# yu45020/Text_Segmentation_Image_Inpainting

Measured on NVIDIA H100. Metric: PartialConv UNet 512x512 images/sec (fwd+bwd), higher is better.
Workload: dtype bf16

## Files before the change

text_segmentation_image_inpainting_b200/csrc/conv_stem.cu:

```cuda
#include <string.h>

#include <algorithm>

#include "pcb_common.cuh"

namespace {

constexpr int S2D_C = 32;
constexpr int SK = 4;

struct StemPlan {
    bool ok;
    pcb_conv sub;
    size_t sub_fe;
    size_t fwd_extra;
};

StemPlan plan_of(const pcb_conv *c) {
    StemPlan K;
    memset(&K, 0, sizeof(K));
    if (getenv("PCB_DISABLE_S2D_STEM")) return K;
    if (c->dtype != PCB_BF16 || c->groups != 1 || c->nparts != 1 || c->kh != 7 || c->kw != 7 || c->stride != 2 || c->pad_h != 3 || c->pad_w != 3 ||
        c->dil != 1) return K;
    const pcb_part &p = c->parts[0];
    if (p.x_up || p.c > 8 || p.x_cstride != 8 || (p.mask && p.mask_up != 0) || ((c->h | c->w) & 1)) return K;
    if (p.x && (reinterpret_cast<uintptr_t>(p.x) & 15)) return K;
    if (c->ho != c->h / 2 || c->wo != c->w / 2 || c->cout < 32 || (c->cout & 7)) return K;
    pcb_conv &S = K.sub;
    S.n = c->n; S.h = c->h / 2; S.w = c->w / 2; S.cin = S2D_C; S.cout = c->cout; S.kh = S.kw = SK; S.stride = 1; S.pad_h = S.pad_w = 2; S.dil = 1;
    S.groups = 1; S.ho = S.h; S.wo = S.w; S.dtype = PCB_BF16; S.no_guard = c->no_guard; S.nparts = 1;
    S.parts[0].x = nullptr; S.parts[0].mask = nullptr; S.parts[0].c = S2D_C; S.parts[0].x_cstride = S2D_C;
    if (!pcb_tc_eligible(&S)) return K;
    size_t de;
    pcb_tc_weight_layout(&S, &K.sub_fe, &de);
    K.sub_fe = (K.sub_fe + 63) / 64 * 64;
    K.fwd_extra = K.sub_fe + 2 * static_cast<size_t>(c->cout) * SK * SK * S2D_C;
    K.ok = true;
    return K;
}

size_t rup256(size_t v) { return (v + 255) / 256 * 256; }
size_t s2d_bytes(const pcb_conv *c) { return rup256(static_cast<size_t>(c->n) * (c->h / 2) * (c->w / 2) * S2D_C * sizeof(bf16)); }
size_t dwsub_bytes(const pcb_conv *c) { return rup256(sizeof(float) * c->cout * SK * SK * S2D_C); }

__global__ void s2d_kernel(const bf16 *__restrict__ x, const uint8_t *__restrict__ mask, bf16 *__restrict__ xs, int n, int h, int w) {
    const int hs = h >> 1, ws = w >> 1;
    const long long total = static_cast<long long>(n) * hs * ws * 2;
    for (long long i = blockIdx.x * static_cast<long long>(blockDim.x) + threadIdx.x; i < total; i += static_cast<long long>(gridDim.x) * blockDim.x) {
        const int a = static_cast<int>(i & 1);
        const long long cell = i >> 1;
        const int sx = static_cast<int>(cell % ws);
        const long long t = cell / ws;
        const int sy = static_cast<int>(t % hs), img = static_cast<int>(t / hs);
        const long long q = (static_cast<long long>(img) * h + 2 * sy + a) * w + 2 * sx;
        uint4 v0 = __ldg(reinterpret_cast<const uint4 *>(x + q * 8)), v1 = __ldg(reinterpret_cast<const uint4 *>(x + q * 8 + 8));
        if (mask) {
            if (mask[q] == 0) v0 = make_uint4(0u, 0u, 0u, 0u);
            if (mask[q + 1] == 0) v1 = make_uint4(0u, 0u, 0u, 0u);
        }
        uint4 *dst = reinterpret_cast<uint4 *>(xs + cell * S2D_C + a * 16);
        dst[0] = v0; dst[1] = v1;
    }
}

__global__ void stem_weight_kernel(const float *__restrict__ w, float *__restrict__ wsub, int cout, int cin) {
    const int i = blockIdx.x * blockDim.x + threadIdx.x;
    if (i >= cout * SK * SK * S2D_C) return;
    const int k = i % S2D_C, jb = (i / S2D_C) % SK, ja = (i / (S2D_C * SK)) % SK, co = i / (S2D_C * SK * SK);
    const int ch = k & 7, b = (k >> 3) & 1, a = k >> 4;
    const int ty = 2 * ja + a - 1, tx = 2 * jb + b - 1;
    wsub[i] = (ty >= 0 && ty < 7 && tx >= 0 && tx < 7 && ch < cin) ? w[((static_cast<long long>(co) * 7 + ty) * 7 + tx) * cin + ch] : 0.f;
}

__global__ void stem_dw_gather_kernel(const float *__restrict__ dwsub, float *__restrict__ dw, int cout, int cin) {
    const int i = blockIdx.x * blockDim.x + threadIdx.x;
    if (i >= cout * 49 * cin) return;
    const int ch = i % cin, tx = (i / cin) % 7, ty = (i / (cin * 7)) % 7, co = i / (cin * 49);
    const int ja = (ty + 1) >> 1, a = (ty + 1) & 1, jb = (tx + 1) >> 1, b = (tx + 1) & 1;
    dw[i] += dwsub[((static_cast<long long>(co) * SK + ja) * SK + jb) * S2D_C + (a * 2 + b) * 8 + ch];
}

int run_s2d(const pcb_conv *c, bf16 *xs, cudaStream_t st) {
    const pcb_part &p = c->parts[0];
    PCB_CHECK(p.x != nullptr, "space-to-depth stem: null x");
    const long long total = static_cast<long long>(c->n) * (c->h / 2) * (c->w / 2) * 2;
    const int grid = static_cast<int>(std::max<long long>(1, std::min<long long>((total + 255) / 256, 16ll * pcb_num_sms())));
    s2d_kernel<<<grid, 256, 0, st>>>(static_cast<const bf16 *>(p.x), p.mask, xs, c->n, c->h, c->w);
    PCB_LAUNCH_CHECK();
    return 0;
}

}

bool pcb_stem_ok(const pcb_conv *c) { return plan_of(c).ok; }

size_t pcb_stem_weight_extra(const pcb_conv *c) {
    const StemPlan K = plan_of(c);
    return K.ok ? K.fwd_extra : 0;
}

size_t pcb_stem_workspace(const pcb_conv *c) {
    StemPlan K = plan_of(c);
    if (!K.ok) return 0;
    return s2d_bytes(c) + dwsub_bytes(c) + pcb_tc_workspace(&K.sub);
}

int pcb_stem_weight_prepare(const pcb_conv *c, const float *w_master, void *w_fwd_extra, bool zero_padding, cudaStream_t st) {
    const StemPlan K = plan_of(c);
    PCB_CHECK(K.ok && w_fwd_extra, "space-to-depth stem: weight prepare on a layer that does not take this path");
    float *wsub = reinterpret_cast<float *>(static_cast<bf16 *>(w_fwd_extra) + K.sub_fe);
    const int total = c->cout * SK * SK * S2D_C;
    stem_weight_kernel<<<(total + 255) / 256, 256, 0, st>>>(w_master, wsub, c->cout, c->cin);
    PCB_LAUNCH_CHECK();
    return pcb_tc_weight_prepare(&K.sub, wsub, w_fwd_extra, nullptr, zero_padding, st);
}

int pcb_stem_forward(const pcb_conv *c, const void *w_fwd_extra, const float *bias, void *y, int y_cstride, const float *msum, void *workspace,
                     double *bn_sums, const pcb_ep *ep, cudaStream_t st) {
    StemPlan K = plan_of(c);
    PCB_CHECK(K.ok && workspace, "space-to-depth stem forward: wrong layer / no workspace");
    uint8_t *ws = static_cast<uint8_t *>(workspace);
    bf16 *xs = reinterpret_cast<bf16 *>(ws);
    if (int rc = run_s2d(c, xs, st)) return rc;
    K.sub.parts[0].x = xs;
    uint64_t *sub_ws = reinterpret_cast<uint64_t *>(ws + s2d_bytes(c) + dwsub_bytes(c));
    if (int rc = pcb_tc_forward_mask_pass(&K.sub, sub_ws, st)) return rc;
    return pcb_tc_forward_ws(&K.sub, w_fwd_extra, bias, y, y_cstride, msum, sub_ws, true, bn_sums, ep, st);
}

int pcb_stem_wgrad(const pcb_conv *c, const void *dc, int dc_cstride, float *dw, void *workspace, bool zero_dw, cudaStream_t st) {
    StemPlan K = plan_of(c);
    PCB_CHECK(K.ok && workspace, "space-to-depth stem wgrad: wrong layer / no workspace");
    if (zero_dw) PCB_CUDA(cudaMemsetAsync(dw, 0, sizeof(float) * c->cout * 49 * c->cin, st));
    uint8_t *ws = static_cast<uint8_t *>(workspace);
    bf16 *xs = reinterpret_cast<bf16 *>(ws);
    float *dwsub = reinterpret_cast<float *>(ws + s2d_bytes(c));
    void *sub_ws = ws + s2d_bytes(c) + dwsub_bytes(c);
    if (int rc = run_s2d(c, xs, st)) return rc;
    K.sub.parts[0].x = xs;
    if (int rc = pcb_tc_wgrad(&K.sub, dc, dc_cstride, dwsub, sub_ws, true, st)) return rc;
    const int total = c->cout * 49 * c->cin;
    stem_dw_gather_kernel<<<(total + 255) / 256, 256, 0, st>>>(dwsub, dw, c->cout, c->cin);
    PCB_LAUNCH_CHECK();
    return 0;
}
```

text_segmentation_image_inpainting_b200/csrc/conv_tc.cu:

```cuda
#include <cuda.h>
#include <stdlib.h>
#include <string.h>

#include <algorithm>

#include "pcb_common.cuh"
#include "pcb_ptx.cuh"

namespace {

constexpr int BLOCK_M = 128;
constexpr int BLOCK_K = 64;
constexpr int A_STAGE_BYTES = BLOCK_M * 128;
constexpr int NUM_PRODUCER_THREADS = 128;
constexpr int TC_MAX_PARTS = 2;
constexpr int MMA_WARPS = 8;
constexpr int MMA_THREADS = MMA_WARPS * 32;
constexpr int acc_pitch(int block_n) { return block_n + 4; }
constexpr int acc_stage_bytes(int block_n) { return BLOCK_M * acc_pitch(block_n) * 4; }

inline int rup(int v, int m) { return (v + m - 1) / m * m; }

struct TcPart {
    const bf16 *x;
// ... 371 lines not shown
                }
#pragma unroll
                for (int p = 0; p < TC_MAX_PARTS; ++p)
                    if (p < P.nparts) wnext[p][i] = __ldg(P.parts[p].tapmask + idx);
            }
        };
        issue_mask_loads(blockIdx.x);
        for (int tile = blockIdx.x; tile < num_tiles && !dead; tile += gridDim.x) {
            const int m0 = (tile / n_tiles) * BLOCK_M, n0 = (tile % n_tiles) * BLOCK_N;
            uint64_t wcur[TC_MAX_PARTS][NW];
#pragma unroll
            for (int p = 0; p < TC_MAX_PARTS; ++p)
#pragma unroll
                for (int i = 0; i < NW; ++i) wcur[p][i] = wnext[p][i];
            issue_mask_loads(tile + gridDim.x);
            if (!tile_active(n0)) continue;
            if (HALO) {
                int ph[HALO_MAX_HG];
                int cterm[TC_MAX_PARTS][HALO_MAX_HG];
                uint32_t vb[TC_MAX_PARTS][HALO_MAX_HG];
#pragma unroll
                for (int i = 0; i < HALO_MAX_HG; ++i) {
                    ph[i] = 0;
#pragma unroll
                    for (int p = 0; p < TC_MAX_PARTS; ++p) { vb[p][i] = 0; cterm[p][i] = 0; }
                    if (i >= HG) continue;
                    const int S = r0 + 16 * i;
                    const int g = S / HG, sl = S - g * HG;
                    const int m = m0 + g * 8;
                    const bool ok = m < P.m_total;
                    const int mm = ok ? m : 0;
                    const int nn = mm / plane, rem = mm - nn * plane;
                    const int hh = rem / pwid, ww = rem - hh * pwid;
                    if (MODE == 0) {
                        ph[i] = hh - P.pad_h;
                        const int col = ww - P.pad_w + sl;
                        const int tcs = sl > 7 ? (sl - 7 + P.dil - 1) / P.dil : 0;
#pragma unroll
                        for (int p = 0; p < TC_MAX_PARTS; ++p) {
                            if (p >= P.nparts || !ok) continue;
                            const TcPart &pt = P.parts[p];
                            const uint64_t word = wcur[p][i];
                            uint32_t bits = 0;
                            for (int tr = 0; tr < P.kh; ++tr) bits |= static_cast<uint32_t>((word >> (tr * P.kw + tcs)) & 1ull) << tr;
                            vb[p][i] = bits;
                            const int colc = min(max(col, 0), P.w - 1) >> pt.xup;
                            cterm[p][i] = (nn * (P.h >> pt.xup) * (P.w >> pt.xup) + colc) * pt.cstride + chunk * 8;
                        }
                    } else {
                        ph[i] = hh + P.pad_h;
                        const int col = ww + P.pad_w - (P.kw - 1) * P.dil + sl;
                        const bool cok = ok && col >= 0 && col < P.wo;
                        uint32_t bits = 0;
                        for (int tr = 0; tr < P.kh; ++tr) { const int hi = ph[i] - tr * P.dil; bits |= (cok && hi >= 0 && hi < P.ho ? 1u : 0u) << tr; }
                        vb[0][i] = bits;
                        cterm[0][i] = (nn * P.ho * P.wo + min(max(col, 0), P.wo - 1)) * P.dc_cstride + chunk * 8;
                    }
                }
                for (int tr = 0; tr < P.kh && !dead; ++tr) {
#pragma unroll
                    for (int p = 0; p < TC_MAX_PARTS; ++p) {
                        if (p >= np || dead) break;
                        const TcPart &pt = P.parts[p];
                        const bf16 *src = (MODE == 0) ? pt.x : P.dc;
                        const int xup = (MODE == 0) ? pt.xup : 0;
                        const int hmax = ((MODE == 0) ? (P.h >> xup) : P.ho) - 1;
                        const int rowpitch = (MODE == 0) ? (P.w >> xup) * pt.cstride : P.wo * P.dc_cstride;
                        const int nb = ((MODE == 0) ? pt.kext : P.dc_kext) / BLOCK_K;
                        const int c8 = (MODE == 0) ? pt.c8 : P.dc_c8;
                        int rterm[HALO_MAX_HG];
#pragma unroll
                        for (int i = 0; i < HALO_MAX_HG; ++i) {
                            const int hi = (MODE == 0) ? ((ph[i] + tr * P.dil) >> xup) : (ph[i] - tr * P.dil);
                            rterm[i] = cterm[p][i] + min(max(hi, 0), hmax) * rowpitch;
                        }
                        for (int cb = 0; cb < nb; ++cb, ++it) {
                            const int s = it % SA;
                            if (!ptx::mbar_wait(bar_empty_a + 8 * s, ((it / SA) & 1) ^ 1, P.abort_flag, 111)) { dead = true; break; }
                            const bool cv = cb * BLOCK_K + chunk * 8 < c8;
                            const uint32_t dst0 = sA + s * A_STAGE + chunk * LBO + r0 * 16;
                            const bf16 *srcb = src + cb * BLOCK_K;
#pragma unroll
                            for (int i = 0; i < HALO_MAX_HG; ++i) {
                                if (i >= HG) break;
                                ptx::cp_async_16(dst0 + i * 256, srcb + rterm[i], cv && ((vb[p][i] >> tr) & 1u));
                            }
                            ptx::cp_async_mbar_arrive(bar_full_a + 8 * s);
                            ptx::mbar_arrive(bar_full_a + 8 * s);
                        }
                    }
                }
            } else {
                const uint32_t sw = static_cast<uint32_t>((chunk ^ (r0 & 7)) << 4);
                int ph[8], pw[8];
                int ibase[TC_MAX_PARTS][8];
                bool prow[8];
                const int ls = 31 - __clz(P.stride);
#pragma unroll
                for (int i = 0; i < 8; ++i) {
                    const int m = m0 + r0 + 16 * i;
                    prow[i] = m < P.m_total;
                    const int mm = prow[i] ? m : 0;
                    const int nn = mm / plane, rem = mm - nn * plane;
                    const int hh = rem / pwid, ww = rem - hh * pwid;
                    if (MODE == 0) {
                        ph[i] = hh * P.stride - P.pad_h; pw[i] = ww * P.stride - P.pad_w;
#pragma unroll
                        for (int p = 0; p < TC_MAX_PARTS; ++p)
                            ibase[p][i] = (p < P.nparts) ? nn * (P.h >> P.parts[p].xup) * (P.w >> P.parts[p].xup) * P.parts[p].cstride + chunk * 8 : 0;
                    } else {
                        ph[i] = hh + P.pad_h; pw[i] = ww + P.pad_w;
                        ibase[0][i] = nn * P.ho * P.wo * P.dc_cstride + chunk * 8;
#pragma unroll
                        for (int p = 1; p < TC_MAX_PARTS; ++p) ibase[p][i] = 0;
                    }
                }
                uint64_t tmv[TC_MAX_PARTS][8];
#pragma unroll
                for (int p = 0; p < TC_MAX_PARTS; ++p)
#pragma unroll
                    for (int i = 0; i < 8; ++i) tmv[p][i] = wcur[p][i];

                auto push = [&](const bf16 *base, const int (&off)[8], const bool (&ok)[8]) -> bool {
                    const int s = it % SA;
                    if (!ptx::mbar_wait(bar_empty_a + 8 * s, ((it / SA) & 1) ^ 1, P.abort_flag, 101)) return false;
                    const uint32_t dst = sA + s * A_STAGE + r0 * 128 + sw;
#pragma unroll
                    for (int i = 0; i < 8; ++i) ptx::cp_async_16(dst + i * (16 * 128), base + off[i], ok[i]);
                    ptx::cp_async_mbar_arrive(bar_full_a + 8 * s);
                    ptx::mbar_arrive(bar_full_a + 8 * s);
                    ++it;
                    return true;
                };
                if (MODE == 0 && P.rowpack) {
                    const TcPart &pt = P.parts[0];
                    const int cs = pt.cstride, rowpitch = P.w * cs;
                    for (int tr = 0; tr < P.kh && !dead; ++tr) {
                        int off[8];
                        bool ok[8];
#pragma unroll
                        for (int i = 0; i < 8; ++i) {
                            const bool v = (chunk < P.kw) && ((tmv[0][i] >> (tr * P.kw + chunk)) & 1ull);
                            off[i] = v ? (ibase[0][i] - chunk * 8) + (ph[i] + tr * P.dil) * rowpitch + (pw[i] + chunk * P.dil) * cs : 0;
                            ok[i] = v;
                        }
                        if (!push(pt.x, off, ok)) dead = true;
                    }
                } else {
                    for (int tap = 0; tap < taps && !dead; ++tap) {
                        const int tr = tap / P.kw, tc = tap - tr * P.kw;
#pragma unroll
                        for (int p = 0; p < TC_MAX_PARTS; ++p) {
                            if (p >= np || dead) break;
                            const TcPart &pt = P.parts[p];
                            const bf16 *src = (MODE == 0) ? pt.x : P.dc;
                            const int cs = (MODE == 0) ? pt.cstride : P.dc_cstride;
                            const int xup = (MODE == 0) ? pt.xup : 0;
                            const int rowpitch = ((MODE == 0) ? (P.w >> xup) : P.wo) * cs;
                            int base[8];
                            bool rv[8];
#pragma unroll
                            for (int i = 0; i < 8; ++i) {
                                bool v;
                                int hi, wi;
                                if (MODE == 0) {
                                    v = (tmv[p][i] >> tap) & 1ull;
                                    hi = (ph[i] + tr * P.dil) >> xup; wi = (pw[i] + tc * P.dil) >> xup;
                                } else {
                                    const int th = ph[i] - tr * P.dil, tw = pw[i] - tc * P.dil;
                                    hi = th >> ls; wi = tw >> ls;
                                    v = prow[i] && th >= 0 && tw >= 0 && ((th | tw) & (P.stride - 1)) == 0 && hi < P.ho && wi < P.wo;
                                }
                                base[i] = v ? ibase[p][i] + hi * rowpitch + wi * cs : 0;
                                rv[i] = v;
                            }
                            const int nb = ((MODE == 0) ? pt.kext : P.dc_kext) / BLOCK_K;
                            const int c8 = (MODE == 0) ? pt.c8 : P.dc_c8;
                            for (int cb = 0; cb < nb; ++cb) {
                                const bool cv = cb * BLOCK_K + chunk * 8 < c8;
                                int off[8];
                                bool ok[8];
#pragma unroll
                                for (int i = 0; i < 8; ++i) { ok[i] = rv[i] && cv; off[i] = ok[i] ? base[i] + cb * BLOCK_K : 0; }
                                if (!push(src, off, ok)) { dead = true; break; }
                            }
                        }
                    }
                }
            }
        }
        ptx::cp_async_wait<0>();
    } else if (warp == 12) {
        if (lane == 0) {
            int itb = 0;
            bool dead = false;
            auto load = [&](int kidx, int n0) -> bool {
                const int s = itb % SB;
                if (!ptx::mbar_wait(bar_empty_b + 8 * s, ((itb / SB) & 1) ^ 1, P.abort_flag, 103)) return false;
                ptx::mbar_arrive_expect_tx(bar_full_b + 8 * s, B_STAGE_BYTES);
                ptx::tma_load_2d(sB + s * B_STAGE_BYTES, &tmap_w, kidx, n0, bar_full_b + 8 * s);
                ++itb;
                return true;
            };
            for (int tile = blockIdx.x; tile < num_tiles && !dead; tile += gridDim.x) {
                const int n0 = (tile % n_tiles) * BLOCK_N;
                if (!tile_active(n0)) continue;
                if (HALO) {
                    for (int tr = 0; tr < P.kh && !dead; ++tr)
                        for (int p = 0; p < np && !dead; ++p) {
                            const int nb = ((MODE == 0) ? P.parts[p].kext : P.dc_kext) / BLOCK_K;
                            for (int cb = 0; cb < nb && !dead; ++cb)
                                for (int tc = 0; tc < P.kw; ++tc) {
                                    const int tap = tr * P.kw + tc;
                                    const int kidx = (MODE == 0) ? tap * P.ktap + P.parts[p].koff + cb * BLOCK_K : tap * P.dc_kext + cb * BLOCK_K;
                                    if (!load(kidx, n0)) { dead = true; break; }
                                }
                        }
                } else {
                    const int num_kb = (MODE == 0) ? (P.rowpack ? P.kh : taps * (P.ktap / BLOCK_K)) : taps * (P.dc_kext / BLOCK_K);
                    for (int kb = 0; kb < num_kb; ++kb)
                        if (!load(kb * BLOCK_K, n0)) { dead = true; break; }
                }
            }
        }
    } else {
        const int e = warp - 4, g = e >> 2;
        const bool leader = (threadIdx.x & 127) == 0;
        int num_a = 0;
        if (HALO) {
            for (int p = 0; p < np; ++p) num_a += ((MODE == 0) ? P.parts[p].kext : P.dc_kext) / BLOCK_K;
            num_a *= P.kh;
        } else {
            num_a = (MODE == 0) ? (P.rowpack ? P.kh : taps * (P.ktap / BLOCK_K)) : taps * (P.dc_kext / BLOCK_K);
        }
        const uint32_t a_rows = HALO ? 8u * HG * 16u : 64u * 128u;
        float *s_stat = (MODE == 0 && P.bn_sums != nullptr && P.partial == nullptr)
                            ? reinterpret_cast<float *>(smem_raw + (s_stat_addr - ptx::smem_u32(smem_raw))) : nullptr;
        const EpiRole<BLOCK_N> R(e);
        float *my_stat = s_stat ? s_stat + R.slice() * STAT_SLICE : nullptr;
        int stat_n0 = -1;
        if (my_stat) {
            for (int i = lane; i < STAT_SLICE; i += 32) my_stat[i] = 0.f;
            __syncwarp();
        }
        int ita = 0, itb = 0;
        bool dead = false;
        for (int tile = blockIdx.x; tile < num_tiles && !dead; tile += gridDim.x) {
            const int m0 = (tile / n_tiles) * BLOCK_M, n0 = (tile % n_tiles) * BLOCK_N;
            if (!tile_active(n0)) continue;
            if (my_stat && n0 != stat_n0) {
                if (stat_n0 >= 0) tc_stats_flush<BLOCK_N>(P, my_stat, lane, stat_n0, R.cb, R.ce, 128);
                stat_n0 = n0;
            }
            float acc[BLOCK_N / 2];
            zero_acc(acc);
            for (int a = 0; a < num_a && !dead; ++a, ++ita) {
                const int sa = ita % SA;
                if (!__all_sync(0xffffffffu, ptx::mbar_wait(bar_full_a + 8 * sa, (ita / SA) & 1, P.abort_flag, 104))) { dead = true; break; }
                ptx::fence_proxy_async_smem();
                const int sb0 = itb % SB;
                for (int tc = 0; tc < nB; ++tc, ++itb) {
                    const int sb = itb % SB;
                    if (!__all_sync(0xffffffffu, ptx::mbar_wait(bar_full_b + 8 * sb, (itb / SB) & 1, P.abort_flag, 105))) { dead = true; break; }
                    const uint64_t db = ptx::make_smem_desc(sB + sb * B_STAGE_BYTES, 16, 1024);
                    ptx::wgmma_fence();
                    if (HALO) {
                        const int shift = ((MODE == 0) ? tc : (P.kw - 1 - tc)) * P.dil;
                        const uint32_t a0 = sA + sa * A_STAGE + g * a_rows + shift * 16;
#pragma unroll
                        for (int k = 0; k < BLOCK_K / 16; ++k)
                            ptx::wgmma_bf16<BLOCK_N, 0, 0>(acc, ptx::make_smem_desc_noswizzle(a0 + k * 2 * LBO, LBO, HG * 16), db + 2 * k);
                    } else {
                        const uint64_t da = ptx::make_smem_desc(sA + sa * A_STAGE + g * a_rows, 16, 1024);
#pragma unroll
                        for (int k = 0; k < BLOCK_K / 16; ++k)
                            ptx::wgmma_bf16<BLOCK_N, 0, 0>(acc, da + 2 * k, db + 2 * k);
                    }
                    ptx::wgmma_commit();
                }
                ptx::wgmma_wait<0>();
                ptx::wgmma_fence_regs(acc);
                if (leader) {
                    for (int tc = 0; tc < nB; ++tc) ptx::mbar_arrive(bar_empty_b + 8 * ((sb0 + tc) % SB));
                    ptx::mbar_arrive(bar_empty_a + 8 * sa);
                }
            }
            if (dead) { stat_n0 = -1; break; }
            mma_epilogue<BLOCK_N, MODE>(P, acc, acc_stage, e, lane, m0, n0, my_stat);
        }
        if (my_stat && stat_n0 >= 0) tc_stats_flush<BLOCK_N>(P, my_stat, lane, stat_n0, R.cb, R.ce, 128);
    }
}


constexpr int EPI_WARP0 = MMA_WARPS + 4;
constexpr int TMA_THREADS = (EPI_WARP0 + EPI_WARPS) * 32;
constexpr int TMA_FIX_THREADS = 96;
constexpr int TMA_REGS = 128;
constexpr int TMA_CONSUMER_REGS = 192, TMA_SUPPORT_REGS = 64;
static_assert(TMA_THREADS == 512 && 2 * 128 * TMA_CONSUMER_REGS + 2 * 128 * TMA_SUPPORT_REGS == TMA_THREADS * TMA_REGS &&
              TMA_THREADS * TMA_REGS <= 65536, "TMA-fed fwd / dgrad register budget");

constexpr size_t TMA_BAR_BYTES = 24 * MAX_RING + 16;

template <int BLOCK_N, int MODE>
__device__ __forceinline__ void tc_epilogue_bf16(const TcParams &P, const EpiRow &er, const bf16 *srow, int lane, int n0, float *s_stat) {
    const bool stats = (MODE == 0) && (s_stat != nullptr);
#pragma unroll 1
    for (int c0 = 0; c0 < BLOCK_N; c0 += 32) {
        const int col = n0 + c0;
        bf16 *orow = nullptr;
        int nstore = 0;
        float scale = 1.f;
        if (MODE == 0) {
            if (er.rvalid && col < P.y_cstride) { orow = P.y + er.mo * P.y_cstride + col; nstore = min(32, P.y_cstride - col); }
        } else {
#pragma unroll
            for (int p = 0; p < TC_MAX_PARTS; ++p) {
                if (p >= P.nparts) break;
                const TcPart &pt = P.parts[p];
                const int local = col - pt.koff;
                if (local >= 0 && local < pt.kext && pt.dx != nullptr && local < pt.c8 && er.rvalid) {
                    orow = pt.dx + er.mo * pt.dx_cstride + local;
                    nstore = min(32, pt.c8 - local);
                    scale = er.dscale[p];
                }
            }
        }
        if (nstore == 0 && !stats) continue;
        uint4 o[4];
#pragma unroll
        for (int j = 0; j < 4; ++j) o[j] = reinterpret_cast<const uint4 *>(srow + c0)[j];
        if (MODE == 1 && scale != 1.f) {
            __nv_bfloat162 *ob = reinterpret_cast<__nv_bfloat162 *>(o);
#pragma unroll
            for (int j = 0; j < 16; ++j) {
                const float2 f = __bfloat1622float2(ob[j]);
                ob[j] = __floats2bfloat162_rn(f.x * scale, f.y * scale);
            }
        }
        if (nstore > 0) {
            uint4 *dst = reinterpret_cast<uint4 *>(orow);
#pragma unroll
            for (int j = 0; j < 4; ++j)
                if (j * 8 < nstore) dst[j] = o[j];
        }
        if (stats) {
            const float live = er.rvalid ? 1.f : 0.f;
            const __nv_bfloat162 *ob = reinterpret_cast<const __nv_bfloat162 *>(o);
            float cs = 0.f, cq = 0.f;
#pragma unroll
            for (int h = 0; h < 2; ++h) {
                float v[16];
#pragma unroll
                for (int j = 0; j < 8; ++j) {
                    const float2 f = __bfloat1622float2(ob[8 * h + j]);
                    v[2 * j] = f.x * live; v[2 * j + 1] = f.y * live;
                }
                const float s = warp_transpose_sum16(v, lane);
#pragma unroll
                for (int j = 0; j < 8; ++j) {
                    const float2 f = __bfloat1622float2(ob[8 * h + j]);
                    const float a = f.x * live, b = f.y * live;
                    v[2 * j] = a * a; v[2 * j + 1] = b * b;
                }
                const float q = warp_transpose_sum16(v, lane);
                if ((lane >> 4) == h) { cs = s; cq = q; }
            }
            s_stat[c0 + lane] += cs;
            s_stat[EPI_STAT_SQ + c0 + lane] += cq;
        }
    }
}

template <int BLOCK_N, int MODE, typename TileFn>
__device__ __forceinline__ void tma_epilogue_warps(const TcParams &P, int tile0, int tstep, int num_tiles, TileFn tile_origin,
                                                   const uint8_t *stage, uint32_t acc_full, uint32_t acc_empty, float *s_stat,
                                                   int &stat_n0, int w, int lane, int code) {
    const int row = w * 32 + lane;
    const bool f32 = P.partial != nullptr;
    if (s_stat) {
        for (int i = lane; i < EPI_STAT_SLICE; i += 32) s_stat[i] = 0.f;
        __syncwarp();
    }
    uint32_t ph = 0;
    for (int tile = tile0; tile < num_tiles; tile += tstep) {
        int m0, n0;
        tile_origin(tile, m0, n0);
        if (n0 < 0) continue;
        if (s_stat && n0 != stat_n0) {
            if (stat_n0 >= 0) tc_stats_flush<BLOCK_N>(P, s_stat, lane, stat_n0, 0, BLOCK_N, EPI_STAT_SQ);
            stat_n0 = n0;
        }
        const EpiRow er = tc_epi_row<MODE>(P, m0 + row, false);
        if (!__all_sync(0xffffffffu, ptx::mbar_wait(acc_full, ph, P.abort_flag, code))) { stat_n0 = -1; return; }
        ph ^= 1;
        if constexpr (BLOCK_N <= 128) {
            if (f32) tc_epilogue<BLOCK_N, MODE>(P, er, reinterpret_cast<const float *>(stage) + row * acc_pitch(BLOCK_N), lane, n0, s_stat, 0, BLOCK_N, EPI_STAT_SQ);
        }
        if (!f32) tc_epilogue_bf16<BLOCK_N, MODE>(P, er, reinterpret_cast<const bf16 *>(stage) + row * bf16_pitch(BLOCK_N), lane, n0, s_stat);
        __syncwarp();
        if (lane == 0) ptx::mbar_arrive(acc_empty);
    }
}

struct ConsRows {
    float inv[2];
    bool hole[2];
};
template <int MODE>
__device__ __forceinline__ ConsRows cons_rows(const TcParams &P, int m0, int e, int lane) {
    ConsRows cr;
#pragma unroll
    for (int h = 0; h < 2; ++h) {
        cr.inv[h] = 0.f; cr.hole[h] = false;
        if (MODE == 0 && P.partial == nullptr) {
            const EpiRow er = tc_epi_row<0>(P, m0 + 64 * (e >> 2) + 16 * (e & 3) + (lane >> 2) + 8 * h);
            cr.inv[h] = er.inv; cr.hole[h] = er.hole;
        }
    }
    return cr;
}

template <int BLOCK_N, int MODE>
__device__ __forceinline__ void stage_acc_bf16(const TcParams &P, const float (&acc)[BLOCK_N / 2], bf16 *stage, int e, int lane, int n0,
                                               const ConsRows &cr) {
    constexpr int PITCH = bf16_pitch(BLOCK_N);
    const int r0 = 64 * (e >> 2) + 16 * (e & 3) + (lane >> 2), c0 = 2 * (lane & 3);
    const bool has_bias = (MODE == 0) && (P.bias != nullptr);
    const bool ep = (MODE == 0) && (P.ep_on != 0);
    const bool ep_aff = ep && (P.ep_scale != nullptr);
#pragma unroll
    for (int j = 0; j < BLOCK_N / 8; ++j) {
        const int col = n0 + 8 * j + c0;
        float b0 = 0.f, b1 = 0.f, s0 = 1.f, s1 = 1.f, t0 = 0.f, t1 = 0.f;
        if (MODE == 0) {
            const bool in0 = col < P.cout, in1 = col + 1 < P.cout;
            if (has_bias) { if (in0) b0 = __ldg(P.bias + col); if (in1) b1 = __ldg(P.bias + col + 1); }
            if (ep_aff) {
                if (in0) { s0 = __ldg(P.ep_scale + col); t0 = __ldg(P.ep_shift + col); }
                if (in1) { s1 = __ldg(P.ep_scale + col + 1); t1 = __ldg(P.ep_shift + col + 1); }
            }
        }
#pragma unroll
        for (int h = 0; h < 2; ++h) {
            float a = acc[4 * j + 2 * h], b = acc[4 * j + 2 * h + 1];
            if (MODE == 0) {
                a = cr.hole[h] ? 0.f : fmaf(a, cr.inv[h], b0);
                b = cr.hole[h] ? 0.f : fmaf(b, cr.inv[h], b1);
                if (ep) {
                    a = apply_act(fmaf(a, s0, t0), P.ep_act, P.ep_slope);
                    b = apply_act(fmaf(b, s1, t1), P.ep_act, P.ep_slope);
                }
                if (col >= P.cout) a = 0.f;
                if (col + 1 >= P.cout) b = 0.f;
            }
            *reinterpret_cast<__nv_bfloat162 *>(stage + (r0 + 8 * h) * PITCH + 8 * j + c0) = __floats2bfloat162_rn(a, b);
        }
    }
}

template <int BLOCK_N, int MODE>
__device__ __forceinline__ bool tma_stage_tile(const TcParams &P, const float (&acc)[BLOCK_N / 2], uint8_t *stage, uint32_t acc_full,
                                               uint32_t acc_empty, uint32_t &ph, int e, int lane, int n0, const ConsRows &cr, int code) {
    if (!__all_sync(0xffffffffu, ptx::mbar_wait(acc_empty, ph, P.abort_flag, code))) return false;
    ph ^= 1;
    if constexpr (BLOCK_N <= 128) {
        if (P.partial != nullptr) stage_acc<BLOCK_N>(acc, reinterpret_cast<float *>(stage), e, lane);
    }
    if (P.partial == nullptr) stage_acc_bf16<BLOCK_N, MODE>(P, acc, reinterpret_cast<bf16 *>(stage), e, lane, n0, cr);
    __syncwarp();
    if (lane == 0) ptx::mbar_arrive(acc_full);
    return true;
}

template <int BLOCK_N, int MODE, bool HALO>
__global__ void __maxnreg__(TMA_REGS)
pconv_tc_tma_kernel(const __grid_constant__ TcParams P, const __grid_constant__ CUtensorMap tmap_w,
                    const __grid_constant__ CUtensorMap tmap_a0, const __grid_constant__ CUtensorMap tmap_a1) {
    constexpr uint32_t B_BYTES = BLOCK_N * 128;
    extern __shared__ uint8_t smem_raw[];
    const uint32_t smem_base = align1024(ptx::smem_u32(smem_raw));
    const int S = P.stages;
    const int nB = HALO ? P.kw : 1;
    const int hx = HALO ? (P.kw - 1) * P.dil : 0;
    const uint32_t A_BYTES = static_cast<uint32_t>(BLOCK_M + hx) * 128u;
    const uint32_t A_ROOM = (A_BYTES + 1023u) & ~1023u;
    const uint32_t STAGE = A_ROOM + nB * B_BYTES;
    const uint32_t STAGE_TX = A_BYTES + nB * B_BYTES;
    const uint32_t sBar = smem_base + S * STAGE;
    const uint32_t bar_full = sBar, bar_fixed = sBar + 8 * MAX_RING, bar_empty = sBar + 16 * MAX_RING;
    const uint32_t acc_full = sBar + 24 * MAX_RING, acc_empty = acc_full + 8;
    const uint32_t s_stat_addr = sBar + TMA_BAR_BYTES;
    const uint32_t s_acc = s_stat_addr + EPI_STAT_SMEM_BYTES;
    uint8_t *smem_gen = smem_raw + (smem_base - ptx::smem_u32(smem_raw));

    const int warp = __shfl_sync(0xffffffffu, threadIdx.x >> 5, 0), lane = threadIdx.x & 31;
    const int np = (MODE == 0) ? P.nparts : 1;
    const int n_tiles = P.ncols / BLOCK_N;
    const int KS = P.ksplit;
    const int m_tiles = (P.m_total + BLOCK_M - 1) / BLOCK_M;
    const int num_tiles = m_tiles * n_tiles * KS;
    const int tile0 = static_cast<int>(blockIdx.x), tstep = static_cast<int>(gridDim.x);
    auto m0_of = [&](int mt) -> int { return mt * BLOCK_M; };
    const bool fix = (MODE == 0) && P.use_fix;
    const int kwi = HALO ? 1 : P.kw;

    auto tile_active = [&](int n0) -> bool {
        if (MODE == 0) return true;
        for (int p = 0; p < P.nparts; ++p)
            if (P.parts[p].dx && n0 < P.parts[p].koff + P.parts[p].kext && n0 + BLOCK_N > P.parts[p].koff) return true;
        return false;
    };

    if (threadIdx.x == 0) {
        for (int s = 0; s < MAX_RING; ++s) {
            ptx::mbar_init(bar_full + 8 * s, 1); ptx::mbar_init(bar_fixed + 8 * s, TMA_FIX_THREADS / 32); ptx::mbar_init(bar_empty + 8 * s, 2);
        }
        ptx::mbar_init(acc_full, MMA_WARPS); ptx::mbar_init(acc_empty, EPI_WARPS);
        ptx::fence_mbar_init();
    }
    if (warp == 8 && lane == 0) { ptx::prefetch_tmap(&tmap_w); ptx::prefetch_tmap(&tmap_a0); if (np > 1) ptx::prefetch_tmap(&tmap_a1); }
    __syncthreads();

    float *s_stat = nullptr;
    int stat_n0 = -1;
    uint8_t *acc_stage = smem_gen + (s_acc - smem_base);
    if (warp < MMA_WARPS) {
        ptx::setmaxnreg_inc<TMA_CONSUMER_REGS>();
        const int e = warp, g = warp >> 2;
        const bool leader = (threadIdx.x & 127) == 0;
        const uint32_t ready = fix ? bar_fixed : bar_full;
        const uint64_t desc_a0 = ptx::make_smem_desc(smem_base + g * 64 * 128, 16, 1024);
        const uint64_t desc_b0 = ptx::make_smem_desc(smem_base + A_ROOM, 16, 1024);
        const uint32_t stage16 = STAGE >> 4;
        const int shift0 = (HALO && MODE == 1) ? hx * 8 : 0;
        const int dshift = HALO ? ((MODE == 1) ? -P.dil * 8 : P.dil * 8) : 0;
        const int rows_a = P.kh * kwi;
        int nb0, nb1 = 0, kl0, kl1 = 4;
        {
            const int kext = (MODE == 0) ? P.parts[0].kext : P.dc_kext, c8 = (MODE == 0) ? P.parts[0].c8 : P.dc_c8;
            nb0 = kext / BLOCK_K; kl0 = min(4, (c8 - (nb0 - 1) * BLOCK_K + 15) >> 4);
            if (MODE == 0 && np > 1) { nb1 = P.parts[1].kext / BLOCK_K; kl1 = min(4, (P.parts[1].c8 - (nb1 - 1) * BLOCK_K + 15) >> 4); }
        }
        int s = 0;
        uint32_t ph = 0, aph = 1;
        bool dead = false;
        for (int tile = tile0; tile < num_tiles && !dead; tile += tstep) {
            const int sp = tile % KS, mn = tile / KS;
            const int n0 = (mn % n_tiles) * BLOCK_N;
            if (!tile_active(n0)) continue;
            const ConsRows cr = cons_rows<MODE>(P, m0_of(mn / n_tiles), e, lane);
            float acc[BLOCK_N / 2];
            zero_acc(acc);
            int held = -1;
            for (int r = 0; r < rows_a && !dead; ++r) {
#pragma unroll
                for (int p = 0; p < TC_MAX_PARTS; ++p) {
                    const int nbp = (p == 0) ? nb0 : nb1, klast = (p == 0) ? kl0 : kl1;
                    const int gb0 = (p == 0) ? 0 : nb0;
                    for (int cb = 0; cb < nbp; ++cb) {
                        if (KS > 1 && (gb0 + cb) % KS != sp) continue;
                        if (!__all_sync(0xffffffffu, ptx::mbar_wait(ready + 8 * s, ph, P.abort_flag, 124))) { dead = true; break; }
                        uint64_t da = desc_a0 + static_cast<uint64_t>(s * stage16 + shift0), db = desc_b0 + static_cast<uint64_t>(s * stage16);
                        const int ksteps = (cb + 1 < nbp) ? 4 : klast;
                        ptx::wgmma_fence();
                        for (int tc = 0; tc < nB; ++tc, da += dshift, db += B_BYTES >> 4) {
                            if (ksteps == 4) {
#pragma unroll
                                for (int k = 0; k < 4; ++k) ptx::wgmma_bf16<BLOCK_N, 0, 0>(acc, da + 2 * k, db + 2 * k);
                            } else {
                                for (int k = 0; k < ksteps; ++k) ptx::wgmma_bf16<BLOCK_N, 0, 0>(acc, da + 2 * k, db + 2 * k);
                            }
                        }
                        ptx::wgmma_commit();
                        ptx::wgmma_wait<1>();
                        if (held >= 0 && leader) ptx::mbar_arrive(bar_empty + 8 * held);
                        held = s;
                        if (++s == S) { s = 0; ph ^= 1; }
                    }
                    if (dead) break;
                }
            }
            ptx::wgmma_wait<0>();
            ptx::wgmma_fence_regs(acc);
            if (held >= 0 && leader) ptx::mbar_arrive(bar_empty + 8 * held);
            if (dead) break;
            if (!tma_stage_tile<BLOCK_N, MODE>(P, acc, acc_stage, acc_full, acc_empty, aph, e, lane, n0, cr, 125)) break;
        }
    } else {
        ptx::setmaxnreg_dec<TMA_SUPPORT_REGS>();
        if (warp >= EPI_WARP0) {
            const int w = warp - EPI_WARP0;
            s_stat = (MODE == 0 && P.bn_sums != nullptr && P.partial == nullptr)
                         ? reinterpret_cast<float *>(smem_gen + (s_stat_addr - smem_base)) + w * EPI_STAT_SLICE : nullptr;
            auto origin = [&](int tile, int &m0, int &n0) {
                const int mn = tile / KS;
                m0 = m0_of(mn / n_tiles); n0 = (mn % n_tiles) * BLOCK_N;
                if (!tile_active(n0)) n0 = -1;
            };
            tma_epilogue_warps<BLOCK_N, MODE>(P, tile0, tstep, num_tiles, origin, acc_stage, acc_full, acc_empty, s_stat, stat_n0, w, lane, 126);
            ptx::named_sync(1, EPI_WARPS * 32);
            if (s_stat != nullptr && stat_n0 >= 0) tc_stats_final<BLOCK_N>(P, s_stat - w * EPI_STAT_SLICE, w, lane, stat_n0);
        } else if (warp == 8) {
            int s = 0;
            uint32_t ph = 1;
            const int plane = (MODE == 0) ? P.ho * P.wo : P.h * P.w;
            const int pwid = (MODE == 0) ? P.wo : P.w;
            const int kext0 = (MODE == 0) ? P.parts[0].kext : P.dc_kext, kext1 = (MODE == 0 && np > 1) ? P.parts[1].kext : 0;
            const int dstep = (MODE == 0) ? P.dil : -P.dil;
            const int row_k = P.wk_row, col_k = P.wk_col;
            bool dead = false;
            for (int tile = tile0; tile < num_tiles && !dead; tile += tstep) {
                const int sp = tile % KS, mn = tile / KS;
                const int m0 = m0_of(mn / n_tiles), n0 = (mn % n_tiles) * BLOCK_N;
                if (!tile_active(n0)) continue;
                const int img = m0 / plane, rem = m0 - img * plane;
                const int oy = rem / pwid, ox = rem - oy * pwid;
                const int x_org = (MODE == 0) ? ox * P.stride - P.pad_w : (HALO ? ox + P.pad_w - hx : ox + P.pad_w);
                const int y_org = (MODE == 0) ? oy * P.stride - P.pad_h : oy + P.pad_h;
                int nx_org = 0, ny_org = 0, nimg = -1;
                if (P.l2pf && tile + tstep < num_tiles) {
                    const int nmn = (tile + tstep) / KS;
                    const int nm0 = m0_of(nmn / n_tiles);
                    if (nm0 != m0) {
                        nimg = nm0 / plane;
                        const int nrem = nm0 - nimg * plane, noy = nrem / pwid, nox = nrem - noy * pwid;
                        nx_org = (MODE == 0) ? nox * P.stride - P.pad_w : (HALO ? nox + P.pad_w - hx : nox + P.pad_w);
                        ny_org = (MODE == 0) ? noy * P.stride - P.pad_h : noy + P.pad_h;
                    }
                }
                int krow = P.wk_base;
                for (int tr = 0, y = y_org; tr < P.kh && !dead; ++tr, y += dstep, krow += row_k)
                    for (int ti = 0, x = x_org, kidx = krow; ti < kwi && !dead; ++ti, x += dstep, kidx = krow + ti * col_k) {
#pragma unroll
                        for (int p = 0; p < TC_MAX_PARTS; ++p) {
                            const int kext = (p == 0) ? kext0 : kext1;
                            const CUtensorMap *ma = (p == 0) ? &tmap_a0 : &tmap_a1;
                            const int gb0 = (p == 0) ? 0 : kext0 / BLOCK_K;
                            for (int c0 = 0; c0 < kext; c0 += BLOCK_K, kidx += BLOCK_K) {
                                if (KS > 1 && (gb0 + c0 / BLOCK_K) % KS != sp) continue;
                                if (!__all_sync(0xffffffffu, ptx::mbar_wait(bar_empty + 8 * s, ph, P.abort_flag, 121))) { dead = true; break; }
                                if (ptx::elect_one()) {
                                    const uint32_t full = bar_full + 8 * s, dst = smem_base + s * STAGE;
                                    ptx::mbar_arrive_expect_tx(full, STAGE_TX);
                                    ptx::tma_load_4d(dst, ma, c0, x, y, img, full);
                                    uint32_t bdst = dst + A_ROOM;
                                    for (int tc = 0, kb = kidx; tc < nB; ++tc, kb += col_k, bdst += B_BYTES)
                                        ptx::tma_load_2d(bdst, &tmap_w, kb, n0, full);
                                    if (nimg >= 0) ptx::tma_prefetch_4d(ma, c0, nx_org + ti * dstep, ny_org + tr * dstep, nimg);
                                }
                                __syncwarp();
                                if (++s == S) { s = 0; ph ^= 1; }
                            }
                            if (dead) break;
                        }
                    }
            }
        } else {
            if (fix) {
                constexpr int FR = HALO ? 3 : 2;
                const int t = (warp - 9) * 32 + lane;
                int s = 0;
                uint32_t ph = 0;
                bool dead = false;
                auto zero_row = [&](int row) {
                    uint4 *r = reinterpret_cast<uint4 *>(smem_gen + s * STAGE + row * 128);
                    const uint4 z = make_uint4(0u, 0u, 0u, 0u);
#pragma unroll
                    for (int k = 0; k < 8; ++k) r[k] = z;
                };
                if (!HALO) {
                    uint64_t wnext[FR][TC_MAX_PARTS];
                    auto load_words = [&](int tl) {
#pragma unroll
                        for (int r = 0; r < FR; ++r)
#pragma unroll
                            for (int p = 0; p < TC_MAX_PARTS; ++p) {
                                wnext[r][p] = 0ull;
                                const int m = m0_of(tl / KS / n_tiles) + t + TMA_FIX_THREADS * r;
                                if (p < P.nparts && tl < num_tiles && t + TMA_FIX_THREADS * r < BLOCK_M && m < P.m_total)
                                    wnext[r][p] = __ldg(P.parts[p].tapmask + m);
                            }
                    };
                    load_words(tile0);
                    for (int tile = tile0; tile < num_tiles && !dead; tile += tstep) {
                        const int sp = tile % KS;
                        uint64_t wcur[FR][TC_MAX_PARTS];
#pragma unroll
                        for (int r = 0; r < FR; ++r)
#pragma unroll
                            for (int p = 0; p < TC_MAX_PARTS; ++p) wcur[r][p] = wnext[r][p];
                        load_words(tile + tstep);
                        if (MODE == 1 && !tile_active(((tile / KS) % n_tiles) * BLOCK_N)) continue;
                        const int taps = P.kh * P.kw;
                        for (int tap = 0; tap < taps && !dead; ++tap) {
#pragma unroll
                            for (int p = 0; p < TC_MAX_PARTS; ++p) {
                                if (p >= np) break;
                                bool hole[FR], mine = false;
#pragma unroll
                                for (int r = 0; r < FR; ++r) {
                                    hole[r] = t + TMA_FIX_THREADS * r < BLOCK_M && ((wcur[r][p] >> tap) & 1ull) == 0ull;
                                    mine = mine || hole[r];
                                }
                                const bool any_hole = __any_sync(0xffffffffu, mine);
                                const int nb = ((MODE == 0) ? P.parts[p].kext : P.dc_kext) / BLOCK_K;
                                const int gb0 = (p == 0) ? 0 : P.parts[0].kext / BLOCK_K;
                                for (int cb = 0; cb < nb; ++cb) {
                                    if (KS > 1 && (gb0 + cb) % KS != sp) continue;
                                    if (!ptx::mbar_wait(bar_full + 8 * s, ph, P.abort_flag, 122)) { dead = true; break; }
                                    if (any_hole) {
#pragma unroll
                                        for (int r = 0; r < FR; ++r)
                                            if (hole[r]) zero_row(t + TMA_FIX_THREADS * r);
                                        ptx::fence_proxy_async_smem();
                                    }
                                    __syncwarp();
                                    if (lane == 0) ptx::mbar_arrive(bar_fixed + 8 * s);
                                    if (++s == S) { s = 0; ph ^= 1; }
                                }
                                if (dead) break;
                            }
                        }
                    }
                } else {
                    const int plane = P.ho * P.wo;
                    auto load_bits = [&](int tl, uint32_t (&b)[FR]) {
#pragma unroll
                        for (int r = 0; r < FR; ++r) b[r] = 0;
                        if (tl >= num_tiles) return;
                        const int m0 = m0_of(tl / KS / n_tiles);
                        const int img = m0 / plane, rem = m0 - img * plane;
                        const int oy = rem / P.wo, ox = rem - oy * P.wo;
#pragma unroll
                        for (int p = 0; p < TC_MAX_PARTS; ++p) {
                            if (p >= P.nparts || P.parts[p].mask == nullptr) continue;
                            const int mup = P.parts[p].mup;
                            const uint8_t *mk = P.parts[p].mask + static_cast<long long>(img) * (P.h >> mup) * (P.w >> mup);
                            for (int tr = 0; tr < P.kh; ++tr) {
                                const int y = oy - P.pad_h + tr * P.dil;
                                if (y < 0 || y >= P.h) continue;
#pragma unroll
                                for (int r = 0; r < FR; ++r) {
                                    const int row = t + TMA_FIX_THREADS * r, x = ox - P.pad_w + row;
                                    if (row < BLOCK_M + hx && x >= 0 && x < P.w && __ldg(mk + (y >> mup) * (P.w >> mup) + (x >> mup)) == 0)
                                        b[r] |= 1u << (p * 8 + tr);
                                }
                            }
                        }
                    };
                    uint32_t nb_bits[FR];
                    load_bits(tile0, nb_bits);
                    for (int tile = tile0; tile < num_tiles && !dead; tile += tstep) {
                        const int sp = tile % KS;
                        uint32_t cb_bits[FR];
#pragma unroll
                        for (int r = 0; r < FR; ++r) cb_bits[r] = nb_bits[r];
                        load_bits(tile + tstep, nb_bits);
                        if (MODE == 1 && !tile_active(((tile / KS) % n_tiles) * BLOCK_N)) continue;
                        for (int tr = 0; tr < P.kh && !dead; ++tr) {
#pragma unroll
                            for (int p = 0; p < TC_MAX_PARTS; ++p) {
                                if (p >= np) break;
                                bool hole[FR], mine = false;
#pragma unroll
                                for (int r = 0; r < FR; ++r) { hole[r] = (cb_bits[r] >> (p * 8 + tr)) & 1u; mine = mine || hole[r]; }
                                const bool any_hole = __any_sync(0xffffffffu, mine);
                                const int nb = ((MODE == 0) ? P.parts[p].kext : P.dc_kext) / BLOCK_K;
                                const int gb0 = (p == 0) ? 0 : P.parts[0].kext / BLOCK_K;
                                for (int cb = 0; cb < nb; ++cb) {
                                    if (KS > 1 && (gb0 + cb) % KS != sp) continue;
                                    if (!ptx::mbar_wait(bar_full + 8 * s, ph, P.abort_flag, 122)) { dead = true; break; }
                                    if (any_hole) {
#pragma unroll
                                        for (int r = 0; r < FR; ++r)
                                            if (hole[r]) zero_row(t + TMA_FIX_THREADS * r);
                                        ptx::fence_proxy_async_smem();
                                    }
                                    __syncwarp();
                                    if (lane == 0) ptx::mbar_arrive(bar_fixed + 8 * s);
                                    if (++s == S) { s = 0; ph ^= 1; }
                                }
                                if (dead) break;
                            }
                        }
                    }
                }
            }
        }
    }

}


constexpr int SP_MAX_ITEMS = 40;
struct SpItem { int part, dx, dy, wk, nb, wk_step, shift0, dshift; };
struct SpTable {
    int n_items;
    int step[TC_MAX_PARTS];
    int es[TC_MAX_PARTS];
    int ph[TC_MAX_PARTS], pw[TC_MAX_PARTS];
    int arows[TC_MAX_PARTS];
    int rows_max;
    SpItem it[SP_MAX_ITEMS];
};

template <int BLOCK_N, int MODE>
__global__ void __maxnreg__(TMA_REGS)
pconv_tc_sp_kernel(const __grid_constant__ TcParams P, const __grid_constant__ SpTable TB, const __grid_constant__ CUtensorMap tmap_w,
                   const __grid_constant__ CUtensorMap tmap_a0, const __grid_constant__ CUtensorMap tmap_a1) {
    constexpr uint32_t B_BYTES = BLOCK_N * 128;
    extern __shared__ uint8_t smem_raw[];
    const uint32_t smem_base = align1024(ptx::smem_u32(smem_raw));
    const int S = P.stages;
    int nb_max = 1;
    for (int i = 0; i < TB.n_items; ++i) nb_max = max(nb_max, TB.it[i].nb);
    const uint32_t A_ROOM = (static_cast<uint32_t>(TB.rows_max) * 128u + 1023u) & ~1023u;
    const uint32_t STAGE = A_ROOM + nb_max * B_BYTES;
    const uint32_t sBar = smem_base + S * STAGE;
    const uint32_t bar_full = sBar, bar_fixed = sBar + 8 * MAX_RING, bar_empty = sBar + 16 * MAX_RING;
    const uint32_t acc_full = sBar + 24 * MAX_RING, acc_empty = acc_full + 8;
    const uint32_t s_stat_addr = sBar + TMA_BAR_BYTES;
    const uint32_t s_acc = s_stat_addr + EPI_STAT_SMEM_BYTES;
    uint8_t *smem_gen = smem_raw + (smem_base - ptx::smem_u32(smem_raw));

    const int warp = __shfl_sync(0xffffffffu, threadIdx.x >> 5, 0), lane = threadIdx.x & 31;
    const int n_tiles = P.ncols / BLOCK_N;
    const int m_tiles = (P.m_total + BLOCK_M - 1) / BLOCK_M;
    const int num_tiles = m_tiles * n_tiles;
    const int tile0 = static_cast<int>(blockIdx.x), tstep = static_cast<int>(gridDim.x);
    const bool fix = P.use_fix != 0;
    const int gw = (MODE == 0) ? P.wo : P.w, gh = (MODE == 0) ? P.ho : P.h;
    const int plane = gw * gh;
    int nbk[TC_MAX_PARTS], klast[TC_MAX_PARTS];
#pragma unroll
    for (int p = 0; p < TC_MAX_PARTS; ++p) {
        const int kext = (MODE == 0) ? P.parts[p].kext : P.dc_kext, c8 = (MODE == 0) ? P.parts[p].c8 : P.dc_c8;
        nbk[p] = (p < ((MODE == 0) ? P.nparts : 1)) ? kext / BLOCK_K : 0;
        klast[p] = nbk[p] ? min(4, (c8 - (nbk[p] - 1) * BLOCK_K + 15) >> 4) : 4;
    }

    if (threadIdx.x == 0) {
        for (int s = 0; s < MAX_RING; ++s) { ptx::mbar_init(bar_full + 8 * s, 1); ptx::mbar_init(bar_fixed + 8 * s, TMA_FIX_THREADS / 32); ptx::mbar_init(bar_empty + 8 * s, 2); }
        ptx::mbar_init(acc_full, MMA_WARPS); ptx::mbar_init(acc_empty, EPI_WARPS);
        ptx::fence_mbar_init();
    }
    if (warp == 8 && lane == 0) { ptx::prefetch_tmap(&tmap_w); ptx::prefetch_tmap(&tmap_a0); ptx::prefetch_tmap(&tmap_a1); }
    __syncthreads();

    float *s_stat = nullptr;
    int stat_n0 = -1;
    uint8_t *acc_stage = smem_gen + (s_acc - smem_base);
    if (warp < MMA_WARPS) {
        ptx::setmaxnreg_inc<TMA_CONSUMER_REGS>();
        const int e = warp, g = warp >> 2;
        const bool leader = (threadIdx.x & 127) == 0;
        const uint32_t ready = fix ? bar_fixed : bar_full;
        const uint64_t desc_a0 = ptx::make_smem_desc(smem_base + g * 64 * 128, 16, 1024);
        const uint64_t desc_b0 = ptx::make_smem_desc(smem_base + A_ROOM, 16, 1024);
        const uint32_t stage16 = STAGE >> 4;
        int s = 0;
        uint32_t ph = 0, aph = 1;
        bool dead = false;
        for (int tile = tile0; tile < num_tiles && !dead; tile += tstep) {
            const ConsRows cr = cons_rows<MODE>(P, (tile / n_tiles) * BLOCK_M, e, lane);
            float acc[BLOCK_N / 2];
            zero_acc(acc);
            int held = -1;
            for (int i = 0; i < TB.n_items && !dead; ++i) {
                const SpItem it = TB.it[i];
                for (int cb = 0; cb < nbk[it.part]; ++cb) {
                    if (!__all_sync(0xffffffffu, ptx::mbar_wait(ready + 8 * s, ph, P.abort_flag, 324))) { dead = true; break; }
                    uint64_t da = desc_a0 + static_cast<uint64_t>(s * stage16 + it.shift0), db = desc_b0 + static_cast<uint64_t>(s * stage16);
                    const int ksteps = (cb + 1 < nbk[it.part]) ? 4 : klast[it.part];
                    ptx::wgmma_fence();
                    for (int tc = 0; tc < it.nb; ++tc, da += it.dshift, db += B_BYTES >> 4)
                        for (int k = 0; k < ksteps; ++k) ptx::wgmma_bf16<BLOCK_N, 0, 0>(acc, da + 2 * k, db + 2 * k);
                    ptx::wgmma_commit();
                    ptx::wgmma_wait<1>();
                    if (held >= 0 && leader) ptx::mbar_arrive(bar_empty + 8 * held);
                    held = s;
                    if (++s == S) { s = 0; ph ^= 1; }
                }
            }
            ptx::wgmma_wait<0>();
            ptx::wgmma_fence_regs(acc);
            if (held >= 0 && leader) ptx::mbar_arrive(bar_empty + 8 * held);
            if (dead) break;
            if (!tma_stage_tile<BLOCK_N, MODE>(P, acc, acc_stage, acc_full, acc_empty, aph, e, lane, (tile % n_tiles) * BLOCK_N, cr, 325)) break;
        }
    } else {
        ptx::setmaxnreg_dec<TMA_SUPPORT_REGS>();
        if (warp >= EPI_WARP0) {
            const int w = warp - EPI_WARP0;
            s_stat = (MODE == 0 && P.bn_sums != nullptr) ? reinterpret_cast<float *>(smem_gen + (s_stat_addr - smem_base)) + w * EPI_STAT_SLICE : nullptr;
            auto origin = [&](int tile, int &m0, int &n0) { m0 = (tile / n_tiles) * BLOCK_M; n0 = (tile % n_tiles) * BLOCK_N; };
            tma_epilogue_warps<BLOCK_N, MODE>(P, tile0, tstep, num_tiles, origin, acc_stage, acc_full, acc_empty, s_stat, stat_n0, w, lane, 326);
            ptx::named_sync(1, EPI_WARPS * 32);
            if (s_stat != nullptr && stat_n0 >= 0) tc_stats_final<BLOCK_N>(P, s_stat - w * EPI_STAT_SLICE, w, lane, stat_n0);
        } else if (warp == 8) {
            int s = 0;
            uint32_t ph = 1;
            bool dead = false;
            for (int tile = tile0; tile < num_tiles && !dead; tile += tstep) {
                const int m0 = (tile / n_tiles) * BLOCK_M, n0 = (tile % n_tiles) * BLOCK_N;
                const int img = m0 / plane, rem = m0 - img * plane;
                const int oy = rem / gw, ox = rem - oy * gw;
                for (int i = 0; i < TB.n_items && !dead; ++i) {
                    const SpItem it = TB.it[i];
                    const CUtensorMap *ma = (it.part == 0) ? &tmap_a0 : &tmap_a1;
                    const int x = ox * TB.step[it.part] + it.dx, y = oy * TB.step[it.part] + it.dy;
                    const uint32_t a_bytes = static_cast<uint32_t>(TB.arows[it.part]) * 128u;
                    for (int cb = 0; cb < nbk[it.part]; ++cb) {
                        if (!__all_sync(0xffffffffu, ptx::mbar_wait(bar_empty + 8 * s, ph, P.abort_flag, 321))) { dead = true; break; }
                        if (ptx::elect_one()) {
                            const uint32_t full = bar_full + 8 * s, dst = smem_base + s * STAGE;
                            ptx::mbar_arrive_expect_tx(full, a_bytes + it.nb * B_BYTES);
                            ptx::tma_load_4d(dst, ma, cb * BLOCK_K, x, y, img, full);
                            uint32_t bdst = dst + A_ROOM;
                            for (int tc = 0, kb = it.wk + cb * BLOCK_K; tc < it.nb; ++tc, kb += it.wk_step, bdst += B_BYTES)
                                ptx::tma_load_2d(bdst, &tmap_w, kb, n0, full);
                        }
                        __syncwarp();
                        if (++s == S) { s = 0; ph ^= 1; }
                    }
                }
            }
        } else {
            if (fix) {
                constexpr int FR = 3;
                const int t = (warp - 9) * 32 + lane;
                int s = 0;
                uint32_t ph = 0;
                bool dead = false;
                auto load_bits = [&](int tl, uint64_t (&b)[FR]) {
#pragma unroll
                    for (int r = 0; r < FR; ++r) b[r] = 0ull;
                    if (tl >= num_tiles) return;
                    const int m0 = (tl / n_tiles) * BLOCK_M;
                    const int img = m0 / plane, rem = m0 - img * plane;
                    const int oy = rem / gw, ox = rem - oy * gw;
                    for (int i = 0; i < TB.n_items; ++i) {
                        const SpItem it = TB.it[i];
                        const uint8_t *mk = P.parts[it.part].mask;
                        if (mk == nullptr) continue;
                        const int pwid = TB.pw[it.part], phei = TB.ph[it.part], es = TB.es[it.part];
                        const int hrows = TB.arows[it.part] - BLOCK_M;
                        const int x0 = ox * TB.step[it.part] + it.dx, y0 = oy * TB.step[it.part] + it.dy;
#pragma unroll
                        for (int r = 0; r < FR; ++r) {
                            const int row = t + TMA_FIX_THREADS * r;
// ... 15 lines not shown
                    for (int r = 0; r < FR; ++r) cb_bits[r] = nb_bits[r];
                    load_bits(tile + tstep, nb_bits);
                    for (int i = 0; i < TB.n_items && !dead; ++i) {
                        bool hole[FR], mine = false;
#pragma unroll
                        for (int r = 0; r < FR; ++r) { hole[r] = (cb_bits[r] >> i) & 1ull; mine = mine || hole[r]; }
                        const bool any_hole = __any_sync(0xffffffffu, mine);
                        const int nb_i = nbk[TB.it[i].part];
                        for (int cb = 0; cb < nb_i; ++cb) {
                            if (!ptx::mbar_wait(bar_full + 8 * s, ph, P.abort_flag, 322)) { dead = true; break; }
                            if (any_hole) {
                                const uint4 z = make_uint4(0u, 0u, 0u, 0u);
#pragma unroll
                                for (int r = 0; r < FR; ++r)
                                    if (hole[r]) {
                                        uint4 *rw = reinterpret_cast<uint4 *>(smem_gen + s * STAGE + (t + TMA_FIX_THREADS * r) * 128);
#pragma unroll
                                        for (int k = 0; k < 8; ++k) rw[k] = z;
                                    }
                                ptx::fence_proxy_async_smem();
                            }
                            __syncwarp();
                            if (lane == 0) ptx::mbar_arrive(bar_fixed + 8 * s);
                            if (++s == S) { s = 0; ph ^= 1; }
                        }
                    }
                }
            }
        }
    }

}

__global__ void upsample_part_kernel(const bf16 *__restrict__ src, int cstride, int c8, long long pixels_src, int hs, int ws, bf16 *__restrict__ dst) {
    const int chunks = c8 >> 3;
    const long long total = pixels_src * chunks;
    for (long long i = blockIdx.x * static_cast<long long>(blockDim.x) + threadIdx.x; i < total; i += static_cast<long long>(gridDim.x) * blockDim.x) {
        const int ch = static_cast<int>(i % chunks);
        const long long pix = i / chunks;
        const int x = static_cast<int>(pix % ws);
        const long long t = pix / ws;
        const int y = static_cast<int>(t % hs);
        const long long n = t / hs;
        const uint4 v = __ldg(reinterpret_cast<const uint4 *>(src + pix * cstride + ch * 8));
        bf16 *d = dst + ((n * (2 * hs) + 2 * y) * (2ll * ws) + 2 * x) * c8 + ch * 8;
        uint4 *d0 = reinterpret_cast<uint4 *>(d), *d1 = reinterpret_cast<uint4 *>(d + 2ll * ws * c8);
        d0[0] = v; *reinterpret_cast<uint4 *>(d + c8) = v;
        d1[0] = v; *reinterpret_cast<uint4 *>(d + 2ll * ws * c8 + c8) = v;
    }
}

struct WgParams {
    int n, h, w, cin, cout, kh, kw, stride, pad_h, pad_w, dil, ho, wo;
    int m_total;
    int nparts, rowpack;
    int ktap;
    int ntaps;
    TcPart parts[TC_MAX_PARTS];
    int tap_groups;
    int ci_tiles;
    int kb_per_split;
    float *dw;
    int *abort_flag;
    int box_w, box_h, box_n, stages, use_fix;
};

constexpr int WGRAD_THREADS = MMA_THREADS + 5 * 32;

template <int BLOCK_N, int T>
__device__ __forceinline__ void wgrad_store(const WgParams &P, const float (&acc)[T][BLOCK_N / 2], int ntap, int lane, int n0,
                                            int ncols, const int (&ci)[2], const int (&tap)[2][T]) {
    const int taps_full = P.kh * P.kw;
#pragma unroll
    for (int tl = 0; tl < T; ++tl) {
        if (tl >= ntap) break;
#pragma unroll
        for (int i = 0; i < BLOCK_N / 2; ++i) {
            if (2 * i >= ncols) break;
            const int h = (i >> 1) & 1;
            const int co = n0 + 8 * (i >> 2) + 2 * (lane & 3) + (i & 1);
            if (ci[h] >= 0 && co < P.cout)
                atomicAdd(P.dw + (static_cast<long long>(co) * taps_full + tap[h][tl]) * P.cin + ci[h], acc[tl][i]);
        }
    }
}

template <int BLOCK_N, int T, int STAGES>
__global__ void __launch_bounds__(WGRAD_THREADS, 1)
pconv_tc_wgrad_kernel(const __grid_constant__ WgParams P, const __grid_constant__ CUtensorMap tmap_dc) {
    constexpr int B_STAGE_BYTES = BLOCK_N * 128;
    constexpr int A_TAP_BYTES = 16384;
    constexpr int A_STAGE = T * A_TAP_BYTES;
    extern __shared__ uint8_t smem_raw[];
    const uint32_t smem_base = align1024(ptx::smem_u32(smem_raw));
    const uint32_t sA = smem_base;
    const uint32_t sB = sA + STAGES * A_STAGE;
    const uint32_t sBar = sB + STAGES * B_STAGE_BYTES;
    const uint32_t bar_full_a = sBar, bar_full_b = sBar + 8 * STAGES, bar_empty = sBar + 16 * STAGES;

    const int warp = threadIdx.x >> 5, lane = threadIdx.x & 31;
    int bx = blockIdx.x;
    const int ci_tile = bx % P.ci_tiles; bx /= P.ci_tiles;
    const int tap_group = bx % P.tap_groups;
    const int co_tile = bx / P.tap_groups;
    const int taps_full = P.kh * P.kw;
    const int tap0 = tap_group * T;
    const int ntap = min(T, P.ntaps - tap0);
    const int n0 = co_tile * BLOCK_N;
    const int total_kb = (P.m_total + 63) / 64;
    const int kb_begin = blockIdx.y * P.kb_per_split;
    const int kb_end = min(total_kb, kb_begin + P.kb_per_split);
    const int num_kb = max(0, kb_end - kb_begin);

    if (threadIdx.x == 0) {
        for (int s = 0; s < STAGES; ++s) {
            ptx::mbar_init(bar_full_a + 8 * s, NUM_PRODUCER_THREADS);
            ptx::mbar_init(bar_full_b + 8 * s, 1);
            ptx::mbar_init(bar_empty + 8 * s, 2);
        }
        ptx::fence_mbar_init();
    }
    if (warp == 12 && lane == 0) ptx::prefetch_tmap(&tmap_dc);
    __syncthreads();

    if (warp >= MMA_WARPS && warp < MMA_WARPS + 4) {
        const int t = threadIdx.x - MMA_THREADS;
        const int chunk = t & 7, r0 = t >> 3;
        const uint32_t sw = static_cast<uint32_t>((chunk ^ (r0 & 7)) << 4);
        int blk_part[2], blk_off[2];
        bool blk_cv[2];
#pragma unroll
        for (int hb = 0; hb < 2; ++hb) {
            const int kpos = ci_tile * 128 + hb * 64;
            blk_part[hb] = -1; blk_off[hb] = 0; blk_cv[hb] = false;
            if (P.rowpack) {
                if (kpos == 0) { blk_part[hb] = 0; blk_cv[hb] = chunk < P.kw; }
            } else {
                for (int p = 0; p < P.nparts; ++p)
                    if (kpos >= P.parts[p].koff && kpos < P.parts[p].koff + P.parts[p].kext) {
                        blk_part[hb] = p; blk_off[hb] = kpos - P.parts[p].koff;
                        blk_cv[hb] = blk_off[hb] + chunk * 8 < P.parts[p].c8;
                    }
            }
        }
        const int plane = P.ho * P.wo;
        bool dead = false;
        int dtr[T], dtc[T], tbit[T];
#pragma unroll
        for (int tl = 0; tl < T; ++tl) {
            const int tg = tap0 + tl;
            if (P.rowpack) { dtr[tl] = tg * P.dil; dtc[tl] = chunk * P.dil; tbit[tl] = tg * P.kw + chunk; }
            else { const int tr = tg / P.kw, tc = tg - tr * P.kw; dtr[tl] = tr * P.dil; dtc[tl] = tc * P.dil; tbit[tl] = tg; }
        }
        const bf16 *bsrc[2];
        int bcs[2], brow[2], bimg[2], bxup[2], boff[2];
#pragma unroll
        for (int hb = 0; hb < 2; ++hb) {
            const TcPart &pt = P.parts[blk_part[hb] >= 0 ? blk_part[hb] : 0];
            bsrc[hb] = pt.x; bcs[hb] = pt.cstride; bxup[hb] = pt.xup;
            brow[hb] = (P.w >> pt.xup) * pt.cstride;
            bimg[hb] = (P.h >> pt.xup) * brow[hb];
            boff[hb] = P.rowpack ? 0 : blk_off[hb] + chunk * 8;
        }
        const bool fastrow = P.wo >= 64;
        uint64_t tm_next[4][2];
        auto load_tm = [&](int kb, uint64_t (&dst)[4][2]) {
#pragma unroll
            for (int i = 0; i < 4; ++i) {
                const int m = kb * 64 + r0 + 16 * i;
#pragma unroll
                for (int hb = 0; hb < 2; ++hb)
                    dst[i][hb] = (m < P.m_total && blk_part[hb] >= 0 && blk_cv[hb]) ? __ldg(P.parts[blk_part[hb]].tapmask + m) : 0ull;
            }
        };
        if (num_kb > 0) load_tm(kb_begin, tm_next);
        for (int it = 0; it < num_kb && !dead; ++it) {
            const int kb = kb_begin + it;
            const int s = it % STAGES;
            const uint32_t parity = ((it / STAGES) & 1) ^ 1;
            uint64_t tm_cur[4][2];
#pragma unroll
            for (int i = 0; i < 4; ++i) { tm_cur[i][0] = tm_next[i][0]; tm_cur[i][1] = tm_next[i][1]; }
            if (it + 1 < num_kb) load_tm(kb + 1, tm_next);
            const int mf = kb * 64;
            const int nf = mf / plane, remf = mf - nf * plane;
            const int ohf = remf / P.wo, owf = remf - ohf * P.wo;
            if (!ptx::mbar_wait(bar_empty + 8 * s, parity, P.abort_flag, 201)) { dead = true; break; }
#pragma unroll
            for (int i = 0; i < 4; ++i) {
                const int r = r0 + 16 * i;
                int nn = nf, oh = ohf, ow = owf + r;
                if (fastrow) {
                    if (ow >= P.wo) { ow -= P.wo; if (++oh >= P.ho) { oh = 0; ++nn; } }
                } else {
                    const int mm = min(mf + r, P.m_total - 1);
                    nn = mm / plane; const int rem = mm - nn * plane; oh = rem / P.wo; ow = rem - oh * P.wo;
                }
                const int hb0 = oh * P.stride - P.pad_h, wb0 = ow * P.stride - P.pad_w;
#pragma unroll
                for (int tl = 0; tl < T; ++tl) {
                    if (tl >= ntap) break;
                    const int hi = hb0 + dtr[tl], wi = wb0 + dtc[tl];
#pragma unroll
                    for (int hb = 0; hb < 2; ++hb) {
                        const bool v = (tm_cur[i][hb] >> tbit[tl]) & 1ull;
                        const int off = v ? nn * bimg[hb] + (hi >> bxup[hb]) * brow[hb] + (wi >> bxup[hb]) * bcs[hb] + boff[hb] : 0;
                        const uint32_t dst = sA + s * A_STAGE + tl * A_TAP_BYTES + hb * 8192 + r * 128 + sw;
                        ptx::cp_async_16(dst, bsrc[hb] + off, v);
                    }
                }
            }
            ptx::cp_async_mbar_arrive(bar_full_a + 8 * s);
            ptx::mbar_arrive(bar_full_a + 8 * s);
        }
        ptx::cp_async_wait<0>();
    } else if (warp == 12) {
        if (lane == 0) {
            for (int it = 0; it < num_kb; ++it) {
                const int kb = kb_begin + it;
                const int s = it % STAGES;
                const uint32_t parity = ((it / STAGES) & 1) ^ 1;
                if (!ptx::mbar_wait(bar_empty + 8 * s, parity, P.abort_flag, 203)) break;
                ptx::mbar_arrive_expect_tx(bar_full_b + 8 * s, B_STAGE_BYTES);
#pragma unroll
                for (int j = 0; j < BLOCK_N / 64; ++j)
                    ptx::tma_load_2d(sB + s * B_STAGE_BYTES + j * 8192, &tmap_dc, n0 + j * 64, kb * 64, bar_full_b + 8 * s);
            }
        }
    } else if (warp < MMA_WARPS && num_kb > 0) {
        const int g = warp >> 2;
        const bool leader = (threadIdx.x & 127) == 0;
        float acc[T][BLOCK_N / 2];
#pragma unroll
        for (int tl = 0; tl < T; ++tl) zero_acc(acc[tl]);
        bool dead = false;
        int held = -1;
        for (int it = 0; it < num_kb && !dead; ++it) {
            const int s = it % STAGES;
            const uint32_t parity = (it / STAGES) & 1;
            if (!__all_sync(0xffffffffu, ptx::mbar_wait(bar_full_a + 8 * s, parity, P.abort_flag, 204) &&
                                             ptx::mbar_wait(bar_full_b + 8 * s, parity, P.abort_flag, 205))) { dead = true; break; }
            ptx::fence_proxy_async_smem();
            ptx::wgmma_fence();
#pragma unroll
            for (int tl = 0; tl < T; ++tl) {
                if (tl >= ntap) break;
#pragma unroll
                for (int k = 0; k < 4; ++k) {
                    const uint64_t da = ptx::make_smem_desc(sA + s * A_STAGE + tl * A_TAP_BYTES + g * 8192 + k * 2048, 8192, 1024);
                    const uint64_t db = ptx::make_smem_desc(sB + s * B_STAGE_BYTES + k * 2048, 8192, 1024);
                    ptx::wgmma_bf16<BLOCK_N, 1, 1>(acc[tl], da, db);
                }
            }
            ptx::wgmma_commit();
            ptx::wgmma_wait<1>();
            if (held >= 0 && leader) ptx::mbar_arrive(bar_empty + 8 * held);
            held = s;
        }
        ptx::wgmma_wait<0>();
#pragma unroll
        for (int tl = 0; tl < T; ++tl) ptx::wgmma_fence_regs(acc[tl]);
        if (held >= 0 && leader) ptx::mbar_arrive(bar_empty + 8 * held);
        if (!dead) {
            int ci[2], tap[2][T];
            for (int h = 0; h < 2; ++h) {
                const int row = 64 * g + 16 * (warp & 3) + (lane >> 2) + 8 * h;
                const int kpos = ci_tile * 128 + row;
                ci[h] = -1;
#pragma unroll
                for (int tl = 0; tl < T; ++tl) tap[h][tl] = tap0 + tl;
                if (P.rowpack) {
                    const int tc = row >> 3, ch = row & 7;
                    if (row < 64 && ci_tile == 0 && tc < P.kw && ch < P.cin) {
                        ci[h] = ch;
#pragma unroll
                        for (int tl = 0; tl < T; ++tl) tap[h][tl] = (tap0 + tl) * P.kw + tc;
                    }
                } else {
                    for (int p = 0; p < P.nparts; ++p) {
                        const int local = kpos - P.parts[p].koff;
                        if (local >= 0 && local < P.parts[p].c) ci[h] = P.parts[p].choff + local;
                    }
                }
            }
            wgrad_store<BLOCK_N, T>(P, acc, ntap, lane, n0, BLOCK_N, ci, tap);
        }
    }
}


constexpr int WGRAD_TMA_THREADS = 384;
constexpr int WGRAD_FIX_THREADS = 96;
constexpr int WGRAD_TMA_REGS = 168;
constexpr int WGRAD_CONSUMER_REGS = 224, WGRAD_SUPPORT_REGS = 56;
static_assert(2 * 128 * WGRAD_CONSUMER_REGS + 128 * WGRAD_SUPPORT_REGS == WGRAD_TMA_THREADS * WGRAD_TMA_REGS &&
              WGRAD_TMA_THREADS * WGRAD_TMA_REGS <= 65536, "wgrad register budget");

template <int BLOCK_N, int T, bool HALO>
__global__ void __maxnreg__(WGRAD_TMA_REGS)
pconv_tc_wgrad_tma_kernel(const __grid_constant__ WgParams P, const __grid_constant__ CUtensorMap tmap_dc,
                          const __grid_constant__ CUtensorMap tmap_a0, const __grid_constant__ CUtensorMap tmap_a1) {
    constexpr uint32_t B_BYTES = BLOCK_N * 128;
    constexpr int FIX_ROWS = HALO ? 3 : 1;
    extern __shared__ uint8_t smem_raw[];
    const uint32_t smem_base = align1024(ptx::smem_u32(smem_raw));
    uint8_t *smem_gen = smem_raw + (smem_base - ptx::smem_u32(smem_raw));
    const int S = P.stages;
    const int hx = HALO ? (P.kw - 1) * P.dil : 0;
    const int rows_a = 64 + hx;
    const uint32_t A_BLK = (static_cast<uint32_t>(rows_a) * 128u + 1023u) & ~1023u;
    const uint32_t A_BYTES = (HALO ? 1 : T) * 2 * A_BLK;
    const uint32_t STAGE = A_BYTES + B_BYTES;
    const uint32_t sBar = smem_base + S * STAGE;
    const uint32_t bar_full = sBar, bar_fixed = sBar + 8 * MAX_RING, bar_empty = sBar + 16 * MAX_RING;

    const int warp = __shfl_sync(0xffffffffu, threadIdx.x >> 5, 0), lane = threadIdx.x & 31;
    int bx = blockIdx.x;
    const int ci_tile = bx % P.ci_tiles; bx /= P.ci_tiles;
    const int tap_group = bx % P.tap_groups;
    const int co_tile = bx / P.tap_groups;
    const int taps_full = P.kh * P.kw;
    const int tap0 = tap_group * T;
    const int ntap = HALO ? T : min(T, taps_full - tap0);
    const int n0 = co_tile * BLOCK_N;
    const int total_kb = (P.m_total + 63) / 64;
    const int kb_begin = blockIdx.y * P.kb_per_split;
    const int num_kb = max(0, min(total_kb, kb_begin + P.kb_per_split) - kb_begin);
    int blk_part[2], blk_c0[2];
#pragma unroll
    for (int hb = 0; hb < 2; ++hb) {
        const int kpos = ci_tile * 128 + hb * 64;
        blk_part[hb] = -1; blk_c0[hb] = 0;
        for (int p = 0; p < P.nparts; ++p)
            if (kpos >= P.parts[p].koff && kpos < P.parts[p].koff + P.parts[p].kext && kpos - P.parts[p].koff < P.parts[p].c8) {
                blk_part[hb] = p; blk_c0[hb] = kpos - P.parts[p].koff;
            }
    }
    const int nblk = (blk_part[0] >= 0 ? 1 : 0) + (blk_part[1] >= 0 ? 1 : 0);
    const int solo = nblk == 1 ? (blk_part[0] >= 0 ? 0 : 1) : -1;
    const bool fix = P.use_fix != 0;

    if (threadIdx.x == 0) {
        for (int s = 0; s < MAX_RING; ++s) {
            ptx::mbar_init(bar_full + 8 * s, 1);
            ptx::mbar_init(bar_fixed + 8 * s, WGRAD_FIX_THREADS / 32);
            ptx::mbar_init(bar_empty + 8 * s, 2);
        }
        ptx::fence_mbar_init();
    }
    if (warp == 8 && lane == 0) { ptx::prefetch_tmap(&tmap_dc); ptx::prefetch_tmap(&tmap_a0); ptx::prefetch_tmap(&tmap_a1); }
    __syncthreads();
    if (warp < MMA_WARPS) {
        ptx::setmaxnreg_inc<WGRAD_CONSUMER_REGS>();
        const int g = warp >> 2;
        const int ablk = solo >= 0 ? solo : g;
        const bool split_n = solo >= 0 && BLOCK_N == 128;
        const bool live = !(solo >= 0 && BLOCK_N == 64) || g == 0;
        const int nc0 = split_n ? 64 * g : 0, ncols = split_n ? 64 : BLOCK_N;
        const bool leader = (threadIdx.x & 127) == 0;
        const uint32_t ready = fix ? bar_fixed : bar_full;
        const uint64_t desc_a0 = ptx::make_smem_desc(smem_base + ablk * A_BLK, A_BLK, 1024);
        const uint64_t desc_b0 = ptx::make_smem_desc(smem_base + A_BYTES + nc0 * 128, 8192, 1024);
        const uint32_t stage16 = STAGE >> 4;
        const uint32_t tap16 = HALO ? static_cast<uint32_t>(P.dil * 8) : (2 * A_BLK) >> 4;
        float acc[T][BLOCK_N / 2];
#pragma unroll
        for (int tl = 0; tl < T; ++tl) zero_acc(acc[tl]);
        int s = 0, held = -1;
        uint32_t ph = 0;
        bool dead = false;
        for (int it = 0; it < num_kb; ++it) {
            if (!__all_sync(0xffffffffu, ptx::mbar_wait(ready + 8 * s, ph, P.abort_flag, 224))) { dead = true; break; }
            if (!live) {
                if (held >= 0 && leader) ptx::mbar_arrive(bar_empty + 8 * held);
                held = s;
                if (++s == S) { s = 0; ph ^= 1; }
                continue;
            }
            uint64_t da = desc_a0 + static_cast<uint64_t>(s * stage16);
            const uint64_t db = desc_b0 + static_cast<uint64_t>(s * stage16);
            ptx::wgmma_fence();
            if (BLOCK_N == 128 && split_n) {
#pragma unroll
                for (int tl = 0; tl < T; ++tl, da += tap16) {
                    if (tl >= ntap) break;
#pragma unroll
                    for (int k = 0; k < 4; ++k)
                        ptx::wgmma_m64n64<1, 1>(acc[tl], da + 128 * k, db + 128 * k);
                }
            } else {
#pragma unroll
                for (int tl = 0; tl < T; ++tl, da += tap16) {
                    if (tl >= ntap) break;
#pragma unroll
                    for (int k = 0; k < 4; ++k)
                        ptx::wgmma_bf16<BLOCK_N, 1, 1>(acc[tl], da + 128 * k, db + 128 * k);
                }
            }
            ptx::wgmma_commit();
            ptx::wgmma_wait<1>();
            if (held >= 0 && leader) ptx::mbar_arrive(bar_empty + 8 * held);
            held = s;
            if (++s == S) { s = 0; ph ^= 1; }
        }
        ptx::wgmma_wait<0>();
#pragma unroll
        for (int tl = 0; tl < T; ++tl) ptx::wgmma_fence_regs(acc[tl]);
        if (held >= 0 && leader) ptx::mbar_arrive(bar_empty + 8 * held);
        if (!dead && live && num_kb > 0) {
            int ci[2], tap[2][T];
            for (int h = 0; h < 2; ++h) {
                const int kpos = ci_tile * 128 + 64 * ablk + 16 * (warp & 3) + (lane >> 2) + 8 * h;
                ci[h] = -1;
                for (int p = 0; p < P.nparts; ++p) {
                    const int local = kpos - P.parts[p].koff;
                    if (local >= 0 && local < P.parts[p].c) ci[h] = P.parts[p].choff + local;
                }
#pragma unroll
                for (int tl = 0; tl < T; ++tl) tap[h][tl] = tap0 + tl;
            }
            wgrad_store<BLOCK_N, T>(P, acc, ntap, lane, n0 + nc0, ncols, ci, tap);
        }
    } else {
        ptx::setmaxnreg_dec<WGRAD_SUPPORT_REGS>();
        if (warp == 8) {
            const int plane = P.ho * P.wo;
            const uint32_t tx_bytes = static_cast<uint32_t>((HALO ? 1 : ntap) * nblk * rows_a * 128) + B_BYTES;
            int s = 0;
            uint32_t ph = 1;
            for (int it = 0; it < num_kb; ++it) {
                const int m0 = (kb_begin + it) * 64;
                const int img = m0 / plane, rem = m0 - img * plane;
                const int oy = rem / P.wo, ox = rem - oy * P.wo;
                if (!__all_sync(0xffffffffu, ptx::mbar_wait(bar_empty + 8 * s, ph, P.abort_flag, 221))) break;
                if (ptx::elect_one()) {
                    const uint32_t full = bar_full + 8 * s, dst = smem_base + s * STAGE;
                    ptx::mbar_arrive_expect_tx(full, tx_bytes);
                    for (int tl = 0; tl < (HALO ? 1 : ntap); ++tl) {
                        const int tap = tap0 + tl;
                        const int tr = HALO ? tap_group : tap / P.kw, tc = HALO ? 0 : tap - tr * P.kw;
                        const int y = oy * P.stride - P.pad_h + tr * P.dil, x = ox * P.stride - P.pad_w + tc * P.dil;
#pragma unroll
                        for (int hb = 0; hb < 2; ++hb)
                            if (blk_part[hb] >= 0)
                                ptx::tma_load_4d(dst + (tl * 2 + hb) * A_BLK, blk_part[hb] == 0 ? &tmap_a0 : &tmap_a1, blk_c0[hb], x, y, img, full);
                    }
#pragma unroll
                    for (int j = 0; j < BLOCK_N / 64; ++j)
                        ptx::tma_load_2d(dst + A_BYTES + j * 8192, &tmap_dc, n0 + j * 64, m0, full);
                }
                __syncwarp();
                if (++s == S) { s = 0; ph ^= 1; }
            }
        } else if (fix) {
            const int fi = (warp - 9) * 32 + lane;
            int jpix[FIX_ROWS], bit[FIX_ROWS];
#pragma unroll
            for (int j = 0; j < FIX_ROWS; ++j) {
                const int f = fi + WGRAD_FIX_THREADS * j;
                const int tcs = (HALO && f > 63) ? (f - 63 + P.dil - 1) / P.dil : 0;
                jpix[j] = f < rows_a ? f - tcs * P.dil : -1;
                bit[j] = HALO ? tap_group * P.kw + tcs : tap0;
            }
            uint64_t wnext[FIX_ROWS][2];
            auto load_words = [&](int kb) {
#pragma unroll
                for (int j = 0; j < FIX_ROWS; ++j) {
                    const int m = kb * 64 + jpix[j];
#pragma unroll
                    for (int hb = 0; hb < 2; ++hb)
                        wnext[j][hb] = (jpix[j] >= 0 && blk_part[hb] >= 0 && m < P.m_total && kb < kb_begin + num_kb) ? __ldg(P.parts[blk_part[hb]].tapmask + m) : 0ull;
                }
            };
            load_words(kb_begin);
            int s = 0;
            uint32_t ph = 0;
            for (int it = 0; it < num_kb; ++it) {
                uint32_t hole = 0;
#pragma unroll
                for (int j = 0; j < FIX_ROWS; ++j)
#pragma unroll
                    for (int hb = 0; hb < 2; ++hb)
#pragma unroll
                        for (int tl = 0; tl < (HALO ? 1 : T); ++tl)
                            if (tl < ntap && jpix[j] >= 0 && blk_part[hb] >= 0 && ((wnext[j][hb] >> (bit[j] + tl)) & 1ull) == 0ull)
                                hole |= 1u << ((j * 2 + hb) * T + tl);
                load_words(kb_begin + it + 1);
                if (!__all_sync(0xffffffffu, ptx::mbar_wait(bar_full + 8 * s, ph, P.abort_flag, 222))) break;
                if (hole) {
#pragma unroll
                    for (int j = 0; j < FIX_ROWS; ++j)
#pragma unroll
                        for (int hb = 0; hb < 2; ++hb)
#pragma unroll
                            for (int tl = 0; tl < (HALO ? 1 : T); ++tl)
                                if ((hole >> ((j * 2 + hb) * T + tl)) & 1u) {
                                    uint4 *r = reinterpret_cast<uint4 *>(smem_gen + s * STAGE + (tl * 2 + hb) * A_BLK + (fi + WGRAD_FIX_THREADS * j) * 128);
                                    const uint4 z = make_uint4(0u, 0u, 0u, 0u);
#pragma unroll
                                    for (int k = 0; k < 8; ++k) r[k] = z;
                                }
                }
                if (__any_sync(0xffffffffu, hole != 0)) ptx::fence_proxy_async_smem();
                __syncwarp();
                if (lane == 0) ptx::mbar_arrive(bar_fixed + 8 * s);
                if (++s == S) { s = 0; ph ^= 1; }
            }
        }
    }
}

struct TapMaskParams {
    int n, h, w, kh, kw, stride, pad_h, pad_w, dil, ho, wo, m_total, nparts;
    const uint8_t *mask[TC_MAX_PARTS];
    int mup[TC_MAX_PARTS];
    uint64_t *out;
};

__global__ void tapmask_kernel(const TapMaskParams P) {
    const int m = blockIdx.x * blockDim.x + threadIdx.x;
    if (m >= P.m_total) return;
    const int plane = P.ho * P.wo;
    const int nn = m / plane, rem = m - nn * plane, oh = rem / P.wo, ow = rem - oh * P.wo;
#pragma unroll
    for (int p = 0; p < TC_MAX_PARTS; ++p) {
        if (p >= P.nparts) break;
        const uint8_t *mk = P.mask[p];
        const int u = P.mup[p];
        uint64_t bits = 0;
        int tap = 0;
        for (int tr = 0; tr < P.kh; ++tr)
            for (int tc = 0; tc < P.kw; ++tc, ++tap) {
                const int hi = oh * P.stride - P.pad_h + tr * P.dil, wi = ow * P.stride - P.pad_w + tc * P.dil;
                bool v = hi >= 0 && hi < P.h && wi >= 0 && wi < P.w;
                if (v && mk) v = mk[(static_cast<long long>(nn) * (P.h >> u) + (hi >> u)) * (P.w >> u) + (wi >> u)] != 0;
                bits |= (v ? 1ull : 0ull) << tap;
            }
        P.out[static_cast<long long>(p) * P.m_total + m] = bits;
    }
}

struct WPrepParams {
    int cout, taps, cin, kw, rowpack, nparts, ktap, cout64;
    int choff[TC_MAX_PARTS], c[TC_MAX_PARTS], koff[TC_MAX_PARTS];
    long long kf, kd;
};

__global__ void __launch_bounds__(256) tc_weight_prepare_tiled_kernel(const float *__restrict__ wm, const WPrepParams P, bf16 *__restrict__ w_fwd,
                                                                      bf16 *__restrict__ w_dg) {
    __shared__ float tile[32][33];
    const int tap = blockIdx.z, co0 = blockIdx.y * 32, ci0 = blockIdx.x * 32;
    const int tx = threadIdx.x & 31, ty = threadIdx.x >> 5;
#pragma unroll
    for (int i = 0; i < 4; ++i) {
        const int co = co0 + ty + 8 * i, ci = ci0 + tx;
        float v = 0.f;
        if (co < P.cout && ci < P.cin) v = wm[(static_cast<long long>(co) * P.taps + tap) * P.cin + ci];
        tile[ty + 8 * i][tx] = v;
    }
    __syncthreads();
    {
        const int ci = ci0 + tx;
        if (ci < P.cin) {
            int p = 0;
            while (p + 1 < P.nparts && ci >= P.choff[p] + P.c[p]) ++p;
            const int kpos = P.koff[p] + (ci - P.choff[p]);
#pragma unroll
            for (int i = 0; i < 4; ++i) {
                const int co = co0 + ty + 8 * i;
                if (co < P.cout) w_fwd[static_cast<long long>(co) * P.kf + static_cast<long long>(tap) * P.ktap + kpos] = __float2bfloat16_rn(tile[ty + 8 * i][tx]);
            }
        }
    }
    if (w_dg) {
        const int co = co0 + tx;
#pragma unroll
        for (int i = 0; i < 4; ++i) {
            const int ci = ci0 + ty + 8 * i;
            if (co < P.cout && ci < P.cin) {
                int p = 0;
                while (p + 1 < P.nparts && ci >= P.choff[p] + P.c[p]) ++p;
                const int kpos = P.koff[p] + (ci - P.choff[p]);
                w_dg[static_cast<long long>(kpos) * P.kd + static_cast<long long>(tap) * P.cout64 + co] = __float2bfloat16_rn(tile[tx][ty + 8 * i]);
            }
        }
    }
}

__global__ void tc_weight_prepare_kernel(const float *__restrict__ wm, const WPrepParams P, bf16 *__restrict__ w_fwd, bf16 *__restrict__ w_dg) {
    const long long total = static_cast<long long>(P.cout) * P.taps * P.cin;
    for (long long i = blockIdx.x * static_cast<long long>(blockDim.x) + threadIdx.x; i < total; i += static_cast<long long>(gridDim.x) * blockDim.x) {
        const int ci = static_cast<int>(i % P.cin);
        const long long t = i / P.cin;
        const int tap = static_cast<int>(t % P.taps), co = static_cast<int>(t / P.taps);
        const bf16 v = __float2bfloat16_rn(wm[i]);
        if (P.rowpack) {
            const int tr = tap / P.kw, tc = tap - tr * P.kw;
            w_fwd[static_cast<long long>(co) * P.kf + tr * 64 + tc * 8 + ci] = v;
        } else {
            int p = 0;
            while (p + 1 < P.nparts && ci >= P.choff[p] + P.c[p]) ++p;
            const int kpos = P.koff[p] + (ci - P.choff[p]);
            w_fwd[static_cast<long long>(co) * P.kf + static_cast<long long>(tap) * P.ktap + kpos] = v;
            if (w_dg) w_dg[static_cast<long long>(kpos) * P.kd + static_cast<long long>(tap) * P.cout64 + co] = v;
        }
    }
}

typedef CUresult (*EncodeTiledFn)(CUtensorMap *, CUtensorMapDataType, cuuint32_t, void *, const cuuint64_t *,
                                  const cuuint64_t *, const cuuint32_t *, const cuuint32_t *, CUtensorMapInterleave,
                                  CUtensorMapSwizzle, CUtensorMapL2promotion, CUtensorMapFloatOOBfill);

EncodeTiledFn get_encode_fn() {
    static EncodeTiledFn fn = nullptr;
    if (!fn) {
        void *p = nullptr;
        cudaDriverEntryPointQueryResult qres;
        if (cudaGetDriverEntryPoint("cuTensorMapEncodeTiled", &p, cudaEnableDefault, &qres) == cudaSuccess &&
            qres == cudaDriverEntryPointSuccess)
            fn = reinterpret_cast<EncodeTiledFn>(p);
    }
    return fn;
}

int make_tmap_2d(CUtensorMap *tm, const void *base, long long rows, long long cols, long long pitch_elems, int box_rows) {
    EncodeTiledFn enc = get_encode_fn();
    PCB_CHECK(enc != nullptr, "cuTensorMapEncodeTiled not available from the driver");
    cuuint64_t dims[2] = {static_cast<cuuint64_t>(cols), static_cast<cuuint64_t>(rows)};
    cuuint64_t strides[1] = {static_cast<cuuint64_t>(pitch_elems) * 2};
    cuuint32_t box[2] = {64, static_cast<cuuint32_t>(box_rows)};
    cuuint32_t estr[2] = {1, 1};
    CUresult r = enc(tm, CU_TENSOR_MAP_DATA_TYPE_BFLOAT16, 2, const_cast<void *>(base), dims, strides, box, estr,
                     CU_TENSOR_MAP_INTERLEAVE_NONE, CU_TENSOR_MAP_SWIZZLE_128B, CU_TENSOR_MAP_L2_PROMOTION_L2_256B,
                     CU_TENSOR_MAP_FLOAT_OOB_FILL_NONE);
    PCB_CHECK(r == CUDA_SUCCESS, "cuTensorMapEncodeTiled failed (%d) rows=%lld cols=%lld pitch=%lld box_rows=%d base=%p", (int)r,
              rows, cols, pitch_elems, box_rows, base);
    return 0;
}

int make_tmap_nhwc(CUtensorMap *tm, const void *base, int channels, int w, int h, int n, long long cstride, int bx, int by, int bn, int es) {
    EncodeTiledFn enc = get_encode_fn();
    PCB_CHECK(enc != nullptr, "cuTensorMapEncodeTiled not available from the driver");
    cuuint64_t dims[4] = {static_cast<cuuint64_t>(channels), static_cast<cuuint64_t>(w), static_cast<cuuint64_t>(h), static_cast<cuuint64_t>(n)};
    cuuint64_t strides[3] = {static_cast<cuuint64_t>(cstride) * 2, static_cast<cuuint64_t>(w) * cstride * 2, static_cast<cuuint64_t>(h) * w * cstride * 2};
    cuuint32_t box[4] = {64, static_cast<cuuint32_t>(bx * es), static_cast<cuuint32_t>(by * es), static_cast<cuuint32_t>(bn)};
    cuuint32_t estr[4] = {1, static_cast<cuuint32_t>(es), static_cast<cuuint32_t>(es), 1};
    CUresult r = enc(tm, CU_TENSOR_MAP_DATA_TYPE_BFLOAT16, 4, const_cast<void *>(base), dims, strides, box, estr,
                     CU_TENSOR_MAP_INTERLEAVE_NONE, CU_TENSOR_MAP_SWIZZLE_128B, CU_TENSOR_MAP_L2_PROMOTION_L2_256B,
                     CU_TENSOR_MAP_FLOAT_OOB_FILL_NONE);
    PCB_CHECK(r == CUDA_SUCCESS, "cuTensorMapEncodeTiled(4D) failed (%d) c=%d w=%d h=%d n=%d cstride=%lld box=%d,%d,%d es=%d base=%p", (int)r,
              channels, w, h, n, cstride, bx, by, bn, es, base);
    return 0;
}

int *abort_flag_ptr() {
    static int *flag[PCB_MAX_DEVICES] = {};
    const int dev = pcb_cur_device();
    if (!flag[dev]) {
        if (cudaMalloc(&flag[dev], sizeof(int)) != cudaSuccess) { flag[dev] = nullptr; return nullptr; }
        cudaMemset(flag[dev], 0, sizeof(int));
    }
    return flag[dev];
}

bool is_rowpack(const pcb_conv *c) { return c->nparts == 1 && c->cin <= 8 && c->kw <= 8 && c->parts[0].x_up == 0; }

bool common_ok(const pcb_conv *c) {
    if (c->dtype != PCB_BF16 || c->groups != 1 || c->kh * c->kw > 64) return false;
    if (c->stride & (c->stride - 1)) return false;
    const long long lim = (1ll << 31) - 1;
    if (static_cast<long long>(c->n) * c->ho * c->wo * rup(c->cout, 64) > lim) return false;
    if (c->nparts < 1 || c->nparts > TC_MAX_PARTS) return false;
    for (int p = 0; p < c->nparts; ++p) {
        const pcb_part &pt = c->parts[p];
        if (pt.x_cstride % 8 != 0 || pt.x_cstride < rup(pt.c, 8)) return false;
        if (static_cast<long long>(c->n) * (c->h >> pt.x_up) * (c->w >> pt.x_up) * pt.x_cstride > lim) return false;
        if (pt.x && (reinterpret_cast<uintptr_t>(pt.x) & 15)) return false;
    }
    if (is_rowpack(c)) return c->cout >= 16;
    return c->cin >= 32 || c->cout >= 32;
}

struct Layout {
    int rowpack, ktap, cout64, rows_f, bn_f;
    long long kf, kd;
    int koff[TC_MAX_PARTS], kext[TC_MAX_PARTS];
};

Layout layout_of(const pcb_conv *c) {
    Layout L;
    memset(&L, 0, sizeof(L));
    L.rowpack = is_rowpack(c);
    const int taps = c->kh * c->kw;
    if (L.rowpack) {
        L.ktap = 64; L.koff[0] = 0; L.kext[0] = 64;
        L.kf = static_cast<long long>(c->kh) * 64;
    } else {
        int off = 0;
        for (int p = 0; p < c->nparts; ++p) { L.koff[p] = off; L.kext[p] = rup(c->parts[p].c, 64); off += L.kext[p]; }
        L.ktap = off;
        L.kf = static_cast<long long>(taps) * L.ktap;
    }
    L.cout64 = rup(c->cout, 64);
    L.bn_f = (c->cout % 128 == 0) ? 128 : 64;
    L.rows_f = rup(c->cout, L.bn_f);
    L.kd = static_cast<long long>(taps) * L.cout64;
    return L;
}

void fill_parts(const pcb_conv *c, const Layout &L, TcPart *out, const uint64_t *tapmask, long long m_total) {
    int off = 0;
    for (int p = 0; p < c->nparts; ++p) {
        out[p].x = static_cast<const bf16 *>(c->parts[p].x);
        out[p].tapmask = tapmask ? tapmask + static_cast<long long>(p) * m_total : nullptr;
        out[p].mask = c->parts[p].mask;
        out[p].dx = nullptr; out[p].dx_cstride = 0;
        out[p].c = c->parts[p].c;
        out[p].c8 = rup(c->parts[p].c, 8);
        out[p].kext = L.kext[p];
        out[p].koff = L.koff[p];
        out[p].choff = off;
        out[p].cstride = c->parts[p].x_cstride;
        out[p].xup = c->parts[p].x_up;
        out[p].mup = c->parts[p].mask_up;
        off += c->parts[p].c;
    }
}

int launch_tapmask(const pcb_conv *c, uint64_t *out, cudaStream_t st) {
    TapMaskParams T;
    memset(&T, 0, sizeof(T));
    T.n = c->n; T.h = c->h; T.w = c->w; T.kh = c->kh; T.kw = c->kw; T.stride = c->stride; T.pad_h = c->pad_h;
    T.pad_w = c->pad_w; T.dil = c->dil; T.ho = c->ho; T.wo = c->wo; T.m_total = c->n * c->ho * c->wo; T.nparts = c->nparts;
    for (int p = 0; p < c->nparts; ++p) { T.mask[p] = c->parts[p].mask; T.mup[p] = c->parts[p].mask_up; }
    T.out = out;
    tapmask_kernel<<<(T.m_total + 255) / 256, 256, 0, st>>>(T);
    PCB_LAUNCH_CHECK();
    return 0;
}

void set_ep(TcParams &P, const pcb_ep *ep) {
    if (ep == nullptr) return;
    P.ep_on = 1; P.ep_scale = ep->scale; P.ep_shift = ep->shift; P.ep_act = ep->act; P.ep_slope = ep->slope;
}

void base_params(TcParams &P, const pcb_conv *c, const Layout &L) {
    memset(&P, 0, sizeof(P));
    P.n = c->n; P.h = c->h; P.w = c->w; P.cin = c->cin; P.cout = c->cout; P.kh = c->kh; P.kw = c->kw; P.stride = c->stride;
    P.pad_h = c->pad_h; P.pad_w = c->pad_w; P.dil = c->dil; P.ho = c->ho; P.wo = c->wo;
    P.nparts = c->nparts; P.no_guard = c->no_guard; P.rowpack = L.rowpack; P.ktap = L.ktap;
    P.sub = 1; P.py = 0; P.px = 0; P.fh = c->h; P.fw = c->w;
    P.l2pf = getenv("PCB_TMA_L2_PREFETCH") != nullptr;
}

int halo_hg(const pcb_conv *c, bool rowpack) {
    if (rowpack || c->stride != 1 || getenv("PCB_DISABLE_HALO")) return 0;
    const int hg = 8 + (c->kw - 1) * c->dil;
    if (c->kw < 2 || hg > HALO_MAX_HG || c->kh > 8) return 0;
    if (c->wo % 8 != 0 || c->w % 8 != 0 || c->wo != c->w) return 0;
    return hg;
}

constexpr size_t MAX_SMEM = 227 * 1024;
constexpr size_t RING_BUDGET = 208 * 1024;

template <int BLOCK_N, int MODE, bool HALO>
int launch_persistent(TcParams &P, const CUtensorMap &tm, cudaStream_t st) {
    const size_t a_stage = HALO ? ((8 * 16 * (16 * P.hg + 1) + 127) / 128 * 128) : A_STAGE_BYTES;
    const size_t b_stage = BLOCK_N * 128;
    const size_t budget = RING_BUDGET - acc_stage_bytes(BLOCK_N);
    P.ring_b = 6;
    P.ring_a = HALO ? 3 : 6;
    while (P.ring_a * a_stage + P.ring_b * b_stage > budget && P.ring_b > 3) --P.ring_b;
    while (P.ring_a * a_stage + P.ring_b * b_stage > budget && P.ring_a > 2) --P.ring_a;
    const size_t smem = 1024 + P.ring_a * a_stage + P.ring_b * b_stage + 32 * MAX_RING + 16 + STAT_SMEM_BYTES + acc_stage_bytes(BLOCK_N);
    PCB_CHECK(smem <= MAX_SMEM, "tensor-core conv: %zu bytes of shared memory do not fit", smem);
    auto kern = pconv_tc_persistent_kernel<BLOCK_N, MODE, HALO>;
    PCB_SMEM_OPT_IN(kern, MAX_SMEM);
    const int num_tiles = ((P.m_total + BLOCK_M - 1) / BLOCK_M) * (P.ncols / BLOCK_N);
    const int grid = std::min(num_tiles, pcb_num_sms());
    kern<<<grid, PERSIST_THREADS, smem, st>>>(P, tm);
    PCB_LAUNCH_CHECK();
    return 0;
}


float *splitk_scratch(size_t bytes) {
    static float *buf[PCB_MAX_DEVICES] = {};
    static size_t cap[PCB_MAX_DEVICES] = {};
    const int dev = pcb_cur_device();
    if (bytes > cap[dev]) {
        const size_t want = std::max<size_t>(bytes, 16u << 20);
        float *fresh = nullptr;
        if (cudaMalloc(&fresh, want) != cudaSuccess) { cudaGetLastError(); return nullptr; }
        buf[dev] = fresh; cap[dev] = want;
    }
    return buf[dev];
}

__global__ void splitk_finish_fwd_kernel(const float *__restrict__ part, int ncols, const float *__restrict__ msum, const float *__restrict__ bias, int cout,
                                         int no_guard, long long m_total, bf16 *__restrict__ y, int y_cstride) {
    const int cv = y_cstride >> 3;
    const long long total = m_total * cv;
    for (long long i = blockIdx.x * static_cast<long long>(blockDim.x) + threadIdx.x; i < total; i += static_cast<long long>(gridDim.x) * blockDim.x) {
        const long long m = i / cv;
        const int col = static_cast<int>(i - m * cv) * 8;
        const float s = msum ? msum[m] : 1.f;
        const bool hole = (s == 0.f) && !no_guard;
        const float inv = hole ? 0.f : 1.0f / s;
        uint4 o;
        __nv_bfloat162 *ob = reinterpret_cast<__nv_bfloat162 *>(&o);
#pragma unroll
        for (int j = 0; j < 4; ++j) {
            const int co = col + 2 * j;
            float a = (co < ncols) ? part[m * ncols + co] : 0.f, b = (co + 1 < ncols) ? part[m * ncols + co + 1] : 0.f;
            a = (hole || co >= cout) ? 0.f : a * inv + (bias ? bias[co] : 0.f);
            b = (hole || co + 1 >= cout) ? 0.f : b * inv + (bias ? bias[co + 1] : 0.f);
            ob[j] = __floats2bfloat162_rn(a, b);
        }
        *reinterpret_cast<uint4 *>(y + m * y_cstride + col) = o;
    }
}

__global__ void splitk_finish_dgrad_kernel(const float *__restrict__ part, const TcParams P) {
    const int cv = P.ncols >> 3;
    const long long total = static_cast<long long>(P.m_total) * cv;
    for (long long i = blockIdx.x * static_cast<long long>(blockDim.x) + threadIdx.x; i < total; i += static_cast<long long>(gridDim.x) * blockDim.x) {
        const int m = static_cast<int>(i / cv);
        const int col = static_cast<int>(i - static_cast<long long>(m) * cv) * 8;
        const int en = m / (P.h * P.w), rem = m - en * P.h * P.w;
        const int eh = (rem / P.w) * P.sub + P.py, ew = (rem % P.w) * P.sub + P.px;
        const long long mo = (static_cast<long long>(en) * P.fh + eh) * P.fw + ew;
        for (int p = 0; p < P.nparts; ++p) {
            const TcPart &pt = P.parts[p];
            const int local = col - pt.koff;
            if (local < 0 || local >= pt.c8 || pt.dx == nullptr) continue;
            float scale = 1.f;
            if (pt.mask != nullptr)
                scale = pt.mask[(static_cast<long long>(en) * (P.fh >> pt.mup) + (eh >> pt.mup)) * (P.fw >> pt.mup) + (ew >> pt.mup)] ? 1.f : 0.f;
            const float *src = part + static_cast<long long>(m) * P.ncols + col;
            uint4 o;
            __nv_bfloat162 *ob = reinterpret_cast<__nv_bfloat162 *>(&o);
#pragma unroll
            for (int j = 0; j < 4; ++j) ob[j] = __floats2bfloat162_rn(src[2 * j] * scale, src[2 * j + 1] * scale);
            *reinterpret_cast<uint4 *>(pt.dx + mo * pt.dx_cstride + local) = o;
        }
    }
}

int pick_ksplit(long long m_total, int ncols, int bn, int blocks_per_tap) {
    if (!getenv("PCB_SPLITK")) return 1;
    const long long tiles = ((m_total + BLOCK_M - 1) / BLOCK_M) * (ncols / bn);
    const int sms = pcb_num_sms();
    if (tiles * 2 > sms) return 1;
    int ks = static_cast<int>(std::min<long long>(16, sms / tiles));
    ks = std::min(ks, blocks_per_tap);
    return ks < 2 ? 1 : ks;
}

bool tile_box(int wt, int ht, int *bw, int *bh, int *bn) {
    if (wt < 4) return false;
    if (wt % 128 == 0) { *bw = 128; *bh = 1; *bn = 1; return true; }
    if (128 % wt) return false;
    const int rows = 128 / wt;
    *bw = wt;
    if (ht % rows == 0) { *bh = rows; *bn = 1; return true; }
    if (rows % ht) return false;
    *bh = ht; *bn = rows / ht;
    return true;
}

bool tma_fwd_ok(const pcb_conv *c) {
    if (getenv("PCB_DISABLE_TMA") || is_rowpack(c)) return false;
    int bw, bh, bn;
    if (!tile_box(c->wo, c->ho, &bw, &bh, &bn)) return false;
    if (c->stride > 2 || bw * c->stride > 256 || bh * c->stride > 256) return false;
    for (int p = 0; p < c->nparts; ++p)
        if (c->parts[p].x_up && ((c->h | c->w) & 1)) return false;
    return true;
}

bool tma_dgrad_ok(const pcb_conv *c) {
    if (getenv("PCB_DISABLE_TMA") || is_rowpack(c) || c->stride != 1) return false;
    int bw, bh, bn;
    return tile_box(c->w, c->h, &bw, &bh, &bn);
}

bool tma_dgrad_s2_ok(const pcb_conv *c) {
    if (getenv("PCB_DISABLE_TMA") || getenv("PCB_DISABLE_TMA_S2") || is_rowpack(c)) return false;
    if (c->stride != 2 || c->dil != 1 || c->kh < 2 || c->kw < 2 || ((c->h | c->w) & 1) || c->ho != c->h / 2 || c->wo != c->w / 2) return false;
    int bw, bh, bn;
    return tile_box(c->w / 2, c->h / 2, &bw, &bh, &bn);
}

size_t up_bytes(const pcb_conv *c, int p) {
    return (static_cast<size_t>(c->n) * c->h * c->w * rup(c->parts[p].c, 8) * 2 + 255) / 256 * 256;
}
size_t tapmask_bytes(const pcb_conv *c) {
    return (static_cast<size_t>(c->nparts) * c->n * c->ho * c->wo * sizeof(uint64_t) + 255) / 256 * 256;
}

size_t tma_fixed_smem(int block_n, bool splitk) {
    return 1024 + TMA_BAR_BYTES + EPI_STAT_SMEM_BYTES + (splitk ? acc_stage_bytes(block_n) : bf16_stage_bytes(block_n));
}

template <int BLOCK_N, int MODE, bool HALO>
int launch_tma_n(TcParams &P, const CUtensorMap &tw, const CUtensorMap &ta0, const CUtensorMap &ta1, cudaStream_t st) {
    const int nb = HALO ? P.kw : 1;
    const size_t a_room = (static_cast<size_t>(BLOCK_M + (HALO ? (P.kw - 1) * P.dil : 0)) * 128 + 1023) / 1024 * 1024;
    const size_t stage = a_room + static_cast<size_t>(nb) * BLOCK_N * 128;
    PCB_CHECK(BLOCK_N <= 128 || P.partial == nullptr, "TMA-fed conv: split-K stages fp32 partials, at most 128 columns wide");
    const size_t fixed = tma_fixed_smem(BLOCK_N, P.partial != nullptr);
    P.stages = static_cast<int>(std::min<size_t>(MAX_RING, (MAX_SMEM - fixed) / stage));
    PCB_CHECK(P.stages >= 2, "TMA-fed conv: stage of %zu bytes does not fit twice", stage);
    const size_t smem = fixed + P.stages * stage;
    auto kern = pconv_tc_tma_kernel<BLOCK_N, MODE, HALO>;
    PCB_SMEM_OPT_IN(kern, MAX_SMEM);
    if (P.ksplit < 1) P.ksplit = 1;
    const int m_tiles = (P.m_total + BLOCK_M - 1) / BLOCK_M;
    const int num_tiles = m_tiles * (P.ncols / BLOCK_N) * P.ksplit;
    const int grid = std::min(num_tiles, pcb_num_sms());
    kern<<<grid, TMA_THREADS, smem, st>>>(P, tw, ta0, ta1);
    PCB_LAUNCH_CHECK();
    return 0;
}

template <int MODE>
int launch_tma(TcParams &P, const CUtensorMap &tw, const CUtensorMap &ta0, const CUtensorMap &ta1, int bn, bool halo, cudaStream_t st) {
    PCB_CHECK(!(halo && bn == 256), "TMA-fed conv: no 256-wide row-halo tiles");
    if (halo) {
        if (bn == 128) return launch_tma_n<128, MODE, true>(P, tw, ta0, ta1, st);
        if (bn == 64) return launch_tma_n<64, MODE, true>(P, tw, ta0, ta1, st);
        return launch_tma_n<32, MODE, true>(P, tw, ta0, ta1, st);
    }
    if (bn == 256) return launch_tma_n<256, MODE, false>(P, tw, ta0, ta1, st);
    if (bn == 128) return launch_tma_n<128, MODE, false>(P, tw, ta0, ta1, st);
    if (bn == 64) return launch_tma_n<64, MODE, false>(P, tw, ta0, ta1, st);
    return launch_tma_n<32, MODE, false>(P, tw, ta0, ta1, st);
}

bool halo_stages_fit(int kw, int dil, int block_n) {
    const size_t stage = (static_cast<size_t>(128 + (kw - 1) * dil) * 128 + 1023) / 1024 * 1024 + static_cast<size_t>(kw) * block_n * 128;
    return 3 * stage + acc_stage_bytes(block_n) <= RING_BUDGET;
}

bool tma_halo_ok(const pcb_conv *c, int bw, int bh, int bn, int block_n) {
    if (getenv("PCB_DISABLE_TMA_HALO")) return false;
    if (!(c->stride == 1 && bw == 128 && bh == 1 && bn == 1 && c->kw >= 2 && 128 + (c->kw - 1) * c->dil <= 256 && c->kh <= 8)) return false;
    return halo_stages_fit(c->kw, c->dil, block_n);
}

int pick_bn(int cols, long long m_total, bool fwd) {
    const long long m_tiles = (m_total + BLOCK_M - 1) / BLOCK_M;
    if (cols <= 32) return 32;
    const long long sms = pcb_num_sms();
    auto waves = [&](int b) { return (m_tiles * (cols / b) + sms - 1) / sms; };
    if (cols % 256 == 0 && 2 * waves(256) <= waves(128) && (!fwd || waves(256) == 1)) return 256;
    int bn = (cols % 128 == 0) ? 128 : 64;
    if (!getenv("PCB_NO_NARROW_N"))
        while (bn > 32 && cols % (bn / 2) == 0 && m_tiles * (cols / bn) < pcb_num_sms() / 2) bn /= 2;
    return bn;
}

template <int MODE>
int launch_tc(TcParams &P, const CUtensorMap &tm, int bn, cudaStream_t st) {
    if (P.hg) return (bn == 128) ? launch_persistent<128, MODE, true>(P, tm, st) : launch_persistent<64, MODE, true>(P, tm, st);
    return (bn == 128) ? launch_persistent<128, MODE, false>(P, tm, st) : launch_persistent<64, MODE, false>(P, tm, st);
}

}

static bool smallco_ok(const pcb_conv *c);
namespace {

struct SpAxis { int e0[2], ne[2], tapbits[2][4]; bool ok; };

int floordiv2(int v) { return v >= 0 ? v / 2 : -((-v + 1) / 2); }

SpAxis sp_axis(int k, int d, int p) {
    SpAxis A;
    memset(&A, 0, sizeof(A));
    A.ok = k <= 4;
    for (int q = 0; q < 2 && A.ok; ++q) {
        A.e0[q] = floordiv2(q - p);
        const int last = floordiv2(q + (k - 1) * d - p);
        A.ne[q] = last - A.e0[q] + 1;
        if (A.ne[q] < 1 || A.ne[q] > 4) { A.ok = false; break; }
        for (int t = 0; t < k; ++t) A.tapbits[q][floordiv2(q + t * d - p) - A.e0[q]] |= 1 << t;
        for (int e = 0; e < A.ne[q]; ++e)
            if (!A.tapbits[q][e]) A.ok = false;
    }
    return A;
}

struct SpPlan {
    bool ok;
    bool fwd, dgrad;
    int pu, ps;
    SpAxis ay, ax;
    int net[4], eoff[4], net_total;
    int kext_u, kext_s, c8_u, c8_s;
    long long kc[4], clsoff[4], sp_fwd_elems, sp_dg_elems, kd_sp;
    int bw, bh, bn;
};

SpPlan sp_plan(const pcb_conv *c) {
    SpPlan S;
    memset(&S, 0, sizeof(S));
    S.pu = S.ps = -1;
    if (getenv("PCB_DISABLE_SUBPIXEL") || getenv("PCB_DISABLE_TMA") || !common_ok(c) || is_rowpack(c)) return S;
    if (c->stride != 1 || c->ho != c->h || c->wo != c->w || ((c->h | c->w) & 1) || c->nparts > 2) return S;
    for (int p = 0; p < c->nparts; ++p) {
        if (c->parts[p].x_up) { if (S.pu >= 0) return S; S.pu = p; }
        else { if (S.ps >= 0) return S; S.ps = p; }
    }
    if (S.pu < 0) return S;
    if (c->parts[S.pu].mask && c->parts[S.pu].mask_up != 1) return S;
    if (S.ps >= 0 && c->parts[S.ps].mask && c->parts[S.ps].mask_up != 0) return S;
    if (smallco_ok(c)) return S;
    S.ay = sp_axis(c->kh, c->dil, c->pad_h);
    S.ax = sp_axis(c->kw, c->dil, c->pad_w);
    if (!S.ay.ok || !S.ax.ok) return S;
    if (!tile_box(c->w / 2, c->h / 2, &S.bw, &S.bh, &S.bn)) return S;
    const Layout L = layout_of(c);
    S.kext_u = L.kext[S.pu]; S.c8_u = rup(c->parts[S.pu].c, 8);
    S.kext_s = S.ps >= 0 ? L.kext[S.ps] : 0; S.c8_s = S.ps >= 0 ? rup(c->parts[S.ps].c, 8) : 0;
    const int taps = c->kh * c->kw;
    long long off = 0;
    int eo = 0;
    for (int cls = 0; cls < 4; ++cls) {
        S.net[cls] = S.ay.ne[cls >> 1] * S.ax.ne[cls & 1];
        S.eoff[cls] = eo; eo += S.net[cls];
        S.kc[cls] = static_cast<long long>(S.net[cls]) * S.kext_u + static_cast<long long>(S.ps >= 0 ? taps : 0) * S.kext_s;
        S.clsoff[cls] = off; off += static_cast<long long>(L.rows_f) * S.kc[cls];
        if (S.net[cls] + (S.ps >= 0 ? taps : 0) > SP_MAX_ITEMS) return S;
    }
    S.net_total = eo;
    if (S.net_total > SP_MAX_ITEMS) return S;
    S.kd_sp = static_cast<long long>(S.net_total) * L.cout64;
    S.ok = true;
    const long long src_tiles = (static_cast<long long>(c->n) * (c->h / 2) * (c->w / 2) + BLOCK_M - 1) / BLOCK_M;
    S.dgrad = src_tiles >= pcb_num_sms() / 3 || getenv("PCB_SUBPIXEL_ALL") != nullptr;
    S.fwd = getenv("PCB_SUBPIXEL_FWD") != nullptr || getenv("PCB_SUBPIXEL_ALL") != nullptr;
    S.sp_fwd_elems = S.fwd ? off : 0;
    S.sp_dg_elems = S.dgrad ? static_cast<long long>(rup(S.kext_u, 128)) * S.kd_sp : 0;
    if (!S.fwd && !S.dgrad) S.ok = false;
    return S;
}

struct SpWParams {
    int cout, taps, cin, kw, cout64, rows_f;
    int choff_u, c_u, kext_u, choff_s, c_s, kext_s, has_skip;
    int net[4], eoff[4], nex[4], slot0[4];
    int ybits[2][4], xbits[2][4];
    long long kc[4], clsoff[4], kd_sp;
    int want_fwd, want_dg;
};

__global__ void sp_weight_prepare_kernel(const float *__restrict__ wm, const SpWParams W, bf16 *__restrict__ w_f, bf16 *__restrict__ w_d) {
    const int co = blockIdx.x;
    int slot = blockIdx.y, cls = 0;
    while (cls < 3 && slot >= W.slot0[cls + 1]) ++cls;
    slot -= W.slot0[cls];
    const float *wrow = wm + static_cast<long long>(co) * W.taps * W.cin;
    if (slot < W.net[cls]) {
        const int ey = slot / W.nex[cls], ex = slot - ey * W.nex[cls];
        const int yb = W.ybits[cls >> 1][ey], xb = W.xbits[cls & 1][ex];
        for (int ci = threadIdx.x; ci < W.c_u; ci += blockDim.x) {
            float v = 0.f;
            for (int tr = 0; tr < 4; ++tr)
                if ((yb >> tr) & 1)
                    for (int tc = 0; tc < 4; ++tc)
                        if ((xb >> tc) & 1) v += wrow[static_cast<long long>(tr * W.kw + tc) * W.cin + W.choff_u + ci];
            const bf16 b = __float2bfloat16_rn(v);
            if (W.want_fwd) w_f[W.clsoff[cls] + static_cast<long long>(co) * W.kc[cls] + static_cast<long long>(slot) * W.kext_u + ci] = b;
            if (W.want_dg) w_d[static_cast<long long>(ci) * W.kd_sp + static_cast<long long>(W.eoff[cls] + slot) * W.cout64 + co] = b;
        }
    } else if (W.has_skip && W.want_fwd) {
        const int tap = slot - W.net[cls];
        for (int ci = threadIdx.x; ci < W.c_s; ci += blockDim.x)
            w_f[W.clsoff[cls] + static_cast<long long>(co) * W.kc[cls] + static_cast<long long>(W.net[cls]) * W.kext_u + static_cast<long long>(tap) * W.kext_s + ci] =
                __float2bfloat16_rn(wrow[static_cast<long long>(tap) * W.cin + W.choff_s + ci]);
    }
}

__global__ void sp_weight_dg_kernel(const float *__restrict__ wm, const SpWParams W, bf16 *__restrict__ w_d) {
    const int ci = blockIdx.x;
    int slot = blockIdx.y, cls = 0;
    while (cls < 3 && slot >= W.eoff[cls + 1]) ++cls;
    slot -= W.eoff[cls];
    const int ey = slot / W.nex[cls], ex = slot - ey * W.nex[cls];
    const int yb = W.ybits[cls >> 1][ey], xb = W.xbits[cls & 1][ex];
    for (int co = threadIdx.x; co < W.cout; co += blockDim.x) {
        const float *wrow = wm + static_cast<long long>(co) * W.taps * W.cin + W.choff_u + ci;
        float v = 0.f;
        for (int tr = 0; tr < 4; ++tr)
            if ((yb >> tr) & 1)
                for (int tc = 0; tc < 4; ++tc)
                    if ((xb >> tc) & 1) v += wrow[static_cast<long long>(tr * W.kw + tc) * W.cin];
        w_d[static_cast<long long>(ci) * W.kd_sp + static_cast<long long>(W.eoff[cls] + slot) * W.cout64 + co] = __float2bfloat16_rn(v);
    }
}

int sp_weight_prepare(const pcb_conv *c, const SpPlan &S, const Layout &L, const float *w_master, bf16 *w_f, bf16 *w_d, cudaStream_t st) {
    SpWParams W;
    memset(&W, 0, sizeof(W));
    W.cout = c->cout; W.taps = c->kh * c->kw; W.cin = c->cin; W.kw = c->kw; W.cout64 = L.cout64; W.rows_f = L.rows_f;
    int off = 0;
    for (int p = 0; p < c->nparts; ++p) {
        if (p == S.pu) { W.choff_u = off; W.c_u = c->parts[p].c; }
        if (p == S.ps) { W.choff_s = off; W.c_s = c->parts[p].c; }
        off += c->parts[p].c;
    }
    W.kext_u = S.kext_u; W.kext_s = S.kext_s; W.has_skip = S.ps >= 0; W.kd_sp = S.kd_sp;
    W.want_fwd = S.fwd; W.want_dg = S.dgrad;
    int slot = 0;
    for (int cls = 0; cls < 4; ++cls) {
        W.net[cls] = S.net[cls]; W.eoff[cls] = S.eoff[cls]; W.nex[cls] = S.ax.ne[cls & 1]; W.slot0[cls] = slot;
        slot += S.net[cls] + (S.ps >= 0 ? W.taps : 0);
        W.kc[cls] = S.kc[cls]; W.clsoff[cls] = S.clsoff[cls];
    }
    for (int q = 0; q < 2; ++q)
        for (int e = 0; e < 4; ++e) { W.ybits[q][e] = S.ay.tapbits[q][e]; W.xbits[q][e] = S.ax.tapbits[q][e]; }
    if (S.fwd) {
        sp_weight_prepare_kernel<<<dim3(c->cout, slot), 128, 0, st>>>(w_master, W, w_f, w_d);
        PCB_LAUNCH_CHECK();
    } else if (S.dgrad) {
        sp_weight_dg_kernel<<<dim3(W.c_u, S.net_total), 128, 0, st>>>(w_master, W, w_d);
        PCB_LAUNCH_CHECK();
    }
    return 0;
}

int sp_bn(int cols, long long m_total) { return std::min(pick_bn(cols, m_total, true), 64); }

template <int BLOCK_N, int MODE>
int launch_sp_n(TcParams &P, const SpTable &TB, const CUtensorMap &tw, const CUtensorMap &ta0, const CUtensorMap &ta1, cudaStream_t st) {
    int nb_max = 1;
    for (int i = 0; i < TB.n_items; ++i) nb_max = std::max(nb_max, TB.it[i].nb);
    const size_t a_room = (static_cast<size_t>(TB.rows_max) * 128 + 1023) / 1024 * 1024;
    const size_t stage = a_room + static_cast<size_t>(nb_max) * BLOCK_N * 128;
    const size_t fixed = tma_fixed_smem(BLOCK_N, false);
    P.stages = static_cast<int>(std::min<size_t>(MAX_RING, (MAX_SMEM - fixed) / stage));
    PCB_CHECK(P.stages >= 2, "sub-pixel conv: stage of %zu bytes does not fit twice", stage);
    const size_t smem = fixed + P.stages * stage;
    auto kern = pconv_tc_sp_kernel<BLOCK_N, MODE>;
    PCB_SMEM_OPT_IN(kern, MAX_SMEM);
    const int num_tiles = ((P.m_total + BLOCK_M - 1) / BLOCK_M) * (P.ncols / BLOCK_N);
    const int grid = std::min(num_tiles, pcb_num_sms());
    kern<<<grid, TMA_THREADS, smem, st>>>(P, TB, tw, ta0, ta1);
    PCB_LAUNCH_CHECK();
    return 0;
}

template <int MODE>
int launch_sp(TcParams &P, const SpTable &TB, const CUtensorMap &tw, const CUtensorMap &ta0, const CUtensorMap &ta1, int bn, cudaStream_t st) {
    if (bn == 64) return launch_sp_n<64, MODE>(P, TB, tw, ta0, ta1, st);
    return launch_sp_n<32, MODE>(P, TB, tw, ta0, ta1, st);
}

struct ClassStreams4 { cudaStream_t aux[3]; cudaEvent_t ev_fork, ev_join[3]; bool ready; };
int class_streams(ClassStreams4 **out) {
    static thread_local ClassStreams4 cs_all[PCB_MAX_DEVICES] = {};
    ClassStreams4 &CS = cs_all[pcb_cur_device()];
    if (!CS.ready) {
        for (int i = 0; i < 3; ++i) {
            PCB_CUDA(cudaStreamCreateWithFlags(&CS.aux[i], cudaStreamNonBlocking));
            PCB_CUDA(cudaEventCreateWithFlags(&CS.ev_join[i], cudaEventDisableTiming));
        }
        PCB_CUDA(cudaEventCreateWithFlags(&CS.ev_fork, cudaEventDisableTiming));
        CS.ready = true;
    }
    *out = &CS;
    return 0;
}

int sp_forward(const pcb_conv *c, const SpPlan &S, const Layout &L, const bf16 *w_sp, const float *bias, void *y, int y_cstride, const float *msum,
               double *bn_sums, const pcb_ep *ep, int *flag, cudaStream_t st) {
    const int hc = c->h / 2, wc = c->w / 2;
    const long long m_class = static_cast<long long>(c->n) * hc * wc;
    TcParams P;
    base_params(P, c, L);
    fill_parts(c, L, P.parts, nullptr, 0);
    P.ho = hc; P.wo = wc; P.m_total = static_cast<int>(m_class);
    P.sub = 2; P.fh = c->ho; P.fw = c->wo;
    P.bias = bias; P.msum = msum; P.y = static_cast<bf16 *>(y); P.y_cstride = y_cstride; P.abort_flag = flag;
    P.bn_sums = bn_sums; P.bn_c = c->cout;
    set_ep(P, ep);
    P.box_w = S.bw; P.box_h = S.bh; P.box_n = S.bn;
    const int cols = (c->cout <= 32) ? 32 : L.rows_f;
    const int bn = sp_bn(cols, m_class);
    P.ncols = cols;
    for (int p = 0; p < c->nparts; ++p)
        if (c->parts[p].mask) P.use_fix = 1;
    const bool row_tiles = S.bw == 128 && S.bh == 1 && S.bn == 1;
    const int taps = c->kh * c->kw;
    const long long class_tiles = ((m_class + BLOCK_M - 1) / BLOCK_M) * (cols / bn);
    const bool fork = class_tiles < pcb_num_sms() && !getenv("PCB_DISABLE_CLASS_STREAMS");
    ClassStreams4 *CS = nullptr;
    if (fork) {
        if (int rc = class_streams(&CS)) return rc;
        PCB_CUDA(cudaEventRecord(CS->ev_fork, st));
    }
    for (int cls = 0; cls < 4; ++cls) {
        const int py = cls >> 1, px = cls & 1;
        const int ney = S.ay.ne[py], nex = S.ax.ne[px], ey0 = S.ay.e0[py], ex0 = S.ax.e0[px];
        SpTable TB;
        memset(&TB, 0, sizeof(TB));
        const int pu = S.pu, ps = S.ps;
        TB.step[pu] = 1; TB.es[pu] = 1; TB.ph[pu] = hc; TB.pw[pu] = wc;
        const bool halo_u = row_tiles && nex > 1 && !getenv("PCB_DISABLE_TMA_HALO");
        TB.arows[pu] = BLOCK_M + (halo_u ? nex - 1 : 0);
        int ni = 0;
        for (int e = 0; e < ney; ++e) {
            if (halo_u) {
                SpItem &it = TB.it[ni++];
                it.part = pu; it.dx = ex0; it.dy = ey0 + e; it.nb = nex; it.wk = (e * nex) * S.kext_u; it.wk_step = S.kext_u; it.shift0 = 0; it.dshift = 8;
            } else {
                for (int f = 0; f < nex; ++f) {
                    SpItem &it = TB.it[ni++];
                    it.part = pu; it.dx = ex0 + f; it.dy = ey0 + e; it.nb = 1; it.wk = (e * nex + f) * S.kext_u; it.wk_step = 0; it.shift0 = 0; it.dshift = 0;
                }
            }
        }
        if (ps >= 0) {
            TB.step[ps] = 2; TB.es[ps] = 2; TB.ph[ps] = c->h; TB.pw[ps] = c->w;
            TB.arows[ps] = BLOCK_M;
            for (int tr = 0; tr < c->kh; ++tr)
                for (int tc = 0; tc < c->kw; ++tc) {
                    SpItem &it = TB.it[ni++];
                    it.part = ps; it.dx = px + tc * c->dil - c->pad_w; it.dy = py + tr * c->dil - c->pad_h; it.nb = 1;
                    it.wk = S.net[cls] * S.kext_u + (tr * c->kw + tc) * S.kext_s; it.wk_step = 0; it.shift0 = 0; it.dshift = 0;
                }
        }
        TB.n_items = ni;
        TB.rows_max = std::max(TB.arows[pu], ps >= 0 ? TB.arows[ps] : 0);
        PCB_CHECK(ni <= SP_MAX_ITEMS, "sub-pixel conv: too many items");
        CUtensorMap ta[TC_MAX_PARTS], tw;
        memset(ta, 0, sizeof(ta));
        if (int rc = make_tmap_nhwc(&ta[pu], c->parts[pu].x, S.c8_u, wc, hc, c->n, c->parts[pu].x_cstride, S.bw + (halo_u ? nex - 1 : 0), S.bh, S.bn, 1)) return rc;
        if (ps >= 0) {
            if (int rc = make_tmap_nhwc(&ta[ps], c->parts[ps].x, S.c8_s, c->w, c->h, c->n, c->parts[ps].x_cstride, S.bw, S.bh, S.bn, 2)) return rc;
        } else ta[1 - pu] = ta[pu];
        if (int rc = make_tmap_2d(&tw, w_sp + S.clsoff[cls], L.rows_f, S.kc[cls], S.kc[cls], bn)) return rc;
        TcParams Q = P;
        Q.py = py; Q.px = px;
        cudaStream_t cs = (fork && cls > 0) ? CS->aux[cls - 1] : st;
        if (fork && cls > 0) PCB_CUDA(cudaStreamWaitEvent(cs, CS->ev_fork, 0));
        if (int rc = launch_sp<0>(Q, TB, tw, ta[0], ta[1], bn, cs)) return rc;
        if (fork && cls > 0) {
            PCB_CUDA(cudaEventRecord(CS->ev_join[cls - 1], cs));
            PCB_CUDA(cudaStreamWaitEvent(st, CS->ev_join[cls - 1], 0));
        }
    }
    return 0;
}

int sp_dgrad_up(const pcb_conv *c, const SpPlan &S, const Layout &L, const void *dc, int dc_cstride, const bf16 *w_sp_dg, void *dx_u, int dx_cstride,
                int *flag, cudaStream_t st) {
    const int hs = c->h / 2, ws = c->w / 2;
    const long long m_src = static_cast<long long>(c->n) * hs * ws;
    TcParams P;
    base_params(P, c, L);
    P.h = hs; P.w = ws; P.m_total = static_cast<int>(m_src);
    P.sub = 1; P.py = 0; P.px = 0; P.fh = hs; P.fw = ws;
    P.nparts = 1;
    memset(P.parts, 0, sizeof(P.parts));
    TcPart &pt = P.parts[0];
    pt.c = c->parts[S.pu].c; pt.c8 = S.c8_u; pt.kext = S.kext_u; pt.koff = 0; pt.mask = c->parts[S.pu].mask; pt.mup = 0;
    pt.dx = static_cast<bf16 *>(dx_u); pt.dx_cstride = dx_cstride;
    PCB_CHECK(dx_cstride % 8 == 0 && dx_cstride >= S.c8_u && (reinterpret_cast<uintptr_t>(dx_u) & 15) == 0, "sub-pixel dgrad: dx must be 16-byte aligned with a channel stride that is a multiple of 8");
    P.dc = static_cast<const bf16 *>(dc); P.dc_cstride = dc_cstride; P.dc_c8 = rup(c->cout, 8); P.dc_kext = L.cout64;
    P.abort_flag = flag;
    P.ncols = S.kext_u;
    P.box_w = S.bw; P.box_h = S.bh; P.box_n = S.bn;
    const int bn = sp_bn(S.kext_u, m_src);
    SpTable TB;
    memset(&TB, 0, sizeof(TB));
    TB.step[0] = 2; TB.es[0] = 2; TB.ph[0] = c->ho; TB.pw[0] = c->wo; TB.arows[0] = BLOCK_M; TB.rows_max = BLOCK_M;
    int ni = 0;
    for (int cls = 0; cls < 4; ++cls) {
        const int py = cls >> 1, px = cls & 1;
        const int ney = S.ay.ne[py], nex = S.ax.ne[px];
        for (int e = 0; e < ney; ++e)
            for (int f = 0; f < nex; ++f) {
                SpItem &it = TB.it[ni++];
                it.part = 0; it.dx = px - 2 * (S.ax.e0[px] + f); it.dy = py - 2 * (S.ay.e0[py] + e); it.nb = 1;
                it.wk = (S.eoff[cls] + e * nex + f) * L.cout64; it.wk_step = 0; it.shift0 = 0; it.dshift = 0;
            }
    }
    TB.n_items = ni;
    CUtensorMap ta, tw;
    if (int rc = make_tmap_nhwc(&ta, dc, P.dc_c8, c->wo, c->ho, c->n, dc_cstride, S.bw, S.bh, S.bn, 2)) return rc;
    if (int rc = make_tmap_2d(&tw, w_sp_dg, rup(S.kext_u, 128), S.kd_sp, S.kd_sp, bn)) return rc;
    return launch_sp<1>(P, TB, tw, ta, ta, bn, st);
}

}

static bool smallco_ok(const pcb_conv *c) { return common_ok(c) && !is_rowpack(c) && pcb_smallco_eligible(c); }
static pcb_smallco_layout smallco_layout(const Layout &L) {
    pcb_smallco_layout S;
    S.ktap = L.ktap; S.koff[0] = L.koff[0]; S.koff[1] = L.koff[1]; S.cout64 = L.cout64; S.kf = L.kf; S.kd = L.kd;
    return S;
}

bool pcb_tc_eligible(const pcb_conv *c) { return common_ok(c) && !getenv("PCB_DISABLE_TC"); }

static bool tma_wgrad_ok(const pcb_conv *c);

static void k2r_bases(const Layout &L, size_t *fe, size_t *de) {
    *fe = (static_cast<size_t>(L.rows_f) * L.kf + 63) / 64 * 64;
    *de = (static_cast<size_t>(rup(L.ktap, 128)) * L.kd + 63) / 64 * 64;
}

static bool stem_ok(const pcb_conv *c) { return common_ok(c) && is_rowpack(c) && pcb_stem_ok(c); }
static size_t stem_base(const Layout &L) { return (static_cast<size_t>(L.rows_f) * L.kf + 63) / 64 * 64; }

size_t pcb_tc_workspace(const pcb_conv *c) {
    if (smallco_ok(c) && pcb_k2r_ok(c)) return pcb_k2r_workspace(c);
    if (stem_ok(c)) return std::max(pcb_stem_workspace(c), tapmask_bytes(c));
    size_t bytes = tapmask_bytes(c);
    if (tma_fwd_ok(c) || tma_wgrad_ok(c))
        for (int p = 0; p < c->nparts; ++p)
            if (c->parts[p].x_up) bytes += up_bytes(c, p);
    return bytes;
}

void pcb_tc_weight_layout(const pcb_conv *c, size_t *fwd_elems, size_t *dgrad_elems) {
    const Layout L = layout_of(c);
    *fwd_elems = static_cast<size_t>(L.rows_f) * L.kf;
    *dgrad_elems = L.rowpack ? 0 : static_cast<size_t>(rup(L.ktap, 128)) * L.kd;
    const SpPlan S = sp_plan(c);
    if (S.ok) { *fwd_elems += static_cast<size_t>(S.sp_fwd_elems); *dgrad_elems += static_cast<size_t>(S.sp_dg_elems); }
    if (smallco_ok(c) && pcb_k2r_ok(c)) {
        size_t fb, db, fx, dx;
        k2r_bases(L, &fb, &db);
        pcb_k2r_weight_layout(c, &fx, &dx);
        *fwd_elems = fb + fx; *dgrad_elems = db + dx;
    }
    if (stem_ok(c)) *fwd_elems = stem_base(L) + pcb_stem_weight_extra(c);
}

bool pcb_tc_subpixel(const pcb_conv *c) {
    if (smallco_ok(c)) return pcb_k2r_ok(c);
    const SpPlan S = sp_plan(c);
    return S.ok && S.dgrad;
}

int pcb_tc_weight_prepare(const pcb_conv *c, const float *w_master, void *w_fwd, void *w_dgrad, bool zero_padding, cudaStream_t st) {
    const Layout L = layout_of(c);
    size_t fe, de;
    pcb_tc_weight_layout(c, &fe, &de);
    if (zero_padding) {
        PCB_CUDA(cudaMemsetAsync(w_fwd, 0, fe * 2, st));
        if (w_dgrad && de) PCB_CUDA(cudaMemsetAsync(w_dgrad, 0, de * 2, st));
    }
    WPrepParams W;
    memset(&W, 0, sizeof(W));
    W.cout = c->cout; W.taps = c->kh * c->kw; W.cin = c->cin; W.kw = c->kw; W.rowpack = L.rowpack; W.nparts = c->nparts;
    W.ktap = L.ktap; W.cout64 = L.cout64; W.kf = L.kf; W.kd = L.kd;
    int off = 0;
    for (int p = 0; p < c->nparts; ++p) { W.choff[p] = off; W.c[p] = c->parts[p].c; W.koff[p] = L.koff[p]; off += c->parts[p].c; }
    if (!L.rowpack && W.taps <= 65535 && c->cout >= 32 && c->cin >= 32) {
        dim3 tg((c->cin + 31) / 32, (c->cout + 31) / 32, W.taps);
        tc_weight_prepare_tiled_kernel<<<tg, 256, 0, st>>>(w_master, W, static_cast<bf16 *>(w_fwd), (w_dgrad && de) ? static_cast<bf16 *>(w_dgrad) : nullptr);
        PCB_LAUNCH_CHECK();
        const SpPlan S = sp_plan(c);
        if (S.ok) {
            PCB_CHECK(w_dgrad != nullptr, "sub-pixel weights need the dgrad operand buffer");
            return sp_weight_prepare(c, S, L, w_master, static_cast<bf16 *>(w_fwd) + static_cast<size_t>(L.rows_f) * L.kf,
                                     static_cast<bf16 *>(w_dgrad) + static_cast<size_t>(rup(L.ktap, 128)) * L.kd, st);
        }
        return 0;
    }
    const long long total = static_cast<long long>(c->cout) * W.taps * c->cin;
    const int grid = static_cast<int>(std::min<long long>((total + 1023) / 1024, 8ll * pcb_num_sms()));
    tc_weight_prepare_kernel<<<grid < 1 ? 1 : grid, 256, 0, st>>>(w_master, W, static_cast<bf16 *>(w_fwd),
                                                                   (w_dgrad && de) ? static_cast<bf16 *>(w_dgrad) : nullptr);
    PCB_LAUNCH_CHECK();
    if (stem_ok(c)) return pcb_stem_weight_prepare(c, w_master, static_cast<bf16 *>(w_fwd) + stem_base(L), zero_padding, st);
    if (smallco_ok(c) && pcb_k2r_ok(c)) {
        PCB_CHECK(w_dgrad != nullptr, "kernel-to-row weights need the dgrad operand buffer");
        size_t fb, db;
        k2r_bases(L, &fb, &db);
        return pcb_k2r_weight_prepare(c, w_master, static_cast<bf16 *>(w_fwd) + fb, static_cast<bf16 *>(w_dgrad) + db, zero_padding, st);
    }
    const SpPlan S = sp_plan(c);
    if (S.ok) {
        PCB_CHECK(w_dgrad != nullptr, "sub-pixel weights need the dgrad operand buffer");
        return sp_weight_prepare(c, S, L, w_master, static_cast<bf16 *>(w_fwd) + static_cast<size_t>(L.rows_f) * L.kf,
                                 static_cast<bf16 *>(w_dgrad) + static_cast<size_t>(rup(L.ktap, 128)) * L.kd, st);
    }
    return 0;
}

int pcb_tc_forward_mask_pass(const pcb_conv *c, uint64_t *tapmask, cudaStream_t st) {
    const long long m_total = static_cast<long long>(c->n) * c->ho * c->wo;
    PCB_CHECK(m_total < (1ll << 31), "problem too large");
    const Layout L = layout_of(c);
    if (smallco_ok(c) || stem_ok(c)) return 0;
    { const SpPlan S = sp_plan(c); if (S.ok && S.fwd) return 0; }
    bool any_mask = false;
    for (int p = 0; p < c->nparts; ++p) any_mask = any_mask || (c->parts[p].mask != nullptr);
    if (tma_fwd_ok(c) && !any_mask) return 0;
    if (tma_fwd_ok(c)) {
        int bw, bh, bn;
        tile_box(c->wo, c->ho, &bw, &bh, &bn);
        if (tma_halo_ok(c, bw, bh, bn, pick_bn(c->cout <= 32 ? 32 : L.rows_f, m_total, true))) return 0;
    }
    return launch_tapmask(c, tapmask, st);
}

bool pcb_tc_fuses_bn_stats(const pcb_conv *c) {
    return pcb_tc_fuses_affine_act(c) && !getenv("PCB_DISABLE_FUSED_BN_STATS");
}

bool pcb_tc_fuses_affine_act(const pcb_conv *c) {
    return pcb_tc_eligible(c) && !smallco_ok(c) && !getenv("PCB_SPLITK");
}

int pcb_tc_forward_ws(const pcb_conv *c, const void *w_fwd, const float *bias, void *y, int y_cstride, const float *msum,
                      uint64_t *tapmask, bool mask_pass_done, double *bn_sums, const pcb_ep *ep, cudaStream_t st) {
    int *flag = abort_flag_ptr();
    PCB_CHECK(flag != nullptr, "cudaMalloc(abort flag) failed");
    const long long m_total = static_cast<long long>(c->n) * c->ho * c->wo;
    PCB_CHECK(m_total < (1ll << 31), "problem too large");
    PCB_CHECK(y_cstride % 8 == 0 && y_cstride >= c->cout, "tensor-core forward: y channel stride must be a multiple of 8 and >= cout");
    const Layout L = layout_of(c);
    if (!mask_pass_done)
        if (int rc = pcb_tc_forward_mask_pass(c, tapmask, st)) return rc;
    if (stem_ok(c)) {
        PCB_CHECK(bn_sums == nullptr || pcb_tc_fuses_bn_stats(c), "fused BatchNorm statistics requested from a kernel that does not produce them");
        PCB_CHECK(ep == nullptr || pcb_tc_fuses_affine_act(c), "fused BatchNorm + activation requested from a kernel that does not apply it");
        return pcb_stem_forward(c, static_cast<const bf16 *>(w_fwd) + stem_base(L), bias, y, y_cstride, msum, tapmask, bn_sums, ep, st);
    }
    if (smallco_ok(c)) {
        PCB_CHECK(ep == nullptr, "fused BatchNorm + activation requested from a small-Cout kernel that does not apply it");
        if (pcb_k2r_ok(c)) {
            size_t fb, db;
            k2r_bases(L, &fb, &db);
            return pcb_k2r_forward(c, smallco_layout(L), w_fwd, static_cast<const bf16 *>(w_fwd) + fb, bias, y, y_cstride, msum, tapmask, st);
        }
        return pcb_smallco_forward(c, smallco_layout(L), w_fwd, bias, y, y_cstride, msum, st);
    }
    {
        const SpPlan S = sp_plan(c);
        if (S.ok && S.fwd) {
            PCB_CHECK(bn_sums == nullptr || pcb_tc_fuses_bn_stats(c), "fused BatchNorm statistics requested from a kernel that does not produce them");
            return sp_forward(c, S, L, static_cast<const bf16 *>(w_fwd) + static_cast<size_t>(L.rows_f) * L.kf, bias, y, y_cstride, msum, bn_sums, ep, flag, st);
        }
    }
    TcParams P;
    base_params(P, c, L);
    P.m_total = static_cast<int>(m_total);
    fill_parts(c, L, P.parts, tapmask, m_total);
    P.bias = bias; P.msum = msum; P.y = static_cast<bf16 *>(y); P.y_cstride = y_cstride; P.abort_flag = flag;
    PCB_CHECK(bn_sums == nullptr || pcb_tc_fuses_bn_stats(c), "fused BatchNorm statistics requested from a kernel that does not produce them");
    P.bn_sums = bn_sums; P.bn_c = c->cout;
    PCB_CHECK(ep == nullptr || pcb_tc_fuses_affine_act(c), "fused BatchNorm + activation requested from a kernel that does not apply it");
    set_ep(P, ep);
    P.ncols = L.rows_f;
    CUtensorMap tm;
    if (tma_fwd_ok(c)) {
        tile_box(c->wo, c->ho, &P.box_w, &P.box_h, &P.box_n);
        const int bn = pick_bn(c->cout <= 32 ? 32 : L.rows_f, m_total, true);
        const bool halo = tma_halo_ok(c, P.box_w, P.box_h, P.box_n, bn);
        const int hx = halo ? (c->kw - 1) * c->dil : 0;
        CUtensorMap ta[TC_MAX_PARTS];
        memset(ta, 0, sizeof(ta));
        uint8_t *extra = reinterpret_cast<uint8_t *>(tapmask) + tapmask_bytes(c);
        for (int p = 0; p < c->nparts; ++p) {
            const pcb_part &pt = c->parts[p];
            const void *src = pt.x;
            long long cs = pt.x_cstride;
            const int c8 = rup(pt.c, 8);
            if (pt.x_up) {
                const long long pix = static_cast<long long>(c->n) * (c->h >> 1) * (c->w >> 1);
                const long long work = pix * (c8 >> 3);
                const int grid = static_cast<int>(std::min<long long>((work + 255) / 256, 16ll * pcb_num_sms()));
                upsample_part_kernel<<<grid, 256, 0, st>>>(static_cast<const bf16 *>(pt.x), pt.x_cstride, c8, pix, c->h >> 1, c->w >> 1, reinterpret_cast<bf16 *>(extra));
                PCB_LAUNCH_CHECK();
                src = extra; cs = c8;
                extra += up_bytes(c, p);
            }
            if (pt.mask) P.use_fix = 1;
            if (int rc = make_tmap_nhwc(&ta[p], src, c8, c->w, c->h, c->n, cs, P.box_w + hx, P.box_h, P.box_n, c->stride)) return rc;
        }
        if (c->nparts < 2) ta[1] = ta[0];
        P.ncols = (c->cout <= 32) ? 32 : L.rows_f;
        P.wk_base = 0; P.wk_col = L.ktap; P.wk_row = c->kw * L.ktap;
        if (int rc = make_tmap_2d(&tm, w_fwd, L.rows_f, L.kf, L.kf, bn)) return rc;
        P.ksplit = pick_ksplit(m_total, P.ncols, bn, L.ktap / BLOCK_K);
        if (P.ksplit > 1) {
            PCB_CHECK(!P.ep_on, "split-K forward: the finish kernel does not apply a fused BatchNorm + activation");
            const size_t bytes = static_cast<size_t>(m_total) * P.ncols * sizeof(float);
            P.partial = splitk_scratch(bytes);
            PCB_CHECK(P.partial != nullptr, "split-K scratch allocation failed");
            PCB_CUDA(cudaMemsetAsync(P.partial, 0, bytes, st));
            if (int rc = launch_tma<0>(P, tm, ta[0], ta[1], bn, halo, st)) return rc;
            const long long work = m_total * (y_cstride / 8);
            splitk_finish_fwd_kernel<<<static_cast<int>(std::min<long long>((work + 255) / 256, 8ll * pcb_num_sms())), 256, 0, st>>>(
                P.partial, P.ncols, msum, bias, c->cout, c->no_guard, m_total, static_cast<bf16 *>(y), y_cstride);
            PCB_LAUNCH_CHECK();
            return 0;
        }
        return launch_tma<0>(P, tm, ta[0], ta[1], bn, halo, st);
    }
    if (int rc = make_tmap_2d(&tm, w_fwd, L.rows_f, L.kf, L.kf, L.bn_f)) return rc;
    P.hg = halo_hg(c, L.rowpack);
    return launch_tc<0>(P, tm, L.bn_f, st);
}

bool pcb_tc_dgrad_supported(const pcb_conv *c) { return pcb_tc_eligible(c) && !is_rowpack(c); }

int pcb_tc_dgrad(const pcb_conv *c, const void *dc, int dc_cstride, const void *w_dgrad, void *const *dx, const int *dx_cstride,
                 cudaStream_t st) {
    int *flag = abort_flag_ptr();
    PCB_CHECK(flag != nullptr, "cudaMalloc(abort flag) failed");
    const long long m_total = static_cast<long long>(c->n) * c->h * c->w;
    PCB_CHECK(m_total < (1ll << 31), "problem too large");
    PCB_CHECK(dc_cstride % 8 == 0 && dc_cstride >= rup(c->cout, 8), "tensor-core dgrad: dc channel stride must be a multiple of 8");
    const Layout L = layout_of(c);
    if (smallco_ok(c)) {
        if (pcb_k2r_ok(c)) {
            size_t fb, db;
            k2r_bases(L, &fb, &db);
            return pcb_k2r_dgrad(c, smallco_layout(L), dc, dc_cstride, w_dgrad, static_cast<const bf16 *>(w_dgrad) + db, dx, dx_cstride, st);
        }
        return pcb_smallco_dgrad(c, smallco_layout(L), dc, dc_cstride, w_dgrad, dx, dx_cstride, st);
    }
    const SpPlan SPL = sp_plan(c);
    void *dx_local[TC_MAX_PARTS] = {nullptr, nullptr};
    for (int p = 0; p < c->nparts && p < TC_MAX_PARTS; ++p) dx_local[p] = dx[p];
    if (SPL.ok && SPL.dgrad) {
        if (dx[SPL.pu] != nullptr)
            if (int rc = sp_dgrad_up(c, SPL, L, dc, dc_cstride, static_cast<const bf16 *>(w_dgrad) + static_cast<size_t>(rup(L.ktap, 128)) * L.kd,
                                     dx[SPL.pu], dx_cstride[SPL.pu], flag, st)) return rc;
        dx_local[SPL.pu] = nullptr;
        if (SPL.ps < 0 || dx[SPL.ps] == nullptr) return 0;
    }
    dx = dx_local;
    TcParams P;
    base_params(P, c, L);
    P.m_total = static_cast<int>(m_total);
    fill_parts(c, L, P.parts, nullptr, 0);
    for (int p = 0; p < c->nparts; ++p) {
        P.parts[p].dx = static_cast<bf16 *>(dx[p]);
        P.parts[p].dx_cstride = dx_cstride[p];
        PCB_CHECK(!dx[p] || (dx_cstride[p] % 8 == 0 && dx_cstride[p] >= P.parts[p].c8 && (reinterpret_cast<uintptr_t>(dx[p]) & 15) == 0),
                  "tensor-core dgrad: dx[%d] must be 16-byte aligned with a channel stride that is a multiple of 8", p);
    }
    P.dc = static_cast<const bf16 *>(dc); P.dc_cstride = dc_cstride; P.dc_c8 = rup(c->cout, 8); P.dc_kext = L.cout64;
    P.abort_flag = flag;
    int bn = (L.ktap % 128 == 0) ? 128 : 64;
    P.ncols = L.ktap;
    CUtensorMap tm;
    if (tma_dgrad_ok(c)) {
        tile_box(c->w, c->h, &P.box_w, &P.box_h, &P.box_n);
        bn = pick_bn(L.ktap, m_total, false);
        const bool halo = tma_halo_ok(c, P.box_w, P.box_h, P.box_n, bn);
        P.wk_base = 0; P.wk_col = L.cout64; P.wk_row = c->kw * L.cout64;
        CUtensorMap ta;
        if (int rc = make_tmap_nhwc(&ta, dc, P.dc_c8, c->wo, c->ho, c->n, dc_cstride, P.box_w + (halo ? (c->kw - 1) * c->dil : 0), P.box_h, P.box_n, 1)) return rc;
        if (int rc = make_tmap_2d(&tm, w_dgrad, rup(L.ktap, 128), L.kd, L.kd, bn)) return rc;
        P.ksplit = pick_ksplit(m_total, P.ncols, bn, L.cout64 / BLOCK_K);
        if (P.ksplit > 1) {
            const size_t bytes = static_cast<size_t>(m_total) * P.ncols * sizeof(float);
            P.partial = splitk_scratch(bytes);
            PCB_CHECK(P.partial != nullptr, "split-K scratch allocation failed");
            PCB_CUDA(cudaMemsetAsync(P.partial, 0, bytes, st));
            if (int rc = launch_tma<1>(P, tm, ta, ta, bn, halo, st)) return rc;
            const long long work = m_total * (P.ncols / 8);
            splitk_finish_dgrad_kernel<<<static_cast<int>(std::min<long long>((work + 255) / 256, 8ll * pcb_num_sms())), 256, 0, st>>>(P.partial, P);
            PCB_LAUNCH_CHECK();
            return 0;
        }
        return launch_tma<1>(P, tm, ta, ta, bn, halo, st);
    }
    if (tma_dgrad_s2_ok(c)) {
        const int hh = c->h / 2, hw = c->w / 2;
        const long long m_class = static_cast<long long>(c->n) * hh * hw;
        tile_box(hw, hh, &P.box_w, &P.box_h, &P.box_n);
        bn = pick_bn(L.ktap, m_class, false);
        if (int rc = make_tmap_2d(&tm, w_dgrad, rup(L.ktap, 128), L.kd, L.kd, bn)) return rc;
        const long long class_tiles = ((m_class + BLOCK_M - 1) / BLOCK_M) * (L.ktap / bn);
        const bool fork = class_tiles < pcb_num_sms() && !getenv("PCB_DISABLE_CLASS_STREAMS");
        struct ClassStreams { cudaStream_t aux[3]; cudaEvent_t ev_fork, ev_join[3]; bool ready; };
        static thread_local ClassStreams cs_all[PCB_MAX_DEVICES] = {};
        ClassStreams &CS = cs_all[pcb_cur_device()];
        cudaStream_t *aux = CS.aux;
        cudaEvent_t *ev_join = CS.ev_join;
        if (fork && !CS.ready) {
            for (int i = 0; i < 3; ++i) {
                PCB_CUDA(cudaStreamCreateWithFlags(&aux[i], cudaStreamNonBlocking));
                PCB_CUDA(cudaEventCreateWithFlags(&ev_join[i], cudaEventDisableTiming));
            }
            PCB_CUDA(cudaEventCreateWithFlags(&CS.ev_fork, cudaEventDisableTiming));
            CS.ready = true;
        }
        cudaEvent_t ev_fork = CS.ev_fork;
        if (fork) PCB_CUDA(cudaEventRecord(ev_fork, st));
        for (int cls = 0; cls < 4; ++cls) {
            TcParams Q = P;
            const int py = cls >> 1, px = cls & 1;
            const int tr0 = (py + c->pad_h) & 1, tc0 = (px + c->pad_w) & 1;
            Q.kh = (c->kh - tr0 + 1) / 2; Q.kw = (c->kw - tc0 + 1) / 2;
            Q.pad_h = (py + c->pad_h - tr0) / 2; Q.pad_w = (px + c->pad_w - tc0) / 2;
            Q.h = hh; Q.w = hw; Q.stride = 1; Q.dil = 1;
            Q.m_total = static_cast<int>(m_class);
            Q.sub = 2; Q.py = py; Q.px = px; Q.fh = c->h; Q.fw = c->w;
            Q.wk_base = (tr0 * c->kw + tc0) * L.cout64; Q.wk_row = 2 * c->kw * L.cout64; Q.wk_col = 2 * L.cout64;
            const bool halo = !getenv("PCB_DISABLE_TMA_HALO") && Q.box_w == 128 && Q.box_h == 1 && Q.box_n == 1 && Q.kw >= 2 &&
                              halo_stages_fit(Q.kw, 1, bn);
            CUtensorMap ta;
            if (int rc = make_tmap_nhwc(&ta, dc, P.dc_c8, c->wo, c->ho, c->n, dc_cstride, Q.box_w + (halo ? Q.kw - 1 : 0), Q.box_h, Q.box_n, 1)) return rc;
            cudaStream_t cs = (fork && cls > 0) ? aux[cls - 1] : st;
            if (fork && cls > 0) PCB_CUDA(cudaStreamWaitEvent(cs, ev_fork, 0));
            if (int rc = launch_tma<1>(Q, tm, ta, ta, bn, halo, cs)) return rc;
            if (fork && cls > 0) {
                PCB_CUDA(cudaEventRecord(ev_join[cls - 1], cs));
                PCB_CUDA(cudaStreamWaitEvent(st, ev_join[cls - 1], 0));
            }
        }
        return 0;
    }
    if (int rc = make_tmap_2d(&tm, w_dgrad, rup(L.ktap, 128), L.kd, L.kd, bn)) return rc;
    P.hg = halo_hg(c, L.rowpack);
    return launch_tc<1>(P, tm, bn, st);
}


static bool kblock_box(int wt, int ht, int *bw, int *bh, int *bn) {
    if (wt < 4) return false;
    if (wt % 64 == 0) { *bw = 64; *bh = 1; *bn = 1; return true; }
    if (64 % wt) return false;
    const int rows = 64 / wt;
    *bw = wt;
    if (ht % rows == 0) { *bh = rows; *bn = 1; return true; }
    if (rows % ht) return false;
    *bh = ht; *bn = rows / ht;
    return true;
}

static bool tma_wgrad_ok(const pcb_conv *c) {
    if (getenv("PCB_DISABLE_TMA") || getenv("PCB_DISABLE_TMA_WGRAD") || is_rowpack(c) || c->stride > 2) return false;
    int bw, bh, bn;
    if (!kblock_box(c->wo, c->ho, &bw, &bh, &bn)) return false;
    for (int p = 0; p < c->nparts; ++p)
        if (c->parts[p].x_up && ((c->h | c->w) & 1)) return false;
    return true;
}

template <int BLOCK_N, int T, bool HALO>
int launch_wgrad_tma(WgParams &P, const CUtensorMap &tdc, const CUtensorMap &ta0, const CUtensorMap &ta1, cudaStream_t st) {
    const int rows_a = 64 + (HALO ? (P.kw - 1) * P.dil : 0);
    PCB_CHECK(rows_a <= (HALO ? 3 : 1) * WGRAD_FIX_THREADS, "TMA-fed wgrad: %d-row A blocks exceed the fixer warps", rows_a);
    const size_t a_blk = (static_cast<size_t>(rows_a) * 128 + 1023) / 1024 * 1024;
    const size_t stage = (HALO ? 1 : T) * 2 * a_blk + static_cast<size_t>(BLOCK_N) * 128;
    P.stages = static_cast<int>(std::min<size_t>(MAX_RING, RING_BUDGET / stage));
    PCB_CHECK(P.stages >= 2, "TMA-fed wgrad: stage of %zu bytes does not fit twice", stage);
    const size_t smem = 1024 + P.stages * stage + 24 * MAX_RING;
    auto kern = pconv_tc_wgrad_tma_kernel<BLOCK_N, T, HALO>;
    PCB_SMEM_OPT_IN(kern, MAX_SMEM);
    P.tap_groups = HALO ? P.kh : (P.kh * P.kw + T - 1) / T;
    P.ci_tiles = (P.ktap + 127) / 128;
    const int co_tiles = (P.cout + BLOCK_N - 1) / BLOCK_N;
    const int base_ctas = co_tiles * P.tap_groups * P.ci_tiles;
    const int total_kb = (P.m_total + 63) / 64;
    int splits = (2 * pcb_num_sms() + base_ctas - 1) / base_ctas;
    splits = std::max(1, std::min(splits, total_kb));
    splits = std::min(splits, 65535);
    P.kb_per_split = (total_kb + splits - 1) / splits;
    splits = (total_kb + P.kb_per_split - 1) / P.kb_per_split;
    dim3 grid(base_ctas, splits);
    kern<<<grid, WGRAD_TMA_THREADS, smem, st>>>(P, tdc, ta0, ta1);
    PCB_LAUNCH_CHECK();
    return 0;
}

template <int BLOCK_N, int T, int STAGES>
static int launch_wgrad(WgParams &P, const CUtensorMap &tm, int cout, cudaStream_t st) {
    constexpr size_t smem = 1024 + STAGES * (T * 16384 + BLOCK_N * 128) + 24 * STAGES;
    auto kern = pconv_tc_wgrad_kernel<BLOCK_N, T, STAGES>;
    PCB_SMEM_OPT_IN(kern, (int)smem);
    P.tap_groups = (P.ntaps + T - 1) / T;
    P.ci_tiles = (P.ktap + 127) / 128;
    const int co_tiles = (cout + BLOCK_N - 1) / BLOCK_N;
    const int base_ctas = co_tiles * P.tap_groups * P.ci_tiles;
    const int total_kb = (P.m_total + 63) / 64;
    int splits = (4 * pcb_num_sms() + base_ctas - 1) / base_ctas;
    splits = std::max(1, std::min(splits, total_kb));
    splits = std::min(splits, 65535);
    P.kb_per_split = (total_kb + splits - 1) / splits;
    splits = (total_kb + P.kb_per_split - 1) / P.kb_per_split;
    dim3 grid(base_ctas, splits);
    kern<<<grid, WGRAD_THREADS, smem, st>>>(P, tm);
    PCB_LAUNCH_CHECK();
    return 0;
}

int pcb_tc_wgrad(const pcb_conv *c, const void *dc, int dc_cstride, float *dw, void *workspace, bool zero_dw, cudaStream_t st) {
    int *flag = abort_flag_ptr();
    PCB_CHECK(flag != nullptr, "cudaMalloc(abort flag) failed");
    PCB_CHECK(workspace != nullptr, "pcb_tc_wgrad: workspace required");
    const long long m_total = static_cast<long long>(c->n) * c->ho * c->wo;
    PCB_CHECK(m_total < (1ll << 31), "problem too large");
    PCB_CHECK(dc_cstride % 8 == 0 && dc_cstride >= c->cout, "tensor-core wgrad: dc channel stride must be a multiple of 8");
    if (stem_ok(c)) return pcb_stem_wgrad(c, dc, dc_cstride, dw, workspace, zero_dw, st);
    if (smallco_ok(c)) {
        if (pcb_k2r_ok(c)) return pcb_k2r_wgrad(c, dc, dc_cstride, dw, workspace, zero_dw, st);
        return pcb_smallco_wgrad(c, smallco_layout(layout_of(c)), dc, dc_cstride, dw, zero_dw, st);
    }
    uint64_t *tapmask = static_cast<uint64_t *>(workspace);
    bool any_mask = false;
    for (int p = 0; p < c->nparts; ++p) any_mask = any_mask || (c->parts[p].mask != nullptr);
    if (any_mask || !tma_wgrad_ok(c))
        if (int rc = launch_tapmask(c, tapmask, st)) return rc;
    const size_t dw_bytes = sizeof(float) * c->cout * c->kh * c->kw * c->cin;
    if (zero_dw) PCB_CUDA(cudaMemsetAsync(dw, 0, dw_bytes, st));
    const Layout L = layout_of(c);
    WgParams P;
    memset(&P, 0, sizeof(P));
    P.n = c->n; P.h = c->h; P.w = c->w; P.cin = c->cin; P.cout = c->cout; P.kh = c->kh; P.kw = c->kw; P.stride = c->stride;
    P.pad_h = c->pad_h; P.pad_w = c->pad_w; P.dil = c->dil; P.ho = c->ho; P.wo = c->wo; P.m_total = static_cast<int>(m_total);
    P.nparts = c->nparts; P.rowpack = L.rowpack; P.ktap = L.ktap; P.ntaps = L.rowpack ? c->kh : c->kh * c->kw;
    fill_parts(c, L, P.parts, tapmask, m_total);
    P.dw = dw; P.abort_flag = flag;
    CUtensorMap tm;
    if (int rc = make_tmap_2d(&tm, dc, m_total, c->cout, dc_cstride, 64)) return rc;
    if (tma_wgrad_ok(c)) {
        kblock_box(c->wo, c->ho, &P.box_w, &P.box_h, &P.box_n);
        const bool halo = !getenv("PCB_DISABLE_TMA_HALO") && c->stride == 1 && c->kw == 3 && P.box_w == 64 &&
                          P.box_h == 1 && P.box_n == 1 && 64 + (c->kw - 1) * c->dil <= 256;
        const int hx = halo ? (c->kw - 1) * c->dil : 0;
        CUtensorMap ta[TC_MAX_PARTS];
        memset(ta, 0, sizeof(ta));
        uint8_t *extra = reinterpret_cast<uint8_t *>(workspace) + tapmask_bytes(c);
        for (int p = 0; p < c->nparts; ++p) {
            const pcb_part &pt = c->parts[p];
            const void *src = pt.x;
            long long cs = pt.x_cstride;
            const int c8 = rup(pt.c, 8);
            if (pt.x_up) {
                const long long pix = static_cast<long long>(c->n) * (c->h >> 1) * (c->w >> 1);
                const long long work = pix * (c8 >> 3);
                const int grid = static_cast<int>(std::min<long long>((work + 255) / 256, 16ll * pcb_num_sms()));
                upsample_part_kernel<<<grid, 256, 0, st>>>(static_cast<const bf16 *>(pt.x), pt.x_cstride, c8, pix, c->h >> 1, c->w >> 1, reinterpret_cast<bf16 *>(extra));
                PCB_LAUNCH_CHECK();
                src = extra; cs = c8;
                extra += up_bytes(c, p);
            }
            if (pt.mask) P.use_fix = 1;
            if (int rc = make_tmap_nhwc(&ta[p], src, c8, c->w, c->h, c->n, cs, P.box_w + hx, P.box_h, P.box_n, c->stride)) return rc;
        }
        if (c->nparts < 2) ta[1] = ta[0];
        if (c->cout > 64 && m_total >= 128 * 64) {
            if (halo) return launch_wgrad_tma<128, 3, true>(P, tm, ta[0], ta[1], st);
            return launch_wgrad_tma<128, 3, false>(P, tm, ta[0], ta[1], st);
        }
        if (halo) return launch_wgrad_tma<64, 3, true>(P, tm, ta[0], ta[1], st);
        return launch_wgrad_tma<64, 3, false>(P, tm, ta[0], ta[1], st);
    }
    return launch_wgrad<64, 3, 3>(P, tm, c->cout, st);
}

int pcb_tc_read_abort_flag(int *value) {
    int *flag = abort_flag_ptr();
    PCB_CHECK(flag != nullptr, "no abort flag");
    PCB_CUDA(cudaMemcpy(value, flag, sizeof(int), cudaMemcpyDeviceToHost));
    if (*value != 0) cudaMemset(flag, 0, sizeof(int));
    return 0;
}
```

text_segmentation_image_inpainting_b200/csrc/pcb_common.cuh:

```cuda
#pragma once
#include <cuda_bf16.h>
#include <cuda_runtime.h>
#include <stdint.h>
#include <stdio.h>

#include "../../include/pconv_b200.h"

int pcb_set_error(const char *fmt, ...);
void pcb_count_launch(int n = 1);

#define PCB_CHECK(cond, ...)                       \
    do {                                           \
        if (!(cond)) return pcb_set_error(__VA_ARGS__); \
    } while (0)

#define PCB_CUDA(expr)                                                                           \
    do {                                                                                         \
        cudaError_t _e = (expr);                                                                 \
        if (_e != cudaSuccess)                                                                   \
            return pcb_set_error("%s:%d: %s -> %s", __FILE__, __LINE__, #expr, cudaGetErrorString(_e)); \
    } while (0)

#define PCB_LAUNCH_CHECK()                                                                        \
    do {                                                                                         \
        cudaError_t _e = cudaGetLastError();                                                     \
        if (_e != cudaSuccess)                                                                   \
            return pcb_set_error("%s:%d: kernel launch -> %s", __FILE__, __LINE__, cudaGetErrorString(_e)); \
        pcb_count_launch();                                                                      \
    } while (0)

constexpr int PCB_MAX_DEVICES = 64;

static inline int pcb_cur_device() {
    int dev = 0;
    cudaGetDevice(&dev);
    return (dev >= 0 && dev < PCB_MAX_DEVICES) ? dev : 0;
}

static inline int pcb_num_sms() {
    static int sms[PCB_MAX_DEVICES] = {0};
    const int dev = pcb_cur_device();
    if (!sms[dev]) {
        int v = 0;
        cudaDeviceGetAttribute(&v, cudaDevAttrMultiProcessorCount, dev);
        sms[dev] = v > 0 ? v : 132;
    }
    return sms[dev];
}

#define PCB_SMEM_OPT_IN(kern, bytes)                                                                          \
    do {                                                                                                      \
        static bool pcb_done_[PCB_MAX_DEVICES] = {};                                                          \
        const int pcb_dev_ = pcb_cur_device();                                                                \
        if (!pcb_done_[pcb_dev_]) {                                                                           \
            PCB_CUDA(cudaFuncSetAttribute(kern, cudaFuncAttributeMaxDynamicSharedMemorySize, (int)(bytes))); \
            pcb_done_[pcb_dev_] = true;                                                                       \
        }                                                                                                     \
    } while (0)

static inline size_t pcb_dtype_size(int dtype) { return dtype == PCB_BF16 ? 2 : 4; }

typedef __nv_bfloat16 bf16;

template <typename T> __device__ __forceinline__ float to_f32(T v);
template <> __device__ __forceinline__ float to_f32<float>(float v) { return v; }
template <> __device__ __forceinline__ float to_f32<bf16>(bf16 v) { return __bfloat162float(v); }

template <typename T> __device__ __forceinline__ T from_f32(float v);
template <> __device__ __forceinline__ float from_f32<float>(float v) { return v; }
template <> __device__ __forceinline__ bf16 from_f32<bf16>(float v) { return __float2bfloat16_rn(v); }

__device__ __forceinline__ float apply_act(float z, int act, float slope) {
    if (act == PCB_ACT_RELU) return z > 0.f ? z : 0.f;
    if (act == PCB_ACT_LEAKY) return z > 0.f ? z : z * slope;
    if (act == PCB_ACT_RELU6) return fminf(fmaxf(z, 0.f), 6.f);
    return z;
}
__device__ __forceinline__ float act_grad(float z, int act, float slope) {
    if (act == PCB_ACT_RELU) return z > 0.f ? 1.f : 0.f;
    if (act == PCB_ACT_LEAKY) return z > 0.f ? 1.f : slope;
    if (act == PCB_ACT_RELU6) return (z > 0.f && z < 6.f) ? 1.f : 0.f;
    return 1.f;
}

template <typename T> struct Vec8;
template <> struct Vec8<bf16> {
    static __device__ __forceinline__ void load(const bf16 *p, float (&v)[8]) {
        uint4 r = *reinterpret_cast<const uint4 *>(p);
        const __nv_bfloat162 *h = reinterpret_cast<const __nv_bfloat162 *>(&r);
#pragma unroll
        for (int i = 0; i < 4; ++i) {
            float2 f = __bfloat1622float2(h[i]);
            v[2 * i] = f.x;
            v[2 * i + 1] = f.y;
        }
    }
    static __device__ __forceinline__ void store(bf16 *p, const float (&v)[8]) {
        uint4 r;
        __nv_bfloat162 *h = reinterpret_cast<__nv_bfloat162 *>(&r);
#pragma unroll
        for (int i = 0; i < 4; ++i) h[i] = __floats2bfloat162_rn(v[2 * i], v[2 * i + 1]);
        *reinterpret_cast<uint4 *>(p) = r;
    }
};
template <> struct Vec8<float> {
    static __device__ __forceinline__ void load(const float *p, float (&v)[8]) {
        float4 a = reinterpret_cast<const float4 *>(p)[0], b = reinterpret_cast<const float4 *>(p)[1];
        v[0] = a.x; v[1] = a.y; v[2] = a.z; v[3] = a.w; v[4] = b.x; v[5] = b.y; v[6] = b.z; v[7] = b.w;
    }
    static __device__ __forceinline__ void store(float *p, const float (&v)[8]) {
        reinterpret_cast<float4 *>(p)[0] = make_float4(v[0], v[1], v[2], v[3]);
        reinterpret_cast<float4 *>(p)[1] = make_float4(v[4], v[5], v[6], v[7]);
    }
};

__device__ __forceinline__ float warp_sum(float v) {
#pragma unroll
    for (int o = 16; o > 0; o >>= 1) v += __shfl_xor_sync(0xffffffffu, v, o);
    return v;
}

struct pcb_ep { const float *scale, *shift; int act; float slope; };

int pcb_generic_forward(const pcb_conv *c, const void *w, const float *bias, void *y, int y_cstride, const float *msum, cudaStream_t st);
int pcb_generic_dgrad(const pcb_conv *c, const void *dc, int dc_cstride, const void *w_krsc, void *const *dx, const int *dx_cstride,
                      cudaStream_t st);
int pcb_generic_wgrad(const pcb_conv *c, const void *dc, int dc_cstride, float *dw, bool zero_dw, cudaStream_t st);
int pcb_mask_sums(const pcb_conv *c, float *msum, uint8_t *newmask, cudaStream_t st);
bool pcb_tc_eligible(const pcb_conv *c);
bool pcb_tc_dgrad_supported(const pcb_conv *c);
size_t pcb_tc_workspace(const pcb_conv *c);
void pcb_tc_weight_layout(const pcb_conv *c, size_t *fwd_elems, size_t *dgrad_elems);
int pcb_tc_weight_prepare(const pcb_conv *c, const float *w_master, void *w_fwd, void *w_dgrad, bool zero_padding, cudaStream_t st);
int pcb_tc_forward_mask_pass(const pcb_conv *c, uint64_t *tapmask, cudaStream_t st);
int pcb_tc_forward_ws(const pcb_conv *c, const void *w_fwd, const float *bias, void *y, int y_cstride, const float *msum,
                      uint64_t *tapmask, bool mask_pass_done, double *bn_sums, const pcb_ep *ep, cudaStream_t st);
bool pcb_tc_fuses_bn_stats(const pcb_conv *c);
bool pcb_tc_fuses_affine_act(const pcb_conv *c);
bool pcb_tc_subpixel(const pcb_conv *c);
int pcb_tc_dgrad(const pcb_conv *c, const void *dc, int dc_cstride, const void *w_dgrad, void *const *dx, const int *dx_cstride,
                 cudaStream_t st);
int pcb_tc_wgrad(const pcb_conv *c, const void *dc, int dc_cstride, float *dw, void *workspace, bool zero_dw, cudaStream_t st);
int pcb_tc_read_abort_flag(int *value);
struct pcb_smallco_layout { int ktap, koff[2], cout64; long long kf, kd; };
bool pcb_smallco_eligible(const pcb_conv *c);
int pcb_smallco_forward(const pcb_conv *c, const pcb_smallco_layout &L, const void *w_fwd, const float *bias, void *y, int y_cstride, const float *msum,
                        cudaStream_t st);
int pcb_smallco_dgrad(const pcb_conv *c, const pcb_smallco_layout &L, const void *dc, int dc_cstride, const void *w_dgrad, void *const *dx, const int *dx_cstride,
                      cudaStream_t st);
int pcb_smallco_wgrad(const pcb_conv *c, const pcb_smallco_layout &L, const void *dc, int dc_cstride, float *dw, bool zero_dw, cudaStream_t st);
bool pcb_k2r_ok(const pcb_conv *c);
void pcb_k2r_weight_layout(const pcb_conv *c, size_t *fwd_extra, size_t *dg_extra);
size_t pcb_k2r_workspace(const pcb_conv *c);
int pcb_k2r_weight_prepare(const pcb_conv *c, const float *w_master, void *w_fwd_extra, void *w_dg_extra, bool zero_padding, cudaStream_t st);
int pcb_k2r_forward(const pcb_conv *c, const pcb_smallco_layout &L, const void *w_fwd, const void *w_fwd_extra, const float *bias, void *y, int y_cstride,
                    const float *msum, void *workspace, cudaStream_t st);
int pcb_k2r_dgrad(const pcb_conv *c, const pcb_smallco_layout &L, const void *dc, int dc_cstride, const void *w_dgrad, const void *w_dg_extra,
                  void *const *dx, const int *dx_cstride, cudaStream_t st);
int pcb_k2r_wgrad(const pcb_conv *c, const void *dc, int dc_cstride, float *dw, void *workspace, bool zero_dw, cudaStream_t st);
bool pcb_stem_ok(const pcb_conv *c);
size_t pcb_stem_weight_extra(const pcb_conv *c);
size_t pcb_stem_workspace(const pcb_conv *c);
int pcb_stem_weight_prepare(const pcb_conv *c, const float *w_master, void *w_fwd_extra, bool zero_padding, cudaStream_t st);
int pcb_stem_forward(const pcb_conv *c, const void *w_fwd_extra, const float *bias, void *y, int y_cstride, const float *msum, void *workspace,
                     double *bn_sums, const pcb_ep *ep, cudaStream_t st);
int pcb_stem_wgrad(const pcb_conv *c, const void *dc, int dc_cstride, float *dw, void *workspace, bool zero_dw, cudaStream_t st);
bool pcb_dw_eligible(const pcb_conv *c);
int pcb_dw_weight_prepare(const pcb_conv *c, const float *w_master, void *w_t, cudaStream_t st);
int pcb_dw_forward(const pcb_conv *c, const void *w_t, const float *bias, void *y, int y_cstride, const float *msum, double *bn_sums,
                   const pcb_ep *ep, cudaStream_t st);
bool pcb_dw_fuses_bn_stats(const pcb_conv *c);
bool pcb_dw_fuses_affine_act(const pcb_conv *c);
int pcb_dw_dgrad(const pcb_conv *c, const void *dc, int dc_cstride, const void *w_t, void *dx, int dx_cstride, cudaStream_t st);
int pcb_dw_wgrad(const pcb_conv *c, const void *dc, int dc_cstride, float *dw, bool zero_dw, cudaStream_t st);
```

text_segmentation_image_inpainting_b200/csrc/pcb_ptx.cuh:

```cuda
#pragma once
#include <cuda.h>
#include <cuda_runtime.h>
#include <stdint.h>

namespace ptx {

__device__ __forceinline__ uint32_t smem_u32(const void *p) { return static_cast<uint32_t>(__cvta_generic_to_shared(p)); }

__device__ __forceinline__ bool elect_one() {
    uint32_t pred = 0;
    asm volatile(
        "{\n\t.reg .pred P;\n\telect.sync _|P, 0xffffffff;\n\tselp.b32 %0, 1, 0, P;\n\t}" : "=r"(pred));
    return pred != 0;
}

__device__ __forceinline__ void mbar_init(uint32_t bar, uint32_t count) {
    asm volatile("mbarrier.init.shared::cta.b64 [%0], %1;" ::"r"(bar), "r"(count) : "memory");
}
__device__ __forceinline__ void fence_mbar_init() { asm volatile("fence.mbarrier_init.release.cluster;" ::: "memory"); }
__device__ __forceinline__ void mbar_arrive(uint32_t bar) {
    asm volatile("mbarrier.arrive.shared::cta.b64 _, [%0];" ::"r"(bar) : "memory");
}
__device__ __forceinline__ void mbar_arrive_expect_tx(uint32_t bar, uint32_t bytes) {
    asm volatile("mbarrier.arrive.expect_tx.shared::cta.b64 _, [%0], %1;" ::"r"(bar), "r"(bytes) : "memory");
}
__device__ __forceinline__ bool mbar_try_wait(uint32_t bar, uint32_t parity) {
    uint32_t ok;
    asm volatile(
        "{\n\t.reg .pred P;\n\t"
        "mbarrier.try_wait.parity.shared::cta.b64 P, [%1], %2;\n\t"
        "selp.b32 %0, 1, 0, P;\n\t}"
        : "=r"(ok)
        : "r"(bar), "r"(parity)
        : "memory");
    return ok != 0;
}
__device__ __forceinline__ bool mbar_wait(uint32_t bar, uint32_t parity, int *abort_flag, int code) {
    if (mbar_try_wait(bar, parity)) return true;
    const long long t0 = clock64();
    for (uint32_t it = 1;; ++it) {
        if (mbar_try_wait(bar, parity)) return true;
        if ((it & 63) == 0) {
            if (*reinterpret_cast<volatile int *>(abort_flag) != 0) return false;
            if (clock64() - t0 > 4000000000ll) break;
        }
    }
    atomicCAS(abort_flag, 0, code);
    return false;
}
__device__ __forceinline__ void cp_async_mbar_arrive(uint32_t bar) {
    asm volatile("cp.async.mbarrier.arrive.shared::cta.b64 [%0];" ::"r"(bar) : "memory");
}

__device__ __forceinline__ void cp_async_16(uint32_t dst, const void *src, bool valid) {
    const uint32_t sz = valid ? 16u : 0u;
    asm volatile("cp.async.cg.shared.global [%0], [%1], 16, %2;" ::"r"(dst), "l"(src), "r"(sz) : "memory");
}
__device__ __forceinline__ void cp_async_commit() { asm volatile("cp.async.commit_group;" ::: "memory"); }
template <int N> __device__ __forceinline__ void cp_async_wait() { asm volatile("cp.async.wait_group %0;" ::"n"(N) : "memory"); }

__device__ __forceinline__ void fence_proxy_async_smem() { asm volatile("fence.proxy.async.shared::cta;" ::: "memory"); }

__device__ __forceinline__ void prefetch_tmap(const CUtensorMap *m) {
    asm volatile("prefetch.tensormap [%0];" ::"l"(reinterpret_cast<uint64_t>(m)) : "memory");
}
__device__ __forceinline__ void tma_load_2d(uint32_t dst, const CUtensorMap *m, int c0, int c1, uint32_t bar) {
    asm volatile(
        "cp.async.bulk.tensor.2d.shared::cluster.global.mbarrier::complete_tx::bytes [%0], [%1, {%3, %4}], [%2];"
        ::"r"(dst), "l"(reinterpret_cast<uint64_t>(m)), "r"(bar), "r"(c0), "r"(c1)
        : "memory");
}
__device__ __forceinline__ void tma_prefetch_4d(const CUtensorMap *m, int c0, int c1, int c2, int c3) {
    asm volatile("cp.async.bulk.prefetch.tensor.4d.L2.global.tile [%0, {%1, %2, %3, %4}];"
                 ::"l"(reinterpret_cast<uint64_t>(m)), "r"(c0), "r"(c1), "r"(c2), "r"(c3)
                 : "memory");
}
__device__ __forceinline__ void tma_load_4d(uint32_t dst, const CUtensorMap *m, int c0, int c1, int c2, int c3, uint32_t bar) {
    asm volatile(
        "cp.async.bulk.tensor.4d.shared::cluster.global.mbarrier::complete_tx::bytes [%0], [%1, {%3, %4, %5, %6}], [%2];"
        ::"r"(dst), "l"(reinterpret_cast<uint64_t>(m)), "r"(bar), "r"(c0), "r"(c1), "r"(c2), "r"(c3)
        : "memory");
}

__device__ __forceinline__ void wgmma_fence() { asm volatile("wgmma.fence.sync.aligned;" ::: "memory"); }
__device__ __forceinline__ void wgmma_commit() { asm volatile("wgmma.commit_group.sync.aligned;" ::: "memory"); }
template <int N> __device__ __forceinline__ void wgmma_wait() { asm volatile("wgmma.wait_group.sync.aligned %0;" ::"n"(N) : "memory"); }
template <int R> __device__ __forceinline__ void wgmma_fence_regs(float (&d)[R]) {
#pragma unroll
    for (int i = 0; i < R; ++i) asm volatile("" : "+f"(d[i])::"memory");
}
template <int TA, int TB> __device__ __forceinline__ void wgmma_m64n32(float (&d)[16], uint64_t a_desc, uint64_t b_desc) {
    asm volatile(
        "{\n\t"
        "wgmma.mma_async.sync.aligned.m64n32k16.f32.bf16.bf16 "
        "{%0, %1, %2, %3, %4, %5, %6, %7, %8, %9, %10, %11, %12, %13, %14, %15}, %16, %17, 1, 1, 1, %18, %19;\n\t"
        "}"
        : "+f"(d[0]), "+f"(d[1]), "+f"(d[2]), "+f"(d[3]), "+f"(d[4]), "+f"(d[5]), "+f"(d[6]), "+f"(d[7]), "+f"(d[8]), "+f"(d[9]), "+f"(d[10]), "+f"(d[11]), "+f"(d[12]), "+f"(d[13]), "+f"(d[14]), "+f"(d[15])
        : "l"(a_desc), "l"(b_desc), "n"(TA), "n"(TB));
}
template <int TA, int TB, int R> __device__ __forceinline__ void wgmma_m64n64(float (&d)[R], uint64_t a_desc, uint64_t b_desc) {
    static_assert(R >= 32, "m64n64 accumulator");
    asm volatile(
        "{\n\t"
        "wgmma.mma_async.sync.aligned.m64n64k16.f32.bf16.bf16 "
        "{%0, %1, %2, %3, %4, %5, %6, %7, %8, %9, %10, %11, %12, %13, %14, %15, %16, %17, %18, %19, %20, %21, %22, %23, %24, %25, %26, %27, %28, %29, %30, %31}, %32, %33, 1, 1, 1, %34, %35;\n\t"
        "}"
        : "+f"(d[0]), "+f"(d[1]), "+f"(d[2]), "+f"(d[3]), "+f"(d[4]), "+f"(d[5]), "+f"(d[6]), "+f"(d[7]), "+f"(d[8]), "+f"(d[9]), "+f"(d[10]), "+f"(d[11]), "+f"(d[12]), "+f"(d[13]), "+f"(d[14]), "+f"(d[15]), "+f"(d[16]), "+f"(d[17]), "+f"(d[18]), "+f"(d[19]), "+f"(d[20]), "+f"(d[21]), "+f"(d[22]), "+f"(d[23]), "+f"(d[24]), "+f"(d[25]), "+f"(d[26]), "+f"(d[27]), "+f"(d[28]), "+f"(d[29]), "+f"(d[30]), "+f"(d[31])
        : "l"(a_desc), "l"(b_desc), "n"(TA), "n"(TB));
}
template <int TA, int TB> __device__ __forceinline__ void wgmma_m64n128(float (&d)[64], uint64_t a_desc, uint64_t b_desc) {
    asm volatile(
        "{\n\t"
        "wgmma.mma_async.sync.aligned.m64n128k16.f32.bf16.bf16 "
        "{%0, %1, %2, %3, %4, %5, %6, %7, %8, %9, %10, %11, %12, %13, %14, %15, %16, %17, %18, %19, %20, %21, %22, %23, %24, %25, %26, %27, %28, %29, %30, %31, %32, %33, %34, %35, %36, %37, %38, %39, %40, %41, %42, %43, %44, %45, %46, %47, %48, %49, %50, %51, %52, %53, %54, %55, %56, %57, %58, %59, %60, %61, %62, %63}, %64, %65, 1, 1, 1, %66, %67;\n\t"
        "}"
        : "+f"(d[0]), "+f"(d[1]), "+f"(d[2]), "+f"(d[3]), "+f"(d[4]), "+f"(d[5]), "+f"(d[6]), "+f"(d[7]), "+f"(d[8]), "+f"(d[9]), "+f"(d[10]), "+f"(d[11]), "+f"(d[12]), "+f"(d[13]), "+f"(d[14]), "+f"(d[15]), "+f"(d[16]), "+f"(d[17]), "+f"(d[18]), "+f"(d[19]), "+f"(d[20]), "+f"(d[21]), "+f"(d[22]), "+f"(d[23]), "+f"(d[24]), "+f"(d[25]), "+f"(d[26]), "+f"(d[27]), "+f"(d[28]), "+f"(d[29]), "+f"(d[30]), "+f"(d[31]), "+f"(d[32]), "+f"(d[33]), "+f"(d[34]), "+f"(d[35]), "+f"(d[36]), "+f"(d[37]), "+f"(d[38]), "+f"(d[39]), "+f"(d[40]), "+f"(d[41]), "+f"(d[42]), "+f"(d[43]), "+f"(d[44]), "+f"(d[45]), "+f"(d[46]), "+f"(d[47]), "+f"(d[48]), "+f"(d[49]), "+f"(d[50]), "+f"(d[51]), "+f"(d[52]), "+f"(d[53]), "+f"(d[54]), "+f"(d[55]), "+f"(d[56]), "+f"(d[57]), "+f"(d[58]), "+f"(d[59]), "+f"(d[60]), "+f"(d[61]), "+f"(d[62]), "+f"(d[63])
        : "l"(a_desc), "l"(b_desc), "n"(TA), "n"(TB));
}
template <int N, int TA, int TB> __device__ __forceinline__ void wgmma_bf16(float (&d)[N / 2], uint64_t a_desc, uint64_t b_desc) {
    if constexpr (N == 32) wgmma_m64n32<TA, TB>(d, a_desc, b_desc);
    else if constexpr (N == 64) wgmma_m64n64<TA, TB>(d, a_desc, b_desc);
    else if constexpr (N == 128) wgmma_m64n128<TA, TB>(d, a_desc, b_desc);
    else {
        static_assert(N == 256 && TB == 0, "wgmma tile width");
        wgmma_m64n128<TA, TB>(*reinterpret_cast<float (*)[64]>(&d[0]), a_desc, b_desc);
        wgmma_m64n128<TA, TB>(*reinterpret_cast<float (*)[64]>(&d[64]), a_desc, b_desc + (16384 >> 4));
    }
}
template <int N> __device__ __forceinline__ void setmaxnreg_inc() { asm volatile("setmaxnreg.inc.sync.aligned.u32 %0;" ::"n"(N)); }
template <int N> __device__ __forceinline__ void setmaxnreg_dec() { asm volatile("setmaxnreg.dec.sync.aligned.u32 %0;" ::"n"(N)); }
__device__ __forceinline__ void named_sync(int id, int threads) { asm volatile("bar.sync %0, %1;" ::"r"(id), "r"(threads) : "memory"); }

__host__ __device__ __forceinline__ uint64_t make_smem_desc(uint32_t smem_addr, uint32_t lbo_bytes, uint32_t sbo_bytes) {
    uint64_t d = 0;
    d |= static_cast<uint64_t>((smem_addr >> 4) & 0x3FFFu);
    d |= static_cast<uint64_t>((lbo_bytes >> 4) & 0x3FFFu) << 16;
    d |= static_cast<uint64_t>((sbo_bytes >> 4) & 0x3FFFu) << 32;
    d |= 1ull << 62;
    return d;
}
__host__ __device__ __forceinline__ uint64_t make_smem_desc_noswizzle(uint32_t smem_addr, uint32_t lbo_bytes, uint32_t sbo_bytes) {
    uint64_t d = 0;
    d |= static_cast<uint64_t>((smem_addr >> 4) & 0x3FFFu);
    d |= static_cast<uint64_t>((lbo_bytes >> 4) & 0x3FFFu) << 16;
    d |= static_cast<uint64_t>((sbo_bytes >> 4) & 0x3FFFu) << 32;
    return d;
}

}
```

Baseline: 1116.

## Keep stem weights resident in shared memory and split wgrad taps across warpgroups

The space-to-depth stem forward now runs a new TMA kernel variant that loads the whole 4x4x32 weight block into shared memory once per CTA, using 64-byte swizzle and 32-channel rows. This replaces the per-stage weight TMA loads and the separate mask pass, so the pipeline ring only streams activations. Wgrad also gains a 4-tap halo path for kw=4 layers (the stem's sub-conv), where the two warpgroups each take half the taps, which lowers accumulator register pressure. The costs are extra shared memory for resident weights, which leaves fewer ring stages, and new descriptor and swizzle code.

```diff
diff --git a/text_segmentation_image_inpainting_b200/csrc/conv_stem.cu b/text_segmentation_image_inpainting_b200/csrc/conv_stem.cu
--- a/text_segmentation_image_inpainting_b200/csrc/conv_stem.cu
+++ b/text_segmentation_image_inpainting_b200/csrc/conv_stem.cu
@@ -30,7 +30,7 @@
     S.n = c->n; S.h = c->h / 2; S.w = c->w / 2; S.cin = S2D_C; S.cout = c->cout; S.kh = S.kw = SK; S.stride = 1; S.pad_h = S.pad_w = 2; S.dil = 1;
     S.groups = 1; S.ho = S.h; S.wo = S.w; S.dtype = PCB_BF16; S.no_guard = c->no_guard; S.nparts = 1;
     S.parts[0].x = nullptr; S.parts[0].mask = nullptr; S.parts[0].c = S2D_C; S.parts[0].x_cstride = S2D_C;
-    if (!pcb_tc_eligible(&S)) return K;
+    if (!pcb_tc_eligible(&S) || !pcb_tc_resident_fwd_ok(&S)) return K;
     size_t de;
     pcb_tc_weight_layout(&S, &K.sub_fe, &de);
     K.sub_fe = (K.sub_fe + 63) / 64 * 64;
@@ -123,9 +123,7 @@
     bf16 *xs = reinterpret_cast<bf16 *>(ws);
     if (int rc = run_s2d(c, xs, st)) return rc;
     K.sub.parts[0].x = xs;
-    uint64_t *sub_ws = reinterpret_cast<uint64_t *>(ws + s2d_bytes(c) + dwsub_bytes(c));
-    if (int rc = pcb_tc_forward_mask_pass(&K.sub, sub_ws, st)) return rc;
-    return pcb_tc_forward_ws(&K.sub, w_fwd_extra, bias, y, y_cstride, msum, sub_ws, true, bn_sums, ep, st);
+    return pcb_tc_forward_resident(&K.sub, w_fwd_extra, bias, y, y_cstride, msum, bn_sums, ep, st);
 }
 
 int pcb_stem_wgrad(const pcb_conv *c, const void *dc, int dc_cstride, float *dw, void *workspace, bool zero_dw, cudaStream_t st) {
diff --git a/text_segmentation_image_inpainting_b200/csrc/conv_tc.cu b/text_segmentation_image_inpainting_b200/csrc/conv_tc.cu
--- a/text_segmentation_image_inpainting_b200/csrc/conv_tc.cu
+++ b/text_segmentation_image_inpainting_b200/csrc/conv_tc.cu
@@ -697,6 +697,7 @@
               TMA_THREADS * TMA_REGS <= 65536, "TMA-fed fwd / dgrad register budget");
 
 constexpr size_t TMA_BAR_BYTES = 24 * MAX_RING + 16;
+constexpr size_t TMA_RESW_BAR_BYTES = 16;
 
 template <int BLOCK_N, int MODE>
 __device__ __forceinline__ void tc_epilogue_bf16(const TcParams &P, const EpiRow &er, const bf16 *srow, int lane, int n0, float *s_stat) {
@@ -869,24 +870,30 @@
     return true;
 }
 
-template <int BLOCK_N, int MODE, bool HALO>
+template <int BLOCK_N, int MODE, bool HALO, bool RESW>
 __global__ void __maxnreg__(TMA_REGS)
 pconv_tc_tma_kernel(const __grid_constant__ TcParams P, const __grid_constant__ CUtensorMap tmap_w,
                     const __grid_constant__ CUtensorMap tmap_a0, const __grid_constant__ CUtensorMap tmap_a1) {
+    static_assert(!RESW || MODE == 0, "resident weights: forward only");
     constexpr uint32_t B_BYTES = BLOCK_N * 128;
+    constexpr uint32_t ROW = RESW ? 64 : 128;
+    constexpr uint32_t W_TILE = BLOCK_N * ROW;
     extern __shared__ uint8_t smem_raw[];
     const uint32_t smem_base = align1024(ptx::smem_u32(smem_raw));
     const int S = P.stages;
     const int nB = HALO ? P.kw : 1;
     const int hx = HALO ? (P.kw - 1) * P.dil : 0;
-    const uint32_t A_BYTES = static_cast<uint32_t>(BLOCK_M + hx) * 128u;
+    const uint32_t A_BYTES = static_cast<uint32_t>(BLOCK_M + hx) * ROW;
     const uint32_t A_ROOM = (A_BYTES + 1023u) & ~1023u;
-    const uint32_t STAGE = A_ROOM + nB * B_BYTES;
-    const uint32_t STAGE_TX = A_BYTES + nB * B_BYTES;
-    const uint32_t sBar = smem_base + S * STAGE;
+    const uint32_t STAGE = A_ROOM + (RESW ? 0u : nB * B_BYTES);
+    const uint32_t STAGE_TX = A_BYTES + (RESW ? 0u : nB * B_BYTES);
+    const int w_tiles = RESW ? P.kh * P.kw * (P.ktap / BLOCK_K) : 0;
+    const uint32_t sW = smem_base + S * STAGE;
+    const uint32_t sBar = sW + w_tiles * W_TILE;
     const uint32_t bar_full = sBar, bar_fixed = sBar + 8 * MAX_RING, bar_empty = sBar + 16 * MAX_RING;
     const uint32_t acc_full = sBar + 24 * MAX_RING, acc_empty = acc_full + 8;
-    const uint32_t s_stat_addr = sBar + TMA_BAR_BYTES;
+    const uint32_t w_full = sBar + TMA_BAR_BYTES;
+    const uint32_t s_stat_addr = sBar + TMA_BAR_BYTES + (RESW ? TMA_RESW_BAR_BYTES : 0);
     const uint32_t s_acc = s_stat_addr + EPI_STAT_SMEM_BYTES;
     uint8_t *smem_gen = smem_raw + (smem_base - ptx::smem_u32(smem_raw));
 
@@ -898,7 +905,7 @@
     const int num_tiles = m_tiles * n_tiles * KS;
     const int tile0 = static_cast<int>(blockIdx.x), tstep = static_cast<int>(gridDim.x);
     auto m0_of = [&](int mt) -> int { return mt * BLOCK_M; };
-    const bool fix = (MODE == 0) && P.use_fix;
+    const bool fix = (MODE == 0) && P.use_fix && !RESW;
     const int kwi = HALO ? 1 : P.kw;
 
     auto tile_active = [&](int n0) -> bool {
@@ -913,6 +920,7 @@
             ptx::mbar_init(bar_full + 8 * s, 1); ptx::mbar_init(bar_fixed + 8 * s, TMA_FIX_THREADS / 32); ptx::mbar_init(bar_empty + 8 * s, 2);
         }
         ptx::mbar_init(acc_full, MMA_WARPS); ptx::mbar_init(acc_empty, EPI_WARPS);
+        if (RESW) ptx::mbar_init(w_full, 1);
         ptx::fence_mbar_init();
     }
     if (warp == 8 && lane == 0) { ptx::prefetch_tmap(&tmap_w); ptx::prefetch_tmap(&tmap_a0); if (np > 1) ptx::prefetch_tmap(&tmap_a1); }
@@ -926,11 +934,13 @@
         const int e = warp, g = warp >> 2;
         const bool leader = (threadIdx.x & 127) == 0;
         const uint32_t ready = fix ? bar_fixed : bar_full;
-        const uint64_t desc_a0 = ptx::make_smem_desc(smem_base + g * 64 * 128, 16, 1024);
-        const uint64_t desc_b0 = ptx::make_smem_desc(smem_base + A_ROOM, 16, 1024);
+        const uint64_t desc_a0 = RESW ? ptx::make_smem_desc_sw64(smem_base + g * 64 * ROW, 512)
+                                      : ptx::make_smem_desc(smem_base + g * 64 * ROW, 16, 1024);
+        const uint64_t desc_b0 = RESW ? ptx::make_smem_desc_sw64(sW, 512) : ptx::make_smem_desc(smem_base + A_ROOM, 16, 1024);
         const uint32_t stage16 = STAGE >> 4;
+        const uint32_t wtile16 = (RESW ? W_TILE : B_BYTES) >> 4, bstep = RESW ? (P.wk_col / BLOCK_K) * wtile16 : wtile16;
         const int shift0 = (HALO && MODE == 1) ? hx * 8 : 0;
-        const int dshift = HALO ? ((MODE == 1) ? -P.dil * 8 : P.dil * 8) : 0;
+        const int dshift = HALO ? ((MODE == 1) ? -P.dil * 8 : P.dil * static_cast<int>(ROW / 16)) : 0;
         const int rows_a = P.kh * kwi;
         int nb0, nb1 = 0, kl0, kl1 = 4;
         {
@@ -940,7 +950,7 @@
         }
         int s = 0;
         uint32_t ph = 0, aph = 1;
-        bool dead = false;
+        bool dead = RESW && !__all_sync(0xffffffffu, ptx::mbar_wait(w_full, 0, P.abort_flag, 127));
         for (int tile = tile0; tile < num_tiles && !dead; tile += tstep) {
             const int sp = tile % KS, mn = tile / KS;
             const int n0 = (mn % n_tiles) * BLOCK_N;
@@ -950,6 +960,7 @@
             zero_acc(acc);
             int held = -1;
             for (int r = 0; r < rows_a && !dead; ++r) {
+                const int wk_r = RESW ? (P.wk_base + (r / kwi) * P.wk_row + (r % kwi) * P.wk_col) / BLOCK_K : 0;
 #pragma unroll
                 for (int p = 0; p < TC_MAX_PARTS; ++p) {
                     const int nbp = (p == 0) ? nb0 : nb1, klast = (p == 0) ? kl0 : kl1;
@@ -957,10 +968,11 @@
                     for (int cb = 0; cb < nbp; ++cb) {
                         if (KS > 1 && (gb0 + cb) % KS != sp) continue;
                         if (!__all_sync(0xffffffffu, ptx::mbar_wait(ready + 8 * s, ph, P.abort_flag, 124))) { dead = true; break; }
-                        uint64_t da = desc_a0 + static_cast<uint64_t>(s * stage16 + shift0), db = desc_b0 + static_cast<uint64_t>(s * stage16);
+                        uint64_t da = desc_a0 + static_cast<uint64_t>(s * stage16 + shift0);
+                        uint64_t db = desc_b0 + static_cast<uint64_t>(RESW ? (wk_r + gb0 + cb) * wtile16 : s * stage16);
                         const int ksteps = (cb + 1 < nbp) ? 4 : klast;
                         ptx::wgmma_fence();
-                        for (int tc = 0; tc < nB; ++tc, da += dshift, db += B_BYTES >> 4) {
+                        for (int tc = 0; tc < nB; ++tc, da += dshift, db += bstep) {
                             if (ksteps == 4) {
 #pragma unroll
                                 for (int k = 0; k < 4; ++k) ptx::wgmma_bf16<BLOCK_N, 0, 0>(acc, da + 2 * k, db + 2 * k);
@@ -1006,6 +1018,13 @@
             const int dstep = (MODE == 0) ? P.dil : -P.dil;
             const int row_k = P.wk_row, col_k = P.wk_col;
             bool dead = false;
+            if (RESW) {
+                if (ptx::elect_one()) {
+                    ptx::mbar_arrive_expect_tx(w_full, w_tiles * W_TILE);
+                    for (int j = 0; j < w_tiles; ++j) ptx::tma_load_2d(sW + j * W_TILE, &tmap_w, j * BLOCK_K, 0, w_full);
+                }
+                __syncwarp();
+            }
             for (int tile = tile0; tile < num_tiles && !dead; tile += tstep) {
                 const int sp = tile % KS, mn = tile / KS;
                 const int m0 = m0_of(mn / n_tiles), n0 = (mn % n_tiles) * BLOCK_N;
@@ -1041,8 +1060,9 @@
                                     ptx::mbar_arrive_expect_tx(full, STAGE_TX);
                                     ptx::tma_load_4d(dst, ma, c0, x, y, img, full);
                                     uint32_t bdst = dst + A_ROOM;
-                                    for (int tc = 0, kb = kidx; tc < nB; ++tc, kb += col_k, bdst += B_BYTES)
-                                        ptx::tma_load_2d(bdst, &tmap_w, kb, n0, full);
+                                    if (!RESW)
+                                        for (int tc = 0, kb = kidx; tc < nB; ++tc, kb += col_k, bdst += B_BYTES)
+                                            ptx::tma_load_2d(bdst, &tmap_w, kb, n0, full);
                                     if (nimg >= 0) ptx::tma_prefetch_4d(ma, c0, nx_org + ti * dstep, ny_org + tr * dstep, nimg);
                                 }
                                 __syncwarp();
@@ -1664,6 +1684,9 @@
                           const __grid_constant__ CUtensorMap tmap_a0, const __grid_constant__ CUtensorMap tmap_a1) {
     constexpr uint32_t B_BYTES = BLOCK_N * 128;
     constexpr int FIX_ROWS = HALO ? 3 : 1;
+    constexpr bool SPLIT_TAPS = HALO && T == 4;
+    constexpr int TA = SPLIT_TAPS ? T / 2 : T;
+    static_assert(!SPLIT_TAPS || BLOCK_N == 64, "tap split: 64-wide tiles");
     extern __shared__ uint8_t smem_raw[];
     const uint32_t smem_base = align1024(ptx::smem_u32(smem_raw));
     uint8_t *smem_gen = smem_raw + (smem_base - ptx::smem_u32(smem_raw));
@@ -1717,17 +1740,18 @@
         const int g = warp >> 2;
         const int ablk = solo >= 0 ? solo : g;
         const bool split_n = solo >= 0 && BLOCK_N == 128;
-        const bool live = !(solo >= 0 && BLOCK_N == 64) || g == 0;
+        const bool live = SPLIT_TAPS || !(solo >= 0 && BLOCK_N == 64) || g == 0;
         const int nc0 = split_n ? 64 * g : 0, ncols = split_n ? 64 : BLOCK_N;
+        const int tw0 = SPLIT_TAPS ? TA * g : 0;
         const bool leader = (threadIdx.x & 127) == 0;
         const uint32_t ready = fix ? bar_fixed : bar_full;
-        const uint64_t desc_a0 = ptx::make_smem_desc(smem_base + ablk * A_BLK, A_BLK, 1024);
+        const uint32_t tap16 = HALO ? static_cast<uint32_t>(P.dil * 8) : (2 * A_BLK) >> 4;
+        const uint64_t desc_a0 = ptx::make_smem_desc(smem_base + ablk * A_BLK, A_BLK, 1024) + tw0 * tap16;
         const uint64_t desc_b0 = ptx::make_smem_desc(smem_base + A_BYTES + nc0 * 128, 8192, 1024);
         const uint32_t stage16 = STAGE >> 4;
-        const uint32_t tap16 = HALO ? static_cast<uint32_t>(P.dil * 8) : (2 * A_BLK) >> 4;
-        float acc[T][BLOCK_N / 2];
-#pragma unroll
-        for (int tl = 0; tl < T; ++tl) zero_acc(acc[tl]);
+        float acc[TA][BLOCK_N / 2];
+#pragma unroll
+        for (int tl = 0; tl < TA; ++tl) zero_acc(acc[tl]);
         int s = 0, held = -1;
         uint32_t ph = 0;
         bool dead = false;
@@ -1744,16 +1768,16 @@
             ptx::wgmma_fence();
             if (BLOCK_N == 128 && split_n) {
 #pragma unroll
-                for (int tl = 0; tl < T; ++tl, da += tap16) {
-                    if (tl >= ntap) break;
+                for (int tl = 0; tl < TA; ++tl, da += tap16) {
+                    if (tw0 + tl >= ntap) break;
 #pragma unroll
                     for (int k = 0; k < 4; ++k)
                         ptx::wgmma_m64n64<1, 1>(acc[tl], da + 128 * k, db + 128 * k);
                 }
             } else {
 #pragma unroll
-                for (int tl = 0; tl < T; ++tl, da += tap16) {
-                    if (tl >= ntap) break;
+                for (int tl = 0; tl < TA; ++tl, da += tap16) {
+                    if (tw0 + tl >= ntap) break;
 #pragma unroll
                     for (int k = 0; k < 4; ++k)
                         ptx::wgmma_bf16<BLOCK_N, 1, 1>(acc[tl], da + 128 * k, db + 128 * k);
@@ -1767,10 +1791,10 @@
         }
         ptx::wgmma_wait<0>();
 #pragma unroll
-        for (int tl = 0; tl < T; ++tl) ptx::wgmma_fence_regs(acc[tl]);
+        for (int tl = 0; tl < TA; ++tl) ptx::wgmma_fence_regs(acc[tl]);
         if (held >= 0 && leader) ptx::mbar_arrive(bar_empty + 8 * held);
         if (!dead && live && num_kb > 0) {
-            int ci[2], tap[2][T];
+            int ci[2], tap[2][TA];
             for (int h = 0; h < 2; ++h) {
                 const int kpos = ci_tile * 128 + 64 * ablk + 16 * (warp & 3) + (lane >> 2) + 8 * h;
                 ci[h] = -1;
@@ -1779,9 +1803,9 @@
                     if (local >= 0 && local < P.parts[p].c) ci[h] = P.parts[p].choff + local;
                 }
 #pragma unroll
-                for (int tl = 0; tl < T; ++tl) tap[h][tl] = tap0 + tl;
-            }
-            wgrad_store<BLOCK_N, T>(P, acc, ntap, lane, n0 + nc0, ncols, ci, tap);
+                for (int tl = 0; tl < TA; ++tl) tap[h][tl] = tap0 + tw0 + tl;
+            }
+            wgrad_store<BLOCK_N, TA>(P, acc, ntap - tw0, lane, n0 + nc0, ncols, ci, tap);
         }
     } else {
         ptx::setmaxnreg_dec<WGRAD_SUPPORT_REGS>();
@@ -1985,30 +2009,31 @@
     return fn;
 }
 
-int make_tmap_2d(CUtensorMap *tm, const void *base, long long rows, long long cols, long long pitch_elems, int box_rows) {
+int make_tmap_2d(CUtensorMap *tm, const void *base, long long rows, long long cols, long long pitch_elems, int box_rows, bool sw64 = false) {
     EncodeTiledFn enc = get_encode_fn();
     PCB_CHECK(enc != nullptr, "cuTensorMapEncodeTiled not available from the driver");
     cuuint64_t dims[2] = {static_cast<cuuint64_t>(cols), static_cast<cuuint64_t>(rows)};
     cuuint64_t strides[1] = {static_cast<cuuint64_t>(pitch_elems) * 2};
-    cuuint32_t box[2] = {64, static_cast<cuuint32_t>(box_rows)};
+    cuuint32_t box[2] = {sw64 ? 32u : 64u, static_cast<cuuint32_t>(box_rows)};
     cuuint32_t estr[2] = {1, 1};
     CUresult r = enc(tm, CU_TENSOR_MAP_DATA_TYPE_BFLOAT16, 2, const_cast<void *>(base), dims, strides, box, estr,
-                     CU_TENSOR_MAP_INTERLEAVE_NONE, CU_TENSOR_MAP_SWIZZLE_128B, CU_TENSOR_MAP_L2_PROMOTION_L2_256B,
+                     CU_TENSOR_MAP_INTERLEAVE_NONE, sw64 ? CU_TENSOR_MAP_SWIZZLE_64B : CU_TENSOR_MAP_SWIZZLE_128B, CU_TENSOR_MAP_L2_PROMOTION_L2_256B,
                      CU_TENSOR_MAP_FLOAT_OOB_FILL_NONE);
     PCB_CHECK(r == CUDA_SUCCESS, "cuTensorMapEncodeTiled failed (%d) rows=%lld cols=%lld pitch=%lld box_rows=%d base=%p", (int)r,
               rows, cols, pitch_elems, box_rows, base);
     return 0;
 }
 
-int make_tmap_nhwc(CUtensorMap *tm, const void *base, int channels, int w, int h, int n, long long cstride, int bx, int by, int bn, int es) {
+int make_tmap_nhwc(CUtensorMap *tm, const void *base, int channels, int w, int h, int n, long long cstride, int bx, int by, int bn, int es,
+                   bool sw64 = false) {
     EncodeTiledFn enc = get_encode_fn();
     PCB_CHECK(enc != nullptr, "cuTensorMapEncodeTiled not available from the driver");
     cuuint64_t dims[4] = {static_cast<cuuint64_t>(channels), static_cast<cuuint64_t>(w), static_cast<cuuint64_t>(h), static_cast<cuuint64_t>(n)};
     cuuint64_t strides[3] = {static_cast<cuuint64_t>(cstride) * 2, static_cast<cuuint64_t>(w) * cstride * 2, static_cast<cuuint64_t>(h) * w * cstride * 2};
-    cuuint32_t box[4] = {64, static_cast<cuuint32_t>(bx * es), static_cast<cuuint32_t>(by * es), static_cast<cuuint32_t>(bn)};
+    cuuint32_t box[4] = {sw64 ? 32u : 64u, static_cast<cuuint32_t>(bx * es), static_cast<cuuint32_t>(by * es), static_cast<cuuint32_t>(bn)};
     cuuint32_t estr[4] = {1, static_cast<cuuint32_t>(es), static_cast<cuuint32_t>(es), 1};
     CUresult r = enc(tm, CU_TENSOR_MAP_DATA_TYPE_BFLOAT16, 4, const_cast<void *>(base), dims, strides, box, estr,
-                     CU_TENSOR_MAP_INTERLEAVE_NONE, CU_TENSOR_MAP_SWIZZLE_128B, CU_TENSOR_MAP_L2_PROMOTION_L2_256B,
+                     CU_TENSOR_MAP_INTERLEAVE_NONE, sw64 ? CU_TENSOR_MAP_SWIZZLE_64B : CU_TENSOR_MAP_SWIZZLE_128B, CU_TENSOR_MAP_L2_PROMOTION_L2_256B,
                      CU_TENSOR_MAP_FLOAT_OOB_FILL_NONE);
     PCB_CHECK(r == CUDA_SUCCESS, "cuTensorMapEncodeTiled(4D) failed (%d) c=%d w=%d h=%d n=%d cstride=%lld box=%d,%d,%d es=%d base=%p", (int)r,
               channels, w, h, n, cstride, bx, by, bn, es, base);
@@ -2266,17 +2291,25 @@
     return 1024 + TMA_BAR_BYTES + EPI_STAT_SMEM_BYTES + (splitk ? acc_stage_bytes(block_n) : bf16_stage_bytes(block_n));
 }
 
-template <int BLOCK_N, int MODE, bool HALO>
+size_t resident_w_bytes(int kblocks, int block_n) { return static_cast<size_t>(kblocks) * block_n * 64 + TMA_RESW_BAR_BYTES; }
+size_t resident_a_room(int kw, int dil, bool halo) {
+    return (static_cast<size_t>(BLOCK_M + (halo ? (kw - 1) * dil : 0)) * 64 + 1023) / 1024 * 1024;
+}
+
+template <int BLOCK_N, int MODE, bool HALO, bool RESW = false>
 int launch_tma_n(TcParams &P, const CUtensorMap &tw, const CUtensorMap &ta0, const CUtensorMap &ta1, cudaStream_t st) {
     const int nb = HALO ? P.kw : 1;
-    const size_t a_room = (static_cast<size_t>(BLOCK_M + (HALO ? (P.kw - 1) * P.dil : 0)) * 128 + 1023) / 1024 * 1024;
-    const size_t stage = a_room + static_cast<size_t>(nb) * BLOCK_N * 128;
+    const size_t a_room = RESW ? resident_a_room(P.kw, P.dil, HALO)
+                               : (static_cast<size_t>(BLOCK_M + (HALO ? (P.kw - 1) * P.dil : 0)) * 128 + 1023) / 1024 * 1024;
+    const size_t stage = a_room + (RESW ? 0 : static_cast<size_t>(nb) * BLOCK_N * 128);
     PCB_CHECK(BLOCK_N <= 128 || P.partial == nullptr, "TMA-fed conv: split-K stages fp32 partials, at most 128 columns wide");
-    const size_t fixed = tma_fixed_smem(BLOCK_N, P.partial != nullptr);
+    PCB_CHECK(!RESW || (P.partial == nullptr && P.ncols == BLOCK_N), "TMA-fed conv: resident weights need one N tile and no split-K");
+    const size_t fixed = tma_fixed_smem(BLOCK_N, P.partial != nullptr) + (RESW ? resident_w_bytes(P.kh * P.kw * (P.ktap / BLOCK_K), BLOCK_N) : 0);
+    PCB_CHECK(fixed < MAX_SMEM, "TMA-fed conv: %zu bytes of resident weights do not fit", fixed);
     P.stages = static_cast<int>(std::min<size_t>(MAX_RING, (MAX_SMEM - fixed) / stage));
     PCB_CHECK(P.stages >= 2, "TMA-fed conv: stage of %zu bytes does not fit twice", stage);
     const size_t smem = fixed + P.stages * stage;
-    auto kern = pconv_tc_tma_kernel<BLOCK_N, MODE, HALO>;
+    auto kern = pconv_tc_tma_kernel<BLOCK_N, MODE, HALO, RESW>;
     PCB_SMEM_OPT_IN(kern, MAX_SMEM);
     if (P.ksplit < 1) P.ksplit = 1;
     const int m_tiles = (P.m_total + BLOCK_M - 1) / BLOCK_M;
@@ -2874,6 +2907,43 @@
     return launch_tc<0>(P, tm, L.bn_f, st);
 }
 
+bool pcb_tc_resident_fwd_ok(const pcb_conv *c) {
+    if (!common_ok(c) || is_rowpack(c) || !tma_fwd_ok(c) || c->nparts != 1 || c->parts[0].mask || c->parts[0].x_up) return false;
+    if (rup(c->parts[0].c, 8) > 32) return false;
+    const Layout L = layout_of(c);
+    if (L.rows_f != 64) return false;
+    const size_t w_bytes = resident_w_bytes(static_cast<int>(L.kf / BLOCK_K), 64);
+    return tma_fixed_smem(64, false) + w_bytes + 2 * resident_a_room(c->kw, c->dil, true) <= MAX_SMEM;
+}
+
+int pcb_tc_forward_resident(const pcb_conv *c, const void *w_fwd, const float *bias, void *y, int y_cstride, const float *msum,
+                            double *bn_sums, const pcb_ep *ep, cudaStream_t st) {
+    PCB_CHECK(pcb_tc_resident_fwd_ok(c), "resident-weight forward: the problem does not take this path");
+    int *flag = abort_flag_ptr();
+    PCB_CHECK(flag != nullptr, "cudaMalloc(abort flag) failed");
+    const long long m_total = static_cast<long long>(c->n) * c->ho * c->wo;
+    PCB_CHECK(m_total < (1ll << 31), "problem too large");
+    PCB_CHECK(y_cstride % 8 == 0 && y_cstride >= c->cout, "tensor-core forward: y channel stride must be a multiple of 8 and >= cout");
+    const Layout L = layout_of(c);
+    TcParams P;
+    base_params(P, c, L);
+    P.m_total = static_cast<int>(m_total);
+    fill_parts(c, L, P.parts, nullptr, m_total);
+    P.bias = bias; P.msum = msum; P.y = static_cast<bf16 *>(y); P.y_cstride = y_cstride; P.abort_flag = flag;
+    P.bn_sums = bn_sums; P.bn_c = c->cout;
+    set_ep(P, ep);
+    P.ncols = L.rows_f; P.ksplit = 1;
+    tile_box(c->wo, c->ho, &P.box_w, &P.box_h, &P.box_n);
+    const bool halo = tma_halo_ok(c, P.box_w, P.box_h, P.box_n, 64);
+    const int hx = halo ? (c->kw - 1) * c->dil : 0;
+    CUtensorMap ta, tm;
+    const pcb_part &pt = c->parts[0];
+    if (int rc = make_tmap_nhwc(&ta, pt.x, rup(pt.c, 8), c->w, c->h, c->n, pt.x_cstride, P.box_w + hx, P.box_h, P.box_n, c->stride, true)) return rc;
+    P.wk_base = 0; P.wk_col = L.ktap; P.wk_row = c->kw * L.ktap;
+    if (int rc = make_tmap_2d(&tm, w_fwd, L.rows_f, L.kf, L.kf, 64, true)) return rc;
+    return halo ? launch_tma_n<64, 0, true, true>(P, tm, ta, ta, st) : launch_tma_n<64, 0, false, true>(P, tm, ta, ta, st);
+}
+
 bool pcb_tc_dgrad_supported(const pcb_conv *c) { return pcb_tc_eligible(c) && !is_rowpack(c); }
 
 int pcb_tc_dgrad(const pcb_conv *c, const void *dc, int dc_cstride, const void *w_dgrad, void *const *dx, const int *dx_cstride,
@@ -3093,9 +3163,11 @@
     if (int rc = make_tmap_2d(&tm, dc, m_total, c->cout, dc_cstride, 64)) return rc;
     if (tma_wgrad_ok(c)) {
         kblock_box(c->wo, c->ho, &P.box_w, &P.box_h, &P.box_n);
-        const bool halo = !getenv("PCB_DISABLE_TMA_HALO") && c->stride == 1 && c->kw == 3 && P.box_w == 64 &&
-                          P.box_h == 1 && P.box_n == 1 && 64 + (c->kw - 1) * c->dil <= 256;
-        const int hx = halo ? (c->kw - 1) * c->dil : 0;
+        const bool halo_box = !getenv("PCB_DISABLE_TMA_HALO") && c->stride == 1 && P.box_w == 64 && P.box_h == 1 && P.box_n == 1 &&
+                              64 + (c->kw - 1) * c->dil <= 256;
+        const bool halo = halo_box && c->kw == 3;
+        const bool halo_split4 = halo_box && c->kw == 4 && c->cout <= 64 && L.ktap == BLOCK_K;
+        const int hx = (halo || halo_split4) ? (c->kw - 1) * c->dil : 0;
         CUtensorMap ta[TC_MAX_PARTS];
         memset(ta, 0, sizeof(ta));
         uint8_t *extra = reinterpret_cast<uint8_t *>(workspace) + tapmask_bytes(c);
@@ -3117,6 +3189,7 @@
             if (int rc = make_tmap_nhwc(&ta[p], src, c8, c->w, c->h, c->n, cs, P.box_w + hx, P.box_h, P.box_n, c->stride)) return rc;
         }
         if (c->nparts < 2) ta[1] = ta[0];
+        if (halo_split4) return launch_wgrad_tma<64, 4, true>(P, tm, ta[0], ta[1], st);
         if (c->cout > 64 && m_total >= 128 * 64) {
             if (halo) return launch_wgrad_tma<128, 3, true>(P, tm, ta[0], ta[1], st);
             return launch_wgrad_tma<128, 3, false>(P, tm, ta[0], ta[1], st);
diff --git a/text_segmentation_image_inpainting_b200/csrc/pcb_common.cuh b/text_segmentation_image_inpainting_b200/csrc/pcb_common.cuh
--- a/text_segmentation_image_inpainting_b200/csrc/pcb_common.cuh
+++ b/text_segmentation_image_inpainting_b200/csrc/pcb_common.cuh
@@ -135,6 +135,9 @@
 int pcb_tc_forward_mask_pass(const pcb_conv *c, uint64_t *tapmask, cudaStream_t st);
 int pcb_tc_forward_ws(const pcb_conv *c, const void *w_fwd, const float *bias, void *y, int y_cstride, const float *msum,
                       uint64_t *tapmask, bool mask_pass_done, double *bn_sums, const pcb_ep *ep, cudaStream_t st);
+bool pcb_tc_resident_fwd_ok(const pcb_conv *c);
+int pcb_tc_forward_resident(const pcb_conv *c, const void *w_fwd, const float *bias, void *y, int y_cstride, const float *msum,
+                            double *bn_sums, const pcb_ep *ep, cudaStream_t st);
 bool pcb_tc_fuses_bn_stats(const pcb_conv *c);
 bool pcb_tc_fuses_affine_act(const pcb_conv *c);
 bool pcb_tc_subpixel(const pcb_conv *c);
diff --git a/text_segmentation_image_inpainting_b200/csrc/pcb_ptx.cuh b/text_segmentation_image_inpainting_b200/csrc/pcb_ptx.cuh
--- a/text_segmentation_image_inpainting_b200/csrc/pcb_ptx.cuh
+++ b/text_segmentation_image_inpainting_b200/csrc/pcb_ptx.cuh
@@ -139,6 +139,14 @@
     d |= 1ull << 62;
     return d;
 }
+__host__ __device__ __forceinline__ uint64_t make_smem_desc_sw64(uint32_t smem_addr, uint32_t sbo_bytes) {
+    uint64_t d = 0;
+    d |= static_cast<uint64_t>((smem_addr >> 4) & 0x3FFFu);
+    d |= 1ull << 16;
+    d |= static_cast<uint64_t>((sbo_bytes >> 4) & 0x3FFFu) << 32;
+    d |= 2ull << 62;
+    return d;
+}
 __host__ __device__ __forceinline__ uint64_t make_smem_desc_noswizzle(uint32_t smem_addr, uint32_t lbo_bytes, uint32_t sbo_bytes) {
     uint64_t d = 0;
     d |= static_cast<uint64_t>((smem_addr >> 4) & 0x3FFFu);
```

New measurement: 1149, median of 6. 3.0% higher.
